# Zokrates/ZoKrates

Measured on AMD Instinct MI355X. Metric: groth16_proofs_per_sec, higher is better.
Workload: dtype u32

## Files before the change

### include/zkhip.h

```cpp
#ifndef ZKHIP_H
#define ZKHIP_H

#include <stddef.h>
#include <stdint.h>

#ifdef __cplusplus
extern "C" {
#endif

#define ZKHIP_OK 0
#define ZKHIP_ERR_BAD_ARG (-1)
#define ZKHIP_ERR_PARSE (-2)
#define ZKHIP_ERR_NOMEM (-3)
#define ZKHIP_ERR_DEVICE (-4)
#define ZKHIP_ERR_UNSATISFIED (-5)
#define ZKHIP_ERR_BUSY (-6)

#define ZKHIP_CURVE_BN128 0
#define ZKHIP_CURVE_BLS12_381 1
#define ZKHIP_CURVE_BLS12_377 2

typedef struct zkhip_ctx zkhip_ctx;
typedef struct zkhip_pk zkhip_pk;
typedef struct zkhip_r1cs zkhip_r1cs;
// ... 55 lines not shown
                        const uint64_t* rowptr_b, const uint32_t* col_b, const uint8_t* val_b,
                        const uint64_t* rowptr_c, const uint32_t* col_c, const uint8_t* val_c,
                        zkhip_r1cs** out);
void zkhip_r1cs_free(zkhip_r1cs* r1cs);

int32_t zkhip_prove_g16(zkhip_ctx* ctx, const zkhip_pk* pk, const zkhip_r1cs* r1cs, const uint8_t* z,
                        const uint8_t* r, const uint8_t* s, uint8_t* proof_out, zkhip_timings* timings);

int32_t zkhip_assignment_upload(zkhip_ctx* ctx, const zkhip_r1cs* r1cs, const uint8_t* z, zkhip_assignment** out);
void zkhip_assignment_free(zkhip_assignment* z);
int32_t zkhip_prove_g16_resident(zkhip_ctx* ctx, const zkhip_pk* pk, const zkhip_r1cs* r1cs, zkhip_assignment* z,
                                 const uint8_t* r, const uint8_t* s, uint8_t* proof_out, zkhip_timings* timings);

int32_t zkhip_assignment_pack_bound(uint64_t m, uint64_t* bytes);
int32_t zkhip_assignment_pack(const uint8_t* z, uint64_t m, uint8_t* out, uint64_t cap, uint64_t* len);
int32_t zkhip_assignment_unpack(const uint8_t* packed, size_t len, uint8_t* z_out, uint64_t m_cap, uint64_t* m);
int32_t zkhip_prog_assignment_packed(const zkhip_prog* prog, const uint8_t* witness, size_t len, uint8_t* packed_out,
                                     uint64_t cap, uint64_t* packed_len, uint8_t* inputs_out, uint64_t inputs_cap,
                                     uint64_t* n_inputs);
int32_t zkhip_assignment_upload_packed(zkhip_ctx* ctx, const zkhip_r1cs* r1cs, const uint8_t* packed, size_t len,
                                       zkhip_assignment** out);

int32_t zkhip_prove_g16_batch(zkhip_ctx* ctx, const zkhip_pk* pk, const zkhip_r1cs* r1cs, uint32_t count,
                              const uint8_t* z, const uint8_t* rs, uint8_t* proofs_out, zkhip_timings* timings);
int32_t zkhip_prove_g16_resident_batch(zkhip_ctx* ctx, const zkhip_pk* pk, const zkhip_r1cs* r1cs, uint32_t count,
                                       zkhip_assignment* const* zs, const uint8_t* rs, uint8_t* proofs_out,
                                       zkhip_timings* timings);

int32_t zkhip_r1cs_check(zkhip_ctx* ctx, const zkhip_r1cs* r1cs, const uint8_t* z, zkhip_assignment* z_resident,
                         uint64_t* first_row, uint64_t* n_bad);
int32_t zkhip_ctx_set_checked(zkhip_ctx* ctx, int32_t on);
int32_t zkhip_ctx_unsatisfied(const zkhip_ctx* ctx, uint32_t cap, uint32_t* proof_idx, uint64_t* first_row,
                              uint64_t* n_bad, uint32_t* count);

typedef struct zkhip_queue zkhip_queue;
int32_t zkhip_queue_open(zkhip_ctx* ctx, const zkhip_pk* pk, const zkhip_r1cs* r1cs, zkhip_queue** out);
int32_t zkhip_queue_state(const zkhip_queue* q, uint32_t* capacity, uint32_t* in_flight);
int32_t zkhip_queue_submit(zkhip_queue* q, const uint8_t* z, zkhip_assignment* z_resident, const uint8_t* rnd, uint64_t* ticket);
int32_t zkhip_queue_submit_packed(zkhip_queue* q, const uint8_t* packed, size_t len, const uint8_t* rnd, uint64_t* ticket);
int32_t zkhip_queue_ready(zkhip_queue* q, int32_t* ready);
int32_t zkhip_queue_collect(zkhip_queue* q, uint64_t* ticket, uint8_t* proof_out, zkhip_timings* timings);
int32_t zkhip_queue_close(zkhip_queue* q);

int32_t zkhip_pk_load_g16_shard(zkhip_ctx* ctx, int32_t curve, const uint8_t* bytes, size_t len, uint32_t rank,
                                uint32_t world, zkhip_pk** out);
int32_t zkhip_partial_size(int32_t curve, uint64_t* bytes);
int32_t zkhip_prove_g16_partial(zkhip_ctx* ctx, const zkhip_pk* pk_shard, const zkhip_r1cs* r1cs, const uint8_t* z,
                                zkhip_assignment* z_resident, const uint8_t* r, const uint8_t* s, uint8_t* partial_out,
                                zkhip_timings* timings);
int32_t zkhip_combine_g16(zkhip_ctx* ctx, const zkhip_pk* pk, uint32_t count, const uint8_t* partials, const uint8_t* r,
                          const uint8_t* s, uint8_t* proof_out);

int32_t zkhip_ntt(zkhip_ctx* ctx, int32_t curve, uint32_t log_n, int32_t dir, uint8_t* data);
int32_t zkhip_witness_map(zkhip_ctx* ctx, const zkhip_r1cs* r1cs, const uint8_t* z, uint8_t* h_out);
int32_t zkhip_msm_g1(zkhip_ctx* ctx, int32_t curve, uint64_t n, const uint8_t* bases, const uint8_t* scalars, uint8_t* out);
int32_t zkhip_msm_g2(zkhip_ctx* ctx, int32_t curve, uint64_t n, const uint8_t* bases, const uint8_t* scalars, uint8_t* out);
int32_t zkhip_field_op(zkhip_ctx* ctx, int32_t curve, int32_t field, int32_t op, uint64_t count,
                       const uint8_t* a, const uint8_t* b, uint8_t* out);

int32_t zkhip_setup_g16_size(const zkhip_r1cs* r1cs, uint64_t* pk_bytes);
int32_t zkhip_setup_g16(zkhip_ctx* ctx, const zkhip_r1cs* r1cs, const uint8_t* toxic, const uint8_t* g1,
                        const uint8_t* g2, uint8_t* pk_out, uint64_t pk_cap);

int32_t zkhip_pk_load_gm17(zkhip_ctx* ctx, int32_t curve, const uint8_t* bytes, size_t len, zkhip_pk** out);
int32_t zkhip_prove_gm17(zkhip_ctx* ctx, const zkhip_pk* pk, const zkhip_r1cs* r1cs, const uint8_t* z, const uint8_t* d1_d2_r,
                         uint8_t* proof_out, zkhip_timings* timings);
// ... 79 lines not shown
```

### integration/zokrates_hip/src/ffi.rs

```rust
#![allow(non_camel_case_types)]
use std::os::raw::c_char;

#[repr(C)] pub struct zkhip_ctx { _p: [u8; 0] }
#[repr(C)] pub struct zkhip_pk { _p: [u8; 0] }
#[repr(C)] pub struct zkhip_r1cs { _p: [u8; 0] }
#[repr(C)] pub struct zkhip_multi { _p: [u8; 0] }
#[repr(C)] pub struct zkhip_prog { _p: [u8; 0] }
#[repr(C)] pub struct zkhip_assignment { _p: [u8; 0] }
#[repr(C)] pub struct zkhip_queue { _p: [u8; 0] }
pub const ZKHIP_ERR_BUSY: i32 = -6;
#[repr(C)] #[derive(Default, Clone, Copy)] pub struct zkhip_timings { pub ms: [f32; 16] }

pub const ZKHIP_CURVE_BN128: i32 = 0;
pub const ZKHIP_CURVE_BLS12_381: i32 = 1;
pub const ZKHIP_CURVE_BLS12_377: i32 = 2;

pub const ZKHIP_TUNE_PIPE_PLAN: i32 = 28;

extern "C" {
    pub fn zkhip_init(hw_queues: i32) -> i32;
    pub fn zkhip_ctx_create(device: i32, out: *mut *mut zkhip_ctx) -> i32;
    pub fn zkhip_ctx_free(ctx: *mut zkhip_ctx);
    pub fn zkhip_ctx_tune(ctx: *mut zkhip_ctx, which: i32, value: i32) -> i32;
    pub fn zkhip_last_error(ctx: *const zkhip_ctx) -> *const c_char;
// ... 6 lines not shown
        rp_c: *const u64, col_c: *const u32, val_c: *const u8, out: *mut *mut zkhip_r1cs) -> i32;
    pub fn zkhip_r1cs_free(cs: *mut zkhip_r1cs);
    pub fn zkhip_prove_g16(ctx: *mut zkhip_ctx, pk: *const zkhip_pk, cs: *const zkhip_r1cs, z: *const u8,
        r: *const u8, s: *const u8, proof_out: *mut u8, timings: *mut zkhip_timings) -> i32;
    pub fn zkhip_prove_gm17(ctx: *mut zkhip_ctx, pk: *const zkhip_pk, cs: *const zkhip_r1cs, z: *const u8,
        d1_d2_r: *const u8, proof_out: *mut u8, timings: *mut zkhip_timings) -> i32;
    pub fn zkhip_prog_parse(bytes: *const u8, len: usize, out: *mut *mut zkhip_prog) -> i32;
    pub fn zkhip_prog_free(prog: *mut zkhip_prog);
    pub fn zkhip_prog_dims(prog: *const zkhip_prog, out: *mut u64 ) -> i32;
    pub fn zkhip_prog_r1cs_load(ctx: *mut zkhip_ctx, prog: *const zkhip_prog, out: *mut *mut zkhip_r1cs) -> i32;
    pub fn zkhip_prog_assignment(prog: *const zkhip_prog, witness: *const u8, len: usize, z_out: *mut u8,
        inputs_out: *mut u8, inputs_cap: u64, n_inputs: *mut u64) -> i32;
    pub fn zkhip_assignment_pack_bound(m: u64, bytes: *mut u64) -> i32;
    pub fn zkhip_assignment_pack(z: *const u8, m: u64, out: *mut u8, cap: u64, len: *mut u64) -> i32;
    pub fn zkhip_assignment_unpack(packed: *const u8, len: usize, z_out: *mut u8, m_cap: u64, m: *mut u64) -> i32;
    pub fn zkhip_prog_assignment_packed(prog: *const zkhip_prog, witness: *const u8, len: usize, packed_out: *mut u8,
        cap: u64, packed_len: *mut u64, inputs_out: *mut u8, inputs_cap: u64, n_inputs: *mut u64) -> i32;
    pub fn zkhip_assignment_upload_packed(ctx: *mut zkhip_ctx, r1cs: *const zkhip_r1cs, packed: *const u8, len: usize,
        out: *mut *mut zkhip_assignment) -> i32;
    pub fn zkhip_assignment_free(z: *mut zkhip_assignment);
    pub fn zkhip_prove_g16_resident(ctx: *mut zkhip_ctx, pk: *const zkhip_pk, cs: *const zkhip_r1cs, z: *mut zkhip_assignment,
        r: *const u8, s: *const u8, proof_out: *mut u8, timings: *mut zkhip_timings) -> i32;
    pub fn zkhip_pk_export_size(pk: *const zkhip_pk, bytes: *mut u64) -> i32;
    pub fn zkhip_pk_export(pk: *const zkhip_pk, out: *mut u8, cap: u64) -> i32;
    pub fn zkhip_pk_import(ctx: *mut zkhip_ctx, bytes: *const u8, len: usize, out: *mut *mut zkhip_pk) -> i32;
    pub fn zkhip_pk_bind_r1cs(ctx: *mut zkhip_ctx, pk: *mut zkhip_pk, r1cs: *const zkhip_r1cs) -> i32;
    pub fn zkhip_pk_unbind(pk: *mut zkhip_pk) -> i32;
    pub fn zkhip_pk_is_bound(pk: *const zkhip_pk, r1cs: *const zkhip_r1cs) -> i32;
    pub fn zkhip_r1cs_check(ctx: *mut zkhip_ctx, r1cs: *const zkhip_r1cs, z: *const u8, z_resident: *mut zkhip_assignment,
        first_row: *mut u64, n_bad: *mut u64) -> i32;
    pub fn zkhip_ctx_set_checked(ctx: *mut zkhip_ctx, on: i32) -> i32;
    pub fn zkhip_ctx_unsatisfied(ctx: *const zkhip_ctx, cap: u32, proof_idx: *mut u32, first_row: *mut u64, n_bad: *mut u64,
        count: *mut u32) -> i32;
    pub fn zkhip_queue_open(ctx: *mut zkhip_ctx, pk: *const zkhip_pk, r1cs: *const zkhip_r1cs, out: *mut *mut zkhip_queue) -> i32;
    pub fn zkhip_queue_state(q: *const zkhip_queue, capacity: *mut u32, in_flight: *mut u32) -> i32;
    pub fn zkhip_queue_submit(q: *mut zkhip_queue, z: *const u8, z_resident: *mut zkhip_assignment, rnd: *const u8, ticket: *mut u64) -> i32;
    pub fn zkhip_queue_submit_packed(q: *mut zkhip_queue, packed: *const u8, len: usize, rnd: *const u8, ticket: *mut u64) -> i32;
    pub fn zkhip_queue_ready(q: *mut zkhip_queue, ready: *mut i32) -> i32;
    pub fn zkhip_queue_collect(q: *mut zkhip_queue, ticket: *mut u64, proof_out: *mut u8, timings: *mut zkhip_timings) -> i32;
    pub fn zkhip_queue_close(q: *mut zkhip_queue) -> i32;
    pub fn zkhip_pk_bind_r1cs_shard(ctx: *mut zkhip_ctx, pk: *mut zkhip_pk, r1cs: *const zkhip_r1cs, key_bytes: *const u8, len: usize) -> i32;
    pub fn zkhip_prove_g16_split_begin(ctx: *mut zkhip_ctx, pk: *const zkhip_pk, r1cs: *const zkhip_r1cs, z: *const u8,
        z_resident: *mut zkhip_assignment, r: *const u8, s: *const u8, half: i32, half_out: *mut u8) -> i32;
    pub fn zkhip_prove_g16_split_end(ctx: *mut zkhip_ctx, pk: *const zkhip_pk, r1cs: *const zkhip_r1cs, other_half: *const u8,
        partial_out: *mut u8, timings: *mut zkhip_timings) -> i32;
    pub fn zkhip_prove_g16_split_abort(ctx: *mut zkhip_ctx) -> i32;
    pub fn zkhip_ctx_create_multi(devices: *const i32, n: i32, out: *mut *mut zkhip_multi) -> i32;
    pub fn zkhip_multi_free(m: *mut zkhip_multi);
    pub fn zkhip_multi_last_error(m: *const zkhip_multi) -> *const c_char;
    pub fn zkhip_multi_use_rccl(m: *mut zkhip_multi, on: i32) -> i32;
    pub fn zkhip_multi_exchange(m: *const zkhip_multi) -> *const c_char;
    pub fn zkhip_multi_r1cs_load(m: *mut zkhip_multi, curve: i32, n: u64, l: u64, w: u64,
        rp_a: *const u64, col_a: *const u32, val_a: *const u8,
        rp_b: *const u64, col_b: *const u32, val_b: *const u8,
        rp_c: *const u64, col_c: *const u32, val_c: *const u8) -> i32;
    pub fn zkhip_multi_pk_load_g16(m: *mut zkhip_multi, curve: i32, bytes: *const u8, len: usize) -> i32;
    pub fn zkhip_multi_pk_load_gm17(m: *mut zkhip_multi, curve: i32, bytes: *const u8, len: usize) -> i32;
    pub fn zkhip_multi_bind(m: *mut zkhip_multi, key_bytes: *const u8, len: usize) -> i32;
    pub fn zkhip_multi_unbind(m: *mut zkhip_multi) -> i32;
    pub fn zkhip_multi_transform_split(m: *mut zkhip_multi, on: i32) -> i32;
    pub fn zkhip_prove_g16_multi(m: *mut zkhip_multi, z: *const u8, r: *const u8, s: *const u8, proof_out: *mut u8,
        timings: *mut zkhip_timings) -> i32;
    pub fn zkhip_prove_gm17_multi(m: *mut zkhip_multi, z: *const u8, d1_d2_r: *const u8, proof_out: *mut u8,
        timings: *mut zkhip_timings) -> i32;
    pub fn zkhip_multi_pk_load_g16_replicas(m: *mut zkhip_multi, curve: i32, bytes: *const u8, len: usize) -> i32;
    pub fn zkhip_prove_g16_multi_batch(m: *mut zkhip_multi, count: u32, z: *const u8, rs: *const u8, proofs_out: *mut u8,
// ... 3 lines not shown
```

### zokrates_amd/csrc/core.cuh

```cuda
#pragma once
#include <algorithm>
#include <atomic>
#include <chrono>
#include <cstdio>
#include <memory>
#include <new>
#include <string>
#include <system_error>
#include <thread>
#include <type_traits>
#include <unordered_set>
#include <vector>

#include "../../include/zkhip.h"
#include "devrt.h"
#include "ec.cuh"
#include "kernels_msm.cuh"
#include "kernels_ntt.cuh"
#include "zpack.cuh"

namespace zk {

struct CurveBn254 {
    static constexpr int ID = ZKHIP_CURVE_BN128;
// ... 49 lines not shown
        dev_free(p);
        p = nullptr;
        cap = 0;
        p = dev_alloc(bytes);
        cap = bytes;
    }
};
template <class T> static inline T* ptr(const DBuf& b) { return (T*)b.p; }

static inline unsigned blocks_for(u64 n, unsigned threads) { return (unsigned)((n + threads - 1) / threads); }
static inline int ilog2_floor(u64 x) { int l = 0; while (x >>= 1) ++l; return l; }
static inline int ilog2_ceil(u64 x) { int l = 0; while (((u64)1 << l) < x) ++l; return l; }

}

using namespace zk;

struct NttPlanBase {
    int curve, logN;
    virtual ~NttPlanBase() {}
};
struct MsmSort {
    DBuf dig, sorted, cnt, off, cursor, chunk_sum, grand;
    DBuf pairs, ccur, tile_off;
    Event ready = nullptr;
};
struct MsmLane {
    Stream stream = 0;
    bool made = false;
    bool high_priority = false;
    DBuf lane_key, heavy, partial, bucket, rows, cols;
    Event done = nullptr;
};
static constexpr int ZK_NLANES = 5;
static constexpr int ZK_NSLOTS = 4;
struct ProofSlot {
    DBuf scalars, zmont, va, vb, vc, ws1, ws2, zflag;
    DBuf verdict;
    int check_idx = -1;
    MsmSort sorts[3];
    MsmLane lanes[ZK_NLANES];
    void* h_ws = nullptr;
    size_t h_ws_cap = 0;
    Event ev[4] = {nullptr, nullptr, nullptr, nullptr};
    Event acc_b[ZK_NLANES] = {}, acc_e[ZK_NLANES] = {};
    Event ntt_b = nullptr, ntt_e = nullptr;
    Event g1_go = nullptr;
    Event half_ready = nullptr;
    int half = -1;
    bool lone = false;
    bool split_pending = false;
    const zkhip_pk* split_pk = nullptr;
    const zkhip_r1cs* split_cs = nullptr;
    bool split_bound = false;
    bool ready = false;
    bool busy = false;
    uint8_t r[32], s[32];
    std::chrono::steady_clock::time_point t_start;
};
struct PackedZ {
    const uint8_t* bytes;
    size_t len;
    u64 tags_off, index_off, payload_off;
};
struct zkhip_queue {
    zkhip_ctx* ctx = nullptr;
    const zkhip_pk* pk = nullptr;
    const zkhip_r1cs* cs = nullptr;
    u32 cap = 0;
    u64 head = 0, next = 0;
    bool checked = false;
    bool broken = false;
    std::string dev_err;
};
struct zkhip_ctx {
    int device = 0;
    Stream stream = 0;
    Stream out_stream = 0;
    Stream ntt_stream = 0;
    bool out_made = false, ntt_made = false;
    Stream ws = 0;
    bool serial = false;
    bool g2_first = true;
    int cus = 256;
    int msm_c_env = 0;
    int b_sort_mode = 0;
    int skip_inf_mode = 0;
    int msm_sets = 0;
    int msm_waves = 0;
    u32 msm_lanes = 0;
    u32 msm_min_slice = 8;
    bool heavy_runs = true;
    int fold_hg = 32;
    bool fold_scan = true;
    bool fuse_z = true;
    int msm_fused_waves = 0;
    int msm_g1_waves = 0, msm_g2_waves = 0;
    int z_gate = 1;
    int g2_head_start = 1;
    int split_min_log = 18;
    int ntt_single_max = 10;
    int ntt_max_sublog = 11;
    int ntt_cols = 2;
    std::vector<Stream> idle_streams;
    std::string pipe_plan;
    bool pipes_made = false;
    Stream ntt_lone_stream = 0;
    bool ntt_lone_made = false;
    int ntt_fuse_first = 1;
    u32 sort_wgs = 256;
    int tenants = 1;
    int nslots = 3;
    bool checked = false;
    struct Unsatisfied { u32 proof; u64 first_row, n_bad; };
    std::vector<Unsatisfied> unsat;
    std::string err;
    std::string desc;
    ProofSlot slots[ZK_NSLOTS];
    ProofSlot* cur = &slots[0];
    zkhip_queue* queue = nullptr;
    DBuf tmp;
    DBuf zpack;
    std::vector<std::unique_ptr<NttPlanBase>> plans;
    std::unordered_set<const void*> lds_opted;
};
#define ZK_PIPE_PLAN_RESIDENT "M=2,N=3,O=1,n=3,G0=0,Z0=1,H0=0,G1=3,Z1=1,H1=0,G2=3,Z2=2,H2=1"
struct PipeWant { Stream* target; bool* made; bool high; int cls; bool done; };
static inline void make_pipe_streams(zkhip_ctx* ctx) {
    if (ctx->pipes_made || ctx->pipe_plan.empty() || ctx->serial) return;
    ctx->pipes_made = true;
    auto find = [&](const std::string& key) -> int {
        size_t pos = 0;
        const std::string& pl = ctx->pipe_plan;
        while (pos < pl.size()) {
            size_t end = pl.find(',', pos);
            if (end == std::string::npos) end = pl.size();
            const std::string tok = pl.substr(pos, end - pos);
            const size_t eq = tok.find('=');
            if (eq != std::string::npos && tok.substr(0, eq) == key && eq + 1 < tok.size() && tok[eq + 1] >= '0' && tok[eq + 1] <= '3') return tok[eq + 1] - '0';
            pos = end + 1;
        }
        return -1;
    };
    std::vector<PipeWant> want;
    static bool dummy_made;
    int c;
    if ((c = find("M")) >= 0) { stream_sync(ctx->stream); stream_destroy(ctx->stream); ctx->stream = 0; want.push_back({&ctx->stream, &dummy_made, true, c, false}); }
    if ((c = find("N")) >= 0 && !ctx->ntt_made) want.push_back({&ctx->ntt_stream, &ctx->ntt_made, true, c, false});
// ... 317 lines not shown
        }
    }
    if (ctx && ctx->msm_c_env) s.c = ctx->msm_c_env;
    if (force_c) s.c = force_c;
    s.c = std::min(s.c, MSM_MAX_C);
    s.W = (scalar_bits + 1 + s.c - 1) / s.c;
    s.K = 1u << (s.c - 1);
    s.sets = table ? (u32)std::max(1, std::min(force_sets ? force_sets : 1, s.W)) : (u32)s.W;
    s.levels = ((u32)s.W + s.sets - 1) / s.sets;
    s.nkeys = s.sets * s.K;
    s.Lw = std::min<u32>(s.K, 256);
    s.H = s.K / s.Lw;
    return s;
}

static inline MsmShape with_inf(MsmShape sh, bool many) { sh.skip_inf = many; return sh; }
static inline u64 msm_table_budget(const zkhip_ctx* ctx, u64 z_n, u64 h_n, u64 N, int W, u32 K) {
    size_t free_b = 0, total_b = 0;
    dev_mem_info(&free_b, &total_b);
    const u64 per_slot = (2 * z_n + h_n) * (u64)W * 16 + 4 * N * 32 + (z_n + 2) * 64 + 6 * ((u64)K + (1u << 19)) * 288 + ((u64)1 << 29);
    const u64 later = (u64)std::max(1, ctx->nslots) * per_slot + ((u64)1 << 30);
    const u64 budget = (u64)((ctx->tenants > 1 ? 0.5 : 0.6) * (double)free_b) / (u64)std::max(1, ctx->tenants);
    return budget > later ? budget - later : 0;
}
static inline void scan_u32(Stream s, const DBuf& cnt, DBuf& off, u64 nk, DBuf& chunk_sum, DBuf& grand) {
    const u32 nchunks = (u32)((nk + SCAN_CHUNK - 1) / SCAN_CHUNK);
    off.ensure((nk + 1) * 4);
    chunk_sum.ensure((size_t)nchunks * 4);
    grand.ensure(4);
    ZK_LAUNCH(k_scan_local, dim3(nchunks), dim3(SCAN_THREADS), 0, s, ptr<u32>(cnt), ptr<u32>(off), ptr<u32>(chunk_sum), nk);
    ZK_LAUNCH(k_scan_chunks, dim3(1), dim3(SCAN_THREADS), 0, s, ptr<u32>(chunk_sum), nchunks, ptr<u32>(grand));
    ZK_LAUNCH(k_scan_add, dim3(blocks_for(nk + 1, 256)), dim3(256), 0, s, ptr<u32>(off), ptr<u32>(chunk_sum), nk, ptr<u32>(grand));
}
static inline void msm_prepare(zkhip_ctx* ctx, Stream s, MsmSort& so, const u32* d_scalars, const MsmShape& sh, u64 level_stride,
                               const u32* keep = nullptr, const MsmSort* wm_of = nullptr) {
    const u64 nk = sh.nkeys;
    require(sh.n * (u64)sh.W < ((u64)1 << 32) - sh.nkeys, ZKHIP_ERR_BAD_ARG, "MSM too large for 32-bit sort offsets");
    require(level_stride * (u64)sh.levels < ((u64)1 << 31) && sh.n < ((u64)1 << 31), ZKHIP_ERR_BAD_ARG, "MSM too large for 31-bit table indices");
    if (!wm_of) so.dig.ensure(sh.n * (u64)sh.W * 4);
    so.sorted.ensure(sh.n * sh.W * 4);
    const unsigned T = 256;
    const u32 kh = std::min(sh.K, MSM_SORT_MAX_KH), halves = sh.K / kh;
    const u64 want_chunks = halves > 1 ? std::max<u64>(1, ctx->sort_wgs / (sh.W * halves)) : std::max<u64>(1, (ctx->sort_wgs + sh.W - 1) / sh.W);
    const u64 max_chunks = std::max<u64>(1, sh.n / (2 * (u64)kh));
    const u64 sort_chunks = std::min(want_chunks, max_chunks);
    const u64 chunk = (sh.n + sort_chunks - 1) / sort_chunks;
    const size_t hist_bytes = (size_t)kh * 4;
    const bool two_level = sh.K >= (1u << MSM_COARSE_BITS) && sh.K <= (1u << 16);
    const u32 nbins = (u32)(nk >> MSM_COARSE_BITS);
    so.cnt.ensure(nk * 4);
    so.cursor.ensure(nk * 4);
    if (two_level) {
        so.ccur.ensure((size_t)nbins * 4);
        so.tile_off.ensure(((size_t)nbins + 1) * 4);
    }
    const MsmZero zero{{ptr<u32>(so.cnt), ptr<u32>(so.cursor), two_level ? ptr<u32>(so.ccur) : nullptr}, {(u32)nk, (u32)nk, two_level ? nbins : 0u}};
    if (!wm_of) ZK_LAUNCH(k_msm_digits, dim3(blocks_for(sh.n, T)), dim3(T), 0, s, d_scalars, sh.n, sh.c, sh.W, ptr<u32>(so.dig), zero);
    else ZK_LAUNCH(k_msm_zero, dim3(blocks_for(nk, T)), dim3(T), 0, s, zero);
    const u32* wm = wm_of ? ptr<u32>(wm_of->dig) : ptr<u32>(so.dig);
    lds_opt_in(ctx, (const void*)k_msm_count);
    lds_opt_in(ctx, (const void*)k_msm_place);
    ZK_LAUNCH(k_msm_count, dim3((unsigned)sort_chunks, sh.W, halves), dim3(ZK_SORT_THREADS), hist_bytes, s, wm, sh.n, sh.c, sh.W, chunk, sh.sets, kh,
              ptr<u32>(so.cnt), keep);
    if (nk <= SCAN_ONE_MAX) {
        so.off.ensure((nk + 1) * 4);
        ZK_LAUNCH(k_scan_one, dim3(1), dim3(SCAN_ONE_THREADS), 0, s, ptr<u32>(so.cnt), ptr<u32>(so.off), (u32)nk, two_level ? ptr<u32>(so.tile_off) : (u32*)nullptr, nbins);
    } else {
        scan_u32(s, so.cnt, so.off, nk, so.chunk_sum, so.grand);
        if (two_level) ZK_LAUNCH(k_msm_tile_offsets, dim3(1), dim3(MSM_TILE_SCAN_THREADS), 0, s, ptr<u32>(so.off), nbins, ptr<u32>(so.tile_off));
    }
    if (two_level) {
        const u64 total_max = sh.n * (u64)sh.W;
        so.pairs.ensure(std::max<u64>(total_max, 1) * 8);
        const u64 c_chunks = std::max<u64>(1, std::min<u64>((1024 + sh.W - 1) / sh.W, (sh.n + 4095) / 4096));
        const u64 c_chunk = (sh.n + c_chunks - 1) / c_chunks;
        ZK_LAUNCH(k_msm_part_coarse, dim3((unsigned)c_chunks, sh.W), dim3(256), 0, s, wm, sh.n, sh.c, sh.W, c_chunk, sh.sets, level_stride, ptr<u32>(so.off),
                  ptr<u32>(so.ccur), (unsigned long long*)so.pairs.p, keep);
        const u64 max_tiles = total_max / MSM_FINE_TILE + nbins;
        ZK_LAUNCH(k_msm_part_fine, dim3((unsigned)max_tiles), dim3(256), 0, s, (const unsigned long long*)so.pairs.p, ptr<u32>(so.off), ptr<u32>(so.tile_off), nbins,
                  ptr<u32>(so.cursor), ptr<u32>(so.sorted));
    } else {
        ZK_LAUNCH(k_msm_place, dim3((unsigned)sort_chunks, sh.W, halves), dim3(ZK_SORT_THREADS), hist_bytes, s, wm, sh.n, sh.c, sh.W, chunk, sh.sets, kh,
                  level_stride, ptr<u32>(so.off), ptr<u32>(so.cursor), ptr<u32>(so.sorted), keep);
    }
    event_record(so.ready, s);
}

template <class F>
void msm_run(zkhip_ctx* ctx, MsmLane& lane, const MsmSort& so, const void* d_table, const MsmShape& sh, Xyzz<F>* d_window_sums,
             Event ev_begin, Event ev_end, Event accum_after = nullptr, Xyzz<F>* h_window_sums = nullptr);
template <class F>
void msm_run_tables(zkhip_ctx* ctx, MsmLane& lane, const MsmSort& so, const void* const* d_tables, int nt, const MsmShape& sh, Xyzz<F>* d_window_sums,
                    u32 sum_stride, Event ev_begin, Event ev_end, Event accum_after, Xyzz<F>* h_window_sums = nullptr);
template <class F>
void points_to_packed(zkhip_ctx* ctx, const Aff<F>* d_in, void* d_out, u64 n);
template <class F>
void msm_table_levels(zkhip_ctx* ctx, void* d_table, u64 count, int bits, int L);
template <class F>
u64 count_infinite(zkhip_ctx* ctx, const void* d_table, u64 count);
template <class F>
void mark_finite(zkhip_ctx* ctx, const void* d_table, u64 count, u32* d_bitmap);
template <class F> static constexpr size_t packed_point_bytes() { return sizeof(AffPacked<typename Unsat<F>::type>); }
template <class F>
size_t bind_xyzz_bytes();
template <class F>
void bind_scale(zkhip_ctx* ctx, const void* d_h_table, u64 N, u64 n_src, u32 n1, u32 n2, u32 n3, const u32* d_scal, const u32* d_konst, int nw, void* d_x);
template <class F>
void bind_fft(zkhip_ctx* ctx, void* d_x, u64 N, const u32* d_tw, int nw);
template <class F>
void bind_h_finish(zkhip_ctx* ctx, const void* d_x, u64 N, int logN, void* d_out);
template <class F>
void bind_cmul(zkhip_ctx* ctx, const void* d_x, int logN, const u32* d_row, const u32* d_val, int nw, const u32* d_minus_one, u64 nnz, void* d_prod);
template <class F>
void bind_l_finish(zkhip_ctx* ctx, const void* d_prod, const u64* d_cptr, const void* d_l_table, u64 m, const u32* d_long_cols, u64 n_long, void* d_sum, void* d_out);
template <class F>
void fixed_base_table(zkhip_ctx* ctx, const Aff<F>* h_pj, int nwin, DBuf& tbl);
template <class F>
void fixed_base_mul(zkhip_ctx* ctx, const DBuf& tbl, int nwin, const u32* d_scalars, u64 count, Aff<F>* d_out);

template <class F>
static Xyzz<F> msm_combine(const Xyzz<F>* ws, const MsmShape& sh) {
    auto set_sum = [&](int j) {
        Xyzz<F> t = ws[sh.ndig * j];
        for (u32 d = 1; d < sh.ndig; ++d) t = xyzz_add(t, ws[sh.ndig * j + d]);
        return t;
    };
// ... 23 lines not shown
static void decode_point(const uint8_t* src, uint8_t* dst) {
    constexpr int SZ = FQ_BYTES * NCOORD;
    const bool inf = src[SZ - 1] & 0x40;
    if (inf) { memset(dst, 0, SZ); return; }
    memcpy(dst, src, SZ);
    dst[SZ - 1] &= 0x3f;
}
template <class F> static void write_fe(const F& mont, uint8_t* out) { F c = fe_from_mont(mont); memcpy(out, c.v, F::BYTES); }

}

struct zkhip_pk {
    int curve;
    int scheme = 0;
    zkhip_ctx* ctx;
    u64 m, w, l, hlen, N;
    int logN;
    DBuf a_ext, b1_ext, l_ext, b2_ext, h_sigma;
    std::vector<uint8_t> delta_g1_canon;
    std::vector<uint8_t> g_gamma2_z2_canon;
    u32 rank = 0, world = 1;
    u64 z_lo = 0, z_n = 0, h_lo = 0, h_n = 0;
    int c_z = 0, c_h = 0;
    DBuf thin_keep;
    u32 thin_mask = 0;
    bool inf_many_thin[4] = {true, true, true, true};
    bool inf_many[5] = {true, true, true, true, true};
    int s_z = 1, s_h = 1;
    int ntt_log1 = -1;
    DBuf h_bound, l_bound;
    u64 bound_uid = 0;
    u64 bound_fp[2] = {0, 0};
    bool inf_many_bound[2] = {true, true};
};

static const char PK_IMAGE_MAGIC[8] = {'Z', 'K', 'H', 'I', 'P', 'P', 'K', '5'};
struct PkImageHeader {
    char magic[8];
    int32_t curve, scheme;
    uint64_t m, w, l, hlen, N;
    int32_t logN, c_z, c_h, sets;
    uint32_t rank, world;
    int32_t ntt_split, reserved;
    uint64_t z_lo, z_n, h_lo, h_n;
    uint64_t len_delta, len_g2z2, len_buf[5];
    uint64_t len_bound[2];
    uint64_t bound_fp[2];
};

static inline u64 zk_next_uid() {
    static std::atomic<u64> next{1};
    return next.fetch_add(1);
}
struct zkhip_r1cs {
    u64 uid = zk_next_uid();
    int curve;
    zkhip_ctx* ctx;
    u64 n, l, w, N;
    int logN;
    DBuf rp[3], col[3], val[3];
    u64 nnz[3];
    u64 nnz_short[3];
    DBuf long_rows;
    u64 n_long = 0, n_huge = 0;
    u64 fp[2] = {0, 0};
    bool fp_made = false;
// ... 20 lines not shown
struct zkhip_assignment {
    int curve;
    zkhip_ctx* ctx;
    u64 m;
    DBuf scalars;
};

namespace zk {

template <class C>
struct SlotSums {
    typedef Xyzz<typename C::Fq> G1;
    typedef Xyzz<typename C::Fq2> G2;
    MsmShape shz, shh;
    int Wmax;
    SlotSums(const zkhip_ctx* ctx, const zkhip_pk* pk)
        : shz(msm_shape(ctx, pk->z_n, C::Fr::Params::BITS, true, pk->c_z, pk->s_z)), shh(msm_shape(ctx, pk->h_n, C::Fr::Params::BITS, true, pk->c_h, pk->s_h)) {
        require(shz.c == pk->c_z && shh.c == pk->c_h && (int)shz.sets == pk->s_z && (int)shh.sets == pk->s_h, ZKHIP_ERR_BAD_ARG,
                "the key's tables were built for a window width this build cannot sort: reload the key");
        Wmax = (int)std::max(shz.nsums(), shh.nsums());
    }
    size_t b1() const { return (size_t)4 * Wmax * sizeof(G1); }
    size_t b2() const { return (size_t)Wmax * sizeof(G2); }
    size_t lane_bytes() const { return (size_t)Wmax * sizeof(G1); }
    size_t record_bytes() const { return b1() + b2() + 24; }
    template <class T> T* lane(T* g1_sums, int k) const { return g1_sums + (size_t)k * Wmax; }
    G1* ws1(const ProofSlot& sl, int k) const { return lane(ptr<G1>(sl.ws1), k); }
    G2* ws2(const ProofSlot& sl) const { return ptr<G2>(sl.ws2); }
    G1* hs1(const ProofSlot& sl, int k) const { return lane((G1*)sl.h_ws, k); }
    G2* hs2(const ProofSlot& sl) const { return (G2*)((uint8_t*)sl.h_ws + b1()); }
    uint8_t* zflag(const ProofSlot& sl) const { return (uint8_t*)sl.h_ws + b1() + b2(); }
    uint8_t* verdict(const ProofSlot& sl) const { return zflag(sl) + 8; }
    u32 zflag_word(const ProofSlot& sl) const { u32 f; memcpy(&f, zflag(sl), 4); return f; }
    void reserve(ProofSlot& sl) const {
        sl.ws1.ensure(b1());
        sl.ws2.ensure(b2());
        if (sl.h_ws_cap < record_bytes()) {
            host_free_pinned(sl.h_ws);
            sl.h_ws = nullptr; sl.h_ws_cap = 0;
            sl.h_ws = host_alloc_pinned(record_bytes());
            sl.h_ws_cap = record_bytes();
        }
    }
};

struct KeySources {
    int scheme;
    u64 m, w, l, hlen, N;
    struct Lane {
        const uint8_t* src; u64 nsrc, shift;
        const uint8_t* extra; u64 extra_at;
        const uint8_t* add0;
    } lane[4];
    const uint8_t* h_src; u64 h_nsrc;
    const uint8_t *delta_g1, *g_gamma2_z2;
};
struct SapShape {
    u64 M, D0, D;
    int logD;
};
static inline SapShape sap_shape(u64 n, u64 l, u64 w) {
    SapShape s;
    s.M = 1 + 2 * (l - 1) + w + n;
    s.D0 = 2 * n + 2 * (l - 1) + 1;
    s.logD = ilog2_ceil(s.D0);
    s.D = (u64)1 << s.logD;
// ... 719 lines not shown
                 (unsigned long long)cs->n, (unsigned long long)u.n_bad);
        throw ApiError{ZKHIP_ERR_UNSATISFIED, msg};
    }
    static Fr k_to_rp() {
        Fr rp = Fr::one();
        for (int i = 32 * Fr::N; i < Fu<typename Fr::Params>::B * Fu<typename Fr::Params>::N; ++i) rp = fe_add(rp, rp);
        return fe_to_mont(rp);
    }
    static void r1cs_check(zkhip_ctx* ctx, const zkhip_r1cs* cs, const uint8_t* z_host, const void* z_dev, u64 out[2]) {
        ProofSlot& sl = *ctx->cur;
        Stream s = ctx->stream;
        ctx->ws = s;
        const u64 m = cs->l + cs->w, n = cs->n;
        const Fr* z = stage_z(ctx, sl, m, m + 2, z_host, z_dev, true, true);
        sl.zmont.ensure(m * 32);
        ZK_LAUNCH((k_mul_const<Fr>), dim3(blocks_for(m, 256)), dim3(256), 0, s, z, ptr<Fr>(sl.zmont), m, k_to_rp());
        sl.vc.ensure(3 * std::max<u64>(n, 1) * sizeof(Fr));
        Fr *ra = ptr<Fr>(sl.vc), *rb = ra + n, *rc = rb + n;
        if (n) matvec(ctx, cs, ptr<Fr>(sl.zmont), ra, rb, rc, n, 0, n);
        enqueue_check(sl, ra, rb, rc, n, s);
        u32 flag = 0;
        dev_d2h(&flag, sl.zflag.p, 4, s);
        dev_d2h(out, sl.verdict.p, 16, s);
        stream_sync(s);
        require_canonical(flag);
    }

    static void upload_z(zkhip_ctx* ctx, DBuf& dst, u64 m, u64 cap, const uint8_t* z, DBuf& flag) {
        Fr z0 = fe_from_bytes_canon<Fr>(z);
        Fr one = Fr::zero(); one.v[0] = 1;
        require(z0.equals(one), ZKHIP_ERR_BAD_ARG, Z0_NOT_ONE_MSG);
        dst.ensure(cap * 32);
        dev_h2d(dst.p, z, m * 32, ctx->stream);
        flag.ensure(4);
        dev_memset(flag.p, 0, 4, ctx->stream);
        ZK_LAUNCH((k_check_canonical<Fr>), dim3(blocks_for(m, 256)), dim3(256), 0, ctx->stream, ptr<Fr>(dst), m, ptr<u32>(flag));
    }
    static void unpack_z(zkhip_ctx* ctx, DBuf& dst, u64 m, u64 cap, const PackedZ& zp, DBuf& flag) {
        Stream s = ctx->stream;
        dst.ensure(cap * 32);
        ctx->zpack.ensure(zp.len);
        dev_h2d(ctx->zpack.p, zp.bytes, zp.len, s);
        flag.ensure(4);
        dev_memset(flag.p, 0, 4, s);
        const uint8_t* d = ptr<uint8_t>(ctx->zpack);
        ZK_LAUNCH((k_unpack_assignment<Fr>), dim3(blocks_for(m, ZPACK_BLOCK_ELEMS)), dim3(256), 0, s, d + zp.tags_off, (const u64*)(d + zp.index_off),
                  d + zp.payload_off, ptr<Fr>(dst), m, ptr<u32>(flag));
    }
    static const Fr* stage_z(zkhip_ctx* ctx, ProofSlot& sl, u64 m, u64 cap, const uint8_t* z_host, const void* z_dev, bool checked, bool in_place = false,
                             const PackedZ* zp = nullptr) {
        Stream st = ctx->stream;
        if (zp) {
            unpack_z(ctx, sl.scalars, m, cap, *zp, sl.zflag);
            if (checked) verdict_reset(sl, st);
            return ptr<Fr>(sl.scalars);
        }
        if (z_host) {
            upload_z(ctx, sl.scalars, m, cap, z_host, sl.zflag);
        } else {
            if (!in_place) {
                sl.scalars.ensure(cap * 32);
                dev_d2d(sl.scalars.p, z_dev, m * 32, st);
            }
            sl.zflag.ensure(4);
            dev_memset(sl.zflag.p, 0, 4, st);
        }
        if (checked) verdict_reset(sl, st);
        return (z_host || !in_place) ? ptr<Fr>(sl.scalars) : (const Fr*)z_dev;
    }
    static void require_canonical(u32 flag) {
        require(flag == 0, ZKHIP_ERR_BAD_ARG, "an assignment entry is not a canonical field element (>= r)");
    }
    static void stage_scalars(zkhip_ctx* ctx, NttPlan<C>* pl, void* d_scalars, u64 m, const uint8_t* r, const uint8_t* s_) {
        Stream s = ctx->stream;
        ctx->cur->zmont.ensure(m * 32);
        dev_h2d((uint8_t*)d_scalars + m * 32, r, 32, s);
        dev_h2d((uint8_t*)d_scalars + (m + 1) * 32, s_, 32, s);
        ZK_LAUNCH((k_mul_const<Fr>), dim3(blocks_for(m, 256)), dim3(256), 0, s, (const Fr*)d_scalars, ptr<Fr>(ctx->cur->zmont), m, pl->k_to_rp);
    }

    static void enqueue(zkhip_ctx* ctx, ProofSlot& sl, const zkhip_pk* pk, const zkhip_r1cs* cs, const uint8_t* z_host, const void* z_dev,
                        const uint8_t* r, const uint8_t* s_, bool lone = false, int check_idx = -1, const PackedZ* zp = nullptr) {
        enqueue_head(ctx, sl, pk, cs, z_host, z_dev, r, s_, lone, -1, check_idx, zp);
        enqueue_tail(ctx, sl, pk, cs);
    }
    static bool can_split(const zkhip_ctx* ctx, const zkhip_pk* pk, const zkhip_r1cs* cs) {
        return pk->scheme == 0 && is_bound(pk, cs) && pk->logN >= ctx->split_min_log;
    }
    static bool is_bound(const zkhip_pk* pk, const zkhip_r1cs* cs) { return pk->bound_uid != 0 && pk->bound_uid == cs->uid; }
    static NttPlan<C>* open_slot(zkhip_ctx* ctx, ProofSlot& sl, const zkhip_pk* pk) {
        require(!sl.busy, ZKHIP_ERR_DEVICE, "internal: proof slot still in flight");
        make_pipe_streams(ctx);
        slot_init(ctx, sl);
        NttPlan<C>* pl = get_plan<C>(ctx, pk->logN);
        require(pl->split() == pk->ntt_log1, ZKHIP_ERR_BAD_ARG, "the key's h bases were ordered for another NTT split (NTT_SINGLE_MAX_LOG changed): reload the key");
        sl.t_start = std::chrono::steady_clock::now();
        ctx->cur = &sl;
        ctx->ws = ctx->stream;
        return pl;
    }
    static void enqueue_head(zkhip_ctx* ctx, ProofSlot& sl, const zkhip_pk* pk, const zkhip_r1cs* cs, const uint8_t* z_host, const void* z_dev,
                             const uint8_t* r, const uint8_t* s_, bool lone, int half, int check_idx = -1, const PackedZ* zp = nullptr) {
        PkLoader<C>::check_match(pk, cs, 0);
        const bool bound = is_bound(pk, cs);
        require(half < 0 || (bound && half <= 1), ZKHIP_ERR_BAD_ARG, "internal: only a proof over a bound key splits its witness map");
        Fr rr = fe_from_bytes_canon<Fr>(r), ss = fe_from_bytes_canon<Fr>(s_);
        require(canon_lt_mod(rr) && canon_lt_mod(ss), ZKHIP_ERR_BAD_ARG, "r or s not a canonical field element");
        NttPlan<C>* pl = open_slot(ctx, sl, pk);
        sl.half = half;
        sl.lone = lone;
        sl.check_idx = half < 0 ? check_idx : -1;
        memcpy(sl.r, r, 32);
        memcpy(sl.s, s_, 32);
        Stream st = ctx->stream;
        stage_z(ctx, sl, pk->m, pk->m + 2, z_host, z_dev, sl.check_idx >= 0, false, zp);
        stage_scalars(ctx, pl, sl.scalars.p, pk->m, r, s_);
        event_record(sl.ev[0], st);

        const Lay ly(ctx, pk);
        ly.reserve(sl);
        start_z_lanes(ctx, sl, pk, ly);

        Stream wn = ctx->serial ? st : slot_ntt_stream(ctx, sl);
        stream_wait_event(wn, sl.ev[0]);
        event_record(sl.ev[1], wn);
        ctx->ws = wn;
        witness_map(ctx, cs, pl, bound, half, sl.check_idx >= 0);
        ctx->ws = ctx->stream;
        if (half >= 0) {
            event_record(sl.half_ready, wn);
            sl.split_pk = pk;
            sl.split_cs = cs;
            sl.split_bound = bound;
            sl.split_pending = true;
        }
    }
    static void enqueue_tail(zkhip_ctx* ctx, ProofSlot& sl, const zkhip_pk* pk, const zkhip_r1cs* cs) {
        const u64 N = pk->N;
        ctx->cur = &sl;
        Stream wn = ctx->serial ? ctx->stream : slot_ntt_stream(ctx, sl);
        const u32* h_scalars = ptr<u32>(sl.va) + (sl.half >= 0 ? 2 * N * 8 : 0);
        if (sl.half >= 0) {
            Fr* a = ptr<Fr>(sl.va);
            ZK_LAUNCH((k_quotient<typename Fr::Params>), dim3(blocks_for(N, 256)), dim3(256), 0, wn, a, a + N, fe_from_mont(get_plan<C>(ctx, pk->logN)->zinv), a + 2 * N, N);
        }
        lanes_after_h(ctx, sl, pk, Lay(ctx, pk), sl.half >= 0 ? sl.split_bound : is_bound(pk, cs), sl.lone, h_scalars, wn);
    }

    static void start_z_lanes(zkhip_ctx* ctx, ProofSlot& sl, const zkhip_pk* pk, const Lay& ly) {
        if (!pk->z_n) return;
        const u32* digits = ptr<u32>(sl.scalars) + pk->z_lo * 8;
        msm_prepare(ctx, ctx->stream, sl.sorts[0], digits, ly.shz, pk->z_n);
        if (pk->thin_mask) msm_prepare(ctx, ctx->stream, sl.sorts[2], digits, ly.shz, pk->z_n, ptr<u32>(pk->thin_keep), &sl.sorts[0]);
        if (z_gate(ctx) < 2) run_g2(ctx, sl, pk, ly, nullptr);
    }
    static void run_g2(zkhip_ctx* ctx, ProofSlot& sl, const zkhip_pk* pk, const Lay& ly, Event after) {
        const bool thin = pk->thin_mask & 8;
        msm_run<Fq2>(ctx, sl.lanes[3], sl.sorts[thin ? 2 : 0], pk->b2_ext.p, with_inf(ly.shz, thin ? pk->inf_many_thin[3] : pk->inf_many[3]), ly.ws2(sl),
                     sl.acc_b[4], sl.acc_e[4], after, ly.hs2(sl));
    }
    static void lanes_after_h(zkhip_ctx* ctx, ProofSlot& sl, const zkhip_pk* pk, const Lay& ly, bool bound, bool lone, const u32* h_scalars, Stream wn) {
        Stream st = ctx->stream;
        event_record(sl.ev[2], wn);
        if (pk->z_n) {
            const int gate = z_gate(ctx);
            const Event h_ready = gate ? sl.ev[2] : nullptr;
            if (gate >= 2) run_g2(ctx, sl, pk, ly, h_ready);
            Event g1_after = h_ready;
            constexpr bool g2_owns_simds = MsmTuning<typename Unsat<Fq2>::type>::ACCUM_WPE == 1;
            if (g2_owns_simds && lone && !ctx->serial && (ctx->g2_head_start == 2 || (ctx->g2_head_start == 1 && bound))) {
                if (h_ready) stream_wait_event(st, h_ready);
                stream_wait_event(st, sl.acc_e[4]);
                event_record(sl.g1_go, st);
                g1_after = sl.g1_go;
            }
            run_z_g1(ctx, sl, pk, ly, g1_after, bound);
        } else {
            empty_msm(ctx, sl, ly, true);
        }
        if (pk->h_n) {
            msm_prepare(ctx, wn, sl.sorts[1], h_scalars + pk->h_lo * 8, ly.shh, pk->h_n);
            msm_run<Fq>(ctx, sl.lanes[4], sl.sorts[1], bound ? pk->h_bound.p : pk->h_sigma.p, with_inf(ly.shh, bound ? pk->inf_many_bound[1] : pk->inf_many[4]),
                        ly.ws1(sl, 3), sl.acc_b[3], sl.acc_e[3], nullptr, ly.hs1(sl, 3));
        } else {
            empty_msm(ctx, sl, ly, false);
        }
        copy_out(ctx, sl, ly);
    }

    static void run_z_g1(zkhip_ctx* ctx, ProofSlot& sl, const zkhip_pk* pk, const Lay& ly, Event h_ready, bool bound) {
        const void* tab[3] = {pk->a_ext.p, pk->b1_ext.p, bound ? pk->l_bound.p : pk->l_ext.p};
        auto thin = [&](int k) { return (bound && k == 2) ? 0u : (pk->thin_mask >> k) & 1u; };
        auto inf_many = [&](int k) { return (bound && k == 2) ? pk->inf_many_bound[0] : thin(k) ? pk->inf_many_thin[k] : pk->inf_many[k]; };
        if (!ctx->fuse_z) {
            for (int k = 0; k < 3; ++k)
                msm_run<Fq>(ctx, sl.lanes[k], thin(k) ? sl.sorts[2] : sl.sorts[0], tab[k], with_inf(ly.shz, inf_many(k)), ly.ws1(sl, k), sl.acc_b[k], sl.acc_e[k], h_ready,
                            ly.hs1(sl, k));
            return;
        }
        for (u32 which = 0; which < 2; ++which) {
            int member[3], nm = 0;
            for (int k = 0; k < 3; ++k)
                if (thin(k) == which) member[nm++] = k;
            if (!nm) continue;
            const int lead = member[0];
            const void* tabs[3];
            bool many = false;
            for (int q = 0; q < nm; ++q) { tabs[q] = tab[member[q]]; many = many || inf_many(member[q]); }
            const int step = nm > 1 ? member[1] - member[0] : 1;
            msm_run_tables<Fq>(ctx, sl.lanes[lead], which ? sl.sorts[2] : sl.sorts[0], tabs, nm, with_inf(ly.shz, many), ly.ws1(sl, lead), (u32)(step * ly.Wmax),
                               sl.acc_b[lead], sl.acc_e[lead], h_ready, ly.hs1(sl, lead));
            Stream s0 = ctx->serial ? ctx->stream : lane_stream(sl.lanes[lead]);
            for (int q = 1; q < nm; ++q) {
                event_record(sl.acc_b[member[q]], s0);
                event_record(sl.acc_e[member[q]], s0);
                event_record(sl.lanes[member[q]].done, s0);
            }
        }
    }

    static void copy_out(zkhip_ctx* ctx, ProofSlot& sl, const Lay& ly) {
        Stream st = ctx->stream;
        Stream so = ctx->serial ? st : ctx_out_stream(ctx);
        for (int k = 0; k < ZK_NLANES; ++k) stream_wait_event(so, sl.lanes[k].done);
        sl.zflag.ensure(4);
        dev_d2h_pinned(ly.zflag(sl), sl.zflag.p, 4, so);
        if (sl.check_idx >= 0) {
            stream_wait_event(so, sl.ev[2]);
            dev_d2h_pinned(ly.verdict(sl), sl.verdict.p, 16, so);
        }
        event_record(sl.ev[3], so);
        sl.busy = true;
    }

    static void empty_msm(zkhip_ctx* ctx, ProofSlot& sl, const Lay& ly, bool over_z) {
        Stream st = ctx->stream;
        const int k0 = over_z ? 0 : 3, nk = over_z ? 3 : 1;
        dev_memset(ly.ws1(sl, k0), 0, nk * ly.lane_bytes(), st);
        memset(ly.hs1(sl, k0), 0, nk * ly.lane_bytes());
        if (over_z) {
            dev_memset(ly.ws2(sl), 0, ly.b2(), st);
            memset(ly.hs2(sl), 0, ly.b2());
        }
        for (int k = over_z ? 0 : 4; k < (over_z ? 4 : 5); ++k) {
            const int e = k == 3 ? 4 : k == 4 ? 3 : k;
            event_record(sl.acc_b[e], st);
            event_record(sl.acc_e[e], st);
            event_record(sl.lanes[k].done, st);
        }
    }

    struct Sums {
        Xyzz<Fq> a, b1, l, h;
        Xyzz<Fq2> b2;
    };
    static Sums collect(zkhip_ctx* ctx, ProofSlot& sl, const zkhip_pk* pk) {
        require(sl.busy, ZKHIP_ERR_DEVICE, "internal: no proof in flight in this slot");
        event_sync(sl.ev[3]);
        sl.busy = false;
        split_clear(sl);
        const Lay ly(ctx, pk);
        require_canonical(ly.zflag_word(sl));
        Sums g;
        HostThreads th;
        th.run([&] { g.a = msm_combine(ly.hs1(sl, 0), ly.shz); });
        th.run([&] { g.b1 = msm_combine(ly.hs1(sl, 1), ly.shz); });
        th.run([&] { g.l = msm_combine(ly.hs1(sl, 2), ly.shz); });
        th.run([&] { g.h = msm_combine(ly.hs1(sl, 3), ly.shh); });
        g.b2 = msm_combine(ly.hs2(sl), ly.shz);
        th.join();
        return g;
    }
    static void assemble(const zkhip_pk* pk, const Sums& g, const uint8_t* r, const uint8_t* s_, uint8_t* out) {
        const Fr rr = fe_from_bytes_canon<Fr>(r), ss = fe_from_bytes_canon<Fr>(s_);
        Xyzz<Fq> sA, rB1, rsD;
        {
            HostThreads th;
            th.run([&] { sA = xyzz_mul_limbs(g.a, ss.v, Fr::N); });
            th.run([&] { rB1 = xyzz_mul_limbs(g.b1, rr.v, Fr::N); });
            rsD = rs_delta(pk, rr, ss);
        }
        assemble_tail(g, sA, rB1, rsD, out);
    }
    static void assemble_tail(const Sums& g, const Xyzz<Fq>& sA, const Xyzz<Fq>& rB1, const Xyzz<Fq>& rsD, uint8_t* out) {
        Xyzz<Fq> gC = xyzz_add(sA, rB1);
        gC = xyzz_add(gC, xyzz_neg(rsD));
        gC = xyzz_add(gC, g.l);
        gC = xyzz_add(gC, g.h);
        Aff<Fq> pa, pc;
        Aff<Fq2> pb;
        {
            HostThreads th;
            th.run([&] { pa = xyzz_to_affine(g.a); });
            th.run([&] { pc = xyzz_to_affine(gC); });
// ... 25 lines not shown
            for (int k = 0; k < 4; ++k) tm->kernel_msm_accum_g1_ms += event_elapsed_ms(sl.acc_b[k], sl.acc_e[k]);
            tm->kernel_msm_accum_g2_ms = event_elapsed_ms(sl.acc_b[4], sl.acc_e[4]);
        }
    }
    static void finish(zkhip_ctx* ctx, ProofSlot& sl, const zkhip_pk* pk, uint8_t* out, zkhip_timings* tm) {
        require(pk->world == 1, ZKHIP_ERR_BAD_ARG, "this proving key is one shard of a multi-GPU key: use zkhip_prove_g16_partial + zkhip_combine_g16");
        require(sl.busy, ZKHIP_ERR_DEVICE, "internal: no proof in flight in this slot");
        const Lay ly(ctx, pk);
        const Fr rr = fe_from_bytes_canon<Fr>(sl.r), ss = fe_from_bytes_canon<Fr>(sl.s);
        Sums g;
        Xyzz<Fq> sA, rB1, rsD;
        std::chrono::steady_clock::time_point t_fin;
        try {
            HostThreads th;
            th.run([&] { rsD = rs_delta(pk, rr, ss); });
            event_sync(sl.lanes[3].done);
            g.b2 = msm_combine(ly.hs2(sl), ly.shz);
            for (int k = 0; k < 3; ++k) event_sync(sl.lanes[k].done);
            g.a = msm_combine(ly.hs1(sl, 0), ly.shz);
            g.b1 = msm_combine(ly.hs1(sl, 1), ly.shz);
            th.run([&] { sA = xyzz_mul_limbs(g.a, ss.v, Fr::N); });
            th.run([&] { rB1 = xyzz_mul_limbs(g.b1, rr.v, Fr::N); });
            g.l = msm_combine(ly.hs1(sl, 2), ly.shz);
            event_sync(sl.lanes[4].done);
            t_fin = std::chrono::steady_clock::now();
            g.h = msm_combine(ly.hs1(sl, 3), ly.shh);
            event_sync(sl.ev[3]);
            th.join();
        } catch (...) {
            sl.busy = false;
            throw;
        }
        sl.busy = false;
        require_canonical(ly.zflag_word(sl));
        if (unsatisfied(ctx, sl, ly)) memset(out, 0, PROOF_BYTES);
        else assemble_tail(g, sA, rB1, rsD, out);
        fill_timings(sl, tm, t_fin);
    }
    static Xyzz<Fq> rs_delta(const zkhip_pk* pk, const Fr& rr, const Fr& ss) {
        const Fr rs = fe_from_mont(fe_mul(fe_to_mont(rr), fe_to_mont(ss)));
        uint8_t dec[2 * FQB];
        decode_point<FQB, 2>(pk->delta_g1_canon.data(), dec);
        Aff<Fq> d1;
        memcpy(&d1, dec, sizeof(d1));
        d1 = PkLoader<C>::to_mont_point(d1);
        return xyzz_mul_limbs(Xyzz<Fq>::from_affine(d1), rs.v, Fr::N);
    }
    template <class F>
    static Xyzz<F> canonical(const Xyzz<F>& p) {
        if (p.is_inf()) return Xyzz<F>::inf();
        const Aff<F> a = xyzz_to_affine(p);
        return {a.x, a.y, F::one(), F::one()};
    }
    static void emit_partial(zkhip_ctx* ctx, ProofSlot& sl, const zkhip_pk* pk, uint8_t* partial_out, zkhip_timings* tm) {
        Sums g = collect(ctx, sl, pk);
        const auto t_fin = std::chrono::steady_clock::now();
        HostThreads th;
        th.run([&] { g.a = canonical(g.a); });
        th.run([&] { g.b1 = canonical(g.b1); });
        th.run([&] { g.l = canonical(g.l); });
        th.run([&] { g.h = canonical(g.h); });
        g.b2 = canonical(g.b2);
        th.join();
        memcpy(partial_out, &g, sizeof(g));
        fill_timings(sl, tm, t_fin);
    }
// ... 36 lines not shown
    static void split_half_out(zkhip_ctx* ctx, const zkhip_pk* pk, uint8_t* out) {
        Stream wn;
        ProofSlot& sl = split_slot(ctx, pk, &wn);
        dev_d2h(out, ptr<Fr>(sl.va) + (u64)sl.half * pk->N, pk->N * sizeof(Fr), wn);
        stream_sync(wn);
    }
    static void split_end_partial(zkhip_ctx* ctx, const zkhip_pk* pk, const zkhip_r1cs* cs, uint8_t* partial_out, zkhip_timings* tm) {
        ProofSlot& sl = split_slot(ctx, pk);
        require(sl.split_cs == cs, ZKHIP_ERR_BAD_ARG, "the split proof pending in this context was begun with another constraint system");
        enqueue_tail(ctx, sl, pk, cs);
        emit_partial(ctx, ctx->slots[0], pk, partial_out, tm);
    }
    static void split_end_device_sums(zkhip_ctx* ctx, const zkhip_pk* pk, const zkhip_r1cs* cs, const void** d_ws1, size_t* b1, const void** d_ws2, size_t* b2,
                                      zkhip_timings* tm) {
        ProofSlot& sl = split_slot(ctx, pk);
        require(sl.split_cs == cs, ZKHIP_ERR_BAD_ARG, "the split proof pending in this context was begun with another constraint system");
        enqueue_tail(ctx, sl, pk, cs);
        hand_out_sums(ctx, ctx->slots[0], pk, d_ws1, b1, d_ws2, b2, tm);
    }
    static void prove_device_sums(zkhip_ctx* ctx, const zkhip_pk* pk, const zkhip_r1cs* cs, const uint8_t* z_host, const uint8_t* r,
                                  const uint8_t* s_, const void** d_ws1, size_t* b1, const void** d_ws2, size_t* b2, zkhip_timings* tm) {
        enqueue(ctx, ctx->slots[0], pk, cs, z_host, nullptr, r, s_);
        hand_out_sums(ctx, ctx->slots[0], pk, d_ws1, b1, d_ws2, b2, tm);
    }
    static void hand_out_sums(zkhip_ctx* ctx, ProofSlot& sl, const zkhip_pk* pk, const void** d_ws1, size_t* b1, const void** d_ws2, size_t* b2,
                              zkhip_timings* tm) {
        require(sl.busy, ZKHIP_ERR_DEVICE, "internal: no proof in flight in this slot");
        event_sync(sl.ev[3]);
        sl.busy = false;
        split_clear(sl);
        const Lay ly(ctx, pk);
        *b1 = ly.b1();
        *b2 = ly.b2();
        require_canonical(ly.zflag_word(sl));
        *d_ws1 = sl.ws1.p;
        *d_ws2 = sl.ws2.p;
        fill_timings(sl, tm, std::chrono::steady_clock::now());
    }
    static void record_from_sums(zkhip_ctx* ctx, const zkhip_pk* pk, const uint8_t* ws1, const uint8_t* ws2, uint8_t* record_out) {
        const Lay ly(ctx, pk);
        std::vector<Xyzz<Fq>> a1(ly.b1() / sizeof(Xyzz<Fq>));
        std::vector<Xyzz<Fq2>> a2(ly.b2() / sizeof(Xyzz<Fq2>));
        memcpy(a1.data(), ws1, ly.b1());
        memcpy(a2.data(), ws2, ly.b2());
        Sums g;
        g.a = msm_combine(ly.lane(a1.data(), 0), ly.shz);
        g.b1 = msm_combine(ly.lane(a1.data(), 1), ly.shz);
        g.l = msm_combine(ly.lane(a1.data(), 2), ly.shz);
        g.h = msm_combine(ly.lane(a1.data(), 3), ly.shh);
        g.b2 = msm_combine(a2.data(), ly.shz);
        memcpy(record_out, &g, sizeof(g));
    }
    static Sums sum_partials(u32 count, const uint8_t* partials) {
        Sums t;
        t.a = t.b1 = t.l = t.h = Xyzz<Fq>::inf();
        t.b2 = Xyzz<Fq2>::inf();
        for (u32 i = 0; i < count; ++i) {
            Sums g;
            memcpy(&g, partials + (size_t)i * sizeof(Sums), sizeof(g));
            t.a = xyzz_add(t.a, g.a); t.b1 = xyzz_add(t.b1, g.b1); t.l = xyzz_add(t.l, g.l); t.h = xyzz_add(t.h, g.h);
            t.b2 = xyzz_add(t.b2, g.b2);
        }
        return t;
    }
    static void combine(const zkhip_pk* pk, u32 count, const uint8_t* partials, const uint8_t* r, const uint8_t* s_, uint8_t* out) {
        const Sums t = sum_partials(count, partials);
// ... 55 lines not shown
        stream_sync(ctx->stream);
        require_canonical(verdict);
    }
    static void assignment_upload_packed(zkhip_ctx* ctx, zkhip_assignment* a, const uint8_t* packed, size_t len, u64 tags_off, u64 index_off,
                                         u64 payload_off) {
        Stream s = ctx->stream;
        DBuf flag;
        unpack_z(ctx, a->scalars, a->m, a->m + 2, PackedZ{packed, len, tags_off, index_off, payload_off}, flag);
        u32 verdict = 0;
        dev_d2h(&verdict, flag.p, 4, s);
        stream_sync(s);
        require_canonical(verdict);
    }

    template <class F, int NC>
    static void msm_api(zkhip_ctx* ctx, u64 n, const uint8_t* bases, const uint8_t* scalars, uint8_t* out) {
        constexpr int PB = FQB * NC;
        memset(out, 0, PB + 1);
        if (n == 0) { out[PB] = 1; return; }
        require(n < ((u64)1 << 31), ZKHIP_ERR_BAD_ARG, "too many points");
        Stream s = ctx->stream;
        std::vector<uint8_t> host(n * PB);
        for (u64 i = 0; i < n; ++i) decode_point<FQB, NC>(bases + i * PB, &host[i * PB]);
        DBuf d_bases, d_ws;
        d_bases.ensure(host.size());
        dev_h2d(d_bases.p, host.data(), host.size(), s);
        ZK_LAUNCH((k_to_mont<Fq>), dim3(blocks_for(n * NC, 256)), dim3(256), 0, s, ptr<Fq>(d_bases), ptr<Fq>(d_bases), n * NC);
        ctx->cur->scalars.ensure(n * 32);
        dev_h2d(ctx->cur->scalars.p, scalars, n * 32, s);
        const MsmShape sh = msm_shape(ctx, n, Fr::Params::BITS, false);
        d_ws.ensure((size_t)sh.nsums() * sizeof(Xyzz<F>));
        DBuf d_packed;
        d_packed.ensure(n * packed_point_bytes<F>());
#ifdef ZK_TEST_MSM_RACE
        msm_prepare(ctx, s, ctx->cur->sorts[0], ptr<u32>(ctx->cur->scalars), sh, 0);
        points_to_packed<F>(ctx, ptr<Aff<F>>(d_bases), d_packed.p, n);
#else
        points_to_packed<F>(ctx, ptr<Aff<F>>(d_bases), d_packed.p, n);
        msm_prepare(ctx, s, ctx->cur->sorts[0], ptr<u32>(ctx->cur->scalars), sh, 0);
#endif
        msm_run<F>(ctx, ctx->cur->lanes[0], ctx->cur->sorts[0], d_packed.p, sh, ptr<Xyzz<F>>(d_ws), nullptr, nullptr);
        stream_wait_event(s, ctx->cur->lanes[0].done);
        std::vector<Xyzz<F>> ws(sh.nsums());
        dev_d2h(ws.data(), d_ws.p, ws.size() * sizeof(Xyzz<F>), s);
        stream_sync(s);
        Xyzz<F> res = msm_combine(ws.data(), sh);
        if (res.is_inf()) { out[PB] = 1; return; }
        Aff<F> a = xyzz_to_affine(res);
        uint8_t tmp[sizeof(Aff<F>)];
        Aff<F> canon = from_mont_point(a);
        memcpy(tmp, &canon, sizeof(canon));
        memcpy(out, tmp, PB);
    }
    static Aff<Fq> from_mont_point(const Aff<Fq>& p) { return {fe_from_mont(p.x), fe_from_mont(p.y)}; }
    static Aff<Fq2> from_mont_point(const Aff<Fq2>& p) { return {fe_from_mont(p.x), fe_from_mont(p.y)}; }

    static void ntt_api(zkhip_ctx* ctx, u32 log_n, int dir, uint8_t* data) {
        NttPlan<C>* pl = get_plan<C>(ctx, (int)log_n);
        Stream s = ctx->stream;
        ctx->ws = s;
        const u64 N = pl->N;
        const unsigned T = 256, B = blocks_for(N, T);
        ctx->cur->va.ensure(N * sizeof(Fr));
        ctx->cur->vb.ensure(N * sizeof(Fr));
        ctx->cur->vc.ensure(N * sizeof(Fr));
        Fr *a = ptr<Fr>(ctx->cur->va), *b = ptr<Fr>(ctx->cur->vb), *t = ptr<Fr>(ctx->cur->vc);
        dev_h2d(a, data, N * 32, s);
        ZK_LAUNCH((k_mul_const<Fr>), dim3(B), dim3(T), 0, s, a, a, N, pl->k_to_rp);
        const bool inverse = dir == 1 || dir == 3;
        if (dir == 2) {
            ZK_LAUNCH((k_pow_table<Fr>), dim3(B), dim3(T), 0, s, t, pl->g, Fr::one(), N, 0u, 0u, 0);
            ZK_LAUNCH((k_mul_table<Fr>), dim3(B), dim3(T), 0, s, a, t, a, N);
        }
        ntt_kind_a<C>(ctx, pl, a, inverse, nullptr, 1, 0, 1);
        ZK_LAUNCH((k_sigma_permute<Fr>), dim3(B), dim3(T), 0, s, a, b, N, pl->N1, pl->N2, 1, pl->N3);
        if (inverse) {
            ZK_LAUNCH((k_pow_table<Fr>), dim3(B), dim3(T), 0, s, t, dir == 3 ? pl->g_inv : Fr::one(), pl->n_inv, N, 0u, 0u, 0);
            ZK_LAUNCH((k_mul_table<Fr>), dim3(B), dim3(T), 0, s, b, t, b, N);
        }
        ZK_LAUNCH((k_from_rp<Fr>), dim3(B), dim3(T), 0, s, b, b, N);
        dev_d2h(data, b, N * 32, s);
        stream_sync(s);
        if (log_n > 24) {
            ctx->cur->va.release(); ctx->cur->vb.release(); ctx->cur->vc.release();
            for (size_t k = 0; k < ctx->plans.size(); ++k)
                if (ctx->plans[k].get() == pl) { ctx->plans.erase(ctx->plans.begin() + (long)k); break; }
        }
    }

    static void witness_map_api(zkhip_ctx* ctx, const zkhip_r1cs* cs, const uint8_t* z, uint8_t* h_out) {
        ctx->ws = ctx->stream;
        NttPlan<C>* pl = get_plan<C>(ctx, cs->logN);
        const u64 m = cs->l + cs->w;
        uint8_t zero[32] = {0};
        upload_z(ctx, ctx->cur->scalars, m, m + 2, z, ctx->cur->zflag);
        stage_scalars(ctx, pl, ctx->cur->scalars.p, m, zero, zero);
        witness_map(ctx, cs, pl);
        ctx->cur->vb.ensure(pl->N * sizeof(Fr));
        ZK_LAUNCH((k_sigma_permute<Fr>), dim3(blocks_for(pl->N, 256)), dim3(256), 0, ctx->stream, ptr<Fr>(ctx->cur->va), ptr<Fr>(ctx->cur->vb), pl->N,
                  pl->N1, pl->N2, 1, pl->N3);
        dev_d2h(h_out, ctx->cur->vb.p, pl->N * 32, ctx->stream);
        stream_sync(ctx->stream);
    }

    template <class F, class Launch>
    static void field_op_api(zkhip_ctx* ctx, u64 count, unsigned T, const uint8_t* a, const uint8_t* b, uint8_t* out, Launch launch) {
        Stream s = ctx->stream;
        const size_t bytes = count * sizeof(F);
        ctx->cur->va.ensure(bytes); ctx->cur->vb.ensure(bytes);
        dev_h2d(ctx->cur->va.p, a, bytes, s);
        dev_h2d(ctx->cur->vb.p, b, bytes, s);
        const unsigned B = blocks_for(count, T);
        ZK_LAUNCH((k_to_mont<F>), dim3(B), dim3(T), 0, s, ptr<F>(ctx->cur->va), ptr<F>(ctx->cur->va), count);
        ZK_LAUNCH((k_to_mont<F>), dim3(B), dim3(T), 0, s, ptr<F>(ctx->cur->vb), ptr<F>(ctx->cur->vb), count);
        launch(dim3(B), dim3(T), s, ptr<F>(ctx->cur->va), ptr<F>(ctx->cur->vb));
        ZK_LAUNCH((k_from_mont<F>), dim3(B), dim3(T), 0, s, ptr<F>(ctx->cur->va), ptr<F>(ctx->cur->va), count);
        dev_d2h(out, ctx->cur->va.p, bytes, s);
        stream_sync(s);
    }

    static void r1cs_load(zkhip_ctx* ctx, zkhip_r1cs* cs, const u64* const rp[3], const u32* const col[3], const uint8_t* const val[3]) {
        Stream s = ctx->stream;
        std::vector<u64> long_rows, huge_rows;
        const u64 huge_min = env_int("ZKHIP_MATVEC_HUGE", 0, 1, 1) ? (u64)MATVEC_HUGE : ~(u64)0;
        for (int k = 0; k < 3; ++k) {
            const u64 nnz = rp[k][cs->n];
            require(rp[k][0] == 0, ZKHIP_ERR_BAD_ARG, "rowptr[0] must be 0");
            for (u64 i = 0; i < cs->n; ++i) require(rp[k][i] <= rp[k][i + 1], ZKHIP_ERR_BAD_ARG, "rowptr not monotone");
            cs->nnz_short[k] = nnz;
// ... 155 lines not shown
```

### zokrates_amd/csrc/devrt.h

```cpp
#pragma once
#include <algorithm>
#include <atomic>
#include <cstddef>
#include <mutex>
#include <unordered_map>
#include <cstdint>
#include <cstdio>
#include <cstdlib>
#include <cstring>
#include <string>
#include <system_error>
#include <thread>
#include <vector>

#ifdef ZK_EMU
#include "emu.h"
#else
#include <hip/hip_runtime.h>
#endif

namespace zk {

struct DevError {
    std::string msg;
// ... 2 lines not shown
struct HostThreads {
    std::vector<std::thread> th;
    HostThreads() { th.reserve(64); }
    HostThreads(const HostThreads&) = delete;
    HostThreads& operator=(const HostThreads&) = delete;
    template <class Fn>
    void run(Fn&& fn) {
        try {
            th.emplace_back(fn);
        } catch (const std::system_error&) {
            fn();
        }
    }
    void join() {
        for (auto& t : th)
            if (t.joinable()) t.join();
        th.clear();
    }
    ~HostThreads() { join(); }
};


template <class Fn>
inline void host_parallel_for(uint64_t n, Fn&& fn, unsigned max_threads = 8) {
    unsigned hw = std::thread::hardware_concurrency();
    const unsigned T = (unsigned)std::max<uint64_t>(1, std::min<uint64_t>(std::min<unsigned>(hw ? hw : 1, max_threads), n / 65536));
    if (T <= 1) { fn((uint64_t)0, n); return; }
    HostThreads th;
    for (unsigned t = 1; t < T; ++t) th.run([&fn, n, t, T] { fn(n * t / T, n * (t + 1) / T); });
    fn((uint64_t)0, n / T);
    th.join();
}

#ifndef ZK_EMU
#define ZK_HIP_CHECK(expr)                                                                        \
    do {                                                                                          \
        hipError_t e_ = (expr);                                                                   \
        if (e_ != hipSuccess)                                                                     \
            throw zk::DevError{std::string(#expr) + ": " + hipGetErrorString(e_)};                \
    } while (0)

typedef hipStream_t Stream;
typedef hipEvent_t Event;

inline int dev_count() {
    int n = 0;
    if (hipGetDeviceCount(&n) != hipSuccess) return 0;
    return n;
}
inline void dev_set(int d) { ZK_HIP_CHECK(hipSetDevice(d)); }
inline void dev_pci_bus_id(int d, char* out, size_t cap) { ZK_HIP_CHECK(hipDeviceGetPCIBusId(out, (int)cap, d)); }
struct DevAllocTable {
    std::mutex mu;
    std::unordered_map<void*, void*> base_of;
    unsigned counter = 0;
};
inline DevAllocTable& dev_alloc_table() {
    static DevAllocTable t;
    return t;
}
inline void* dev_alloc(size_t bytes) {
    const size_t page = (size_t)2 << 20, slots = 61;
    static const size_t step = getenv("ZKHIP_ALLOC_STEP") ? (size_t)atol(getenv("ZKHIP_ALLOC_STEP")) / 256 * 256 : 4352;
    DevAllocTable& t = dev_alloc_table();
    std::lock_guard<std::mutex> lock(t.mu);
    const size_t offset = (size_t)(t.counter++ % slots) * step;
    void* base = nullptr;
    ZK_HIP_CHECK(hipMalloc(&base, (std::max<size_t>(bytes, 1) + offset + page - 1) / page * page));
// ... 71 lines not shown
    std::mutex mu;
    void init() {
        if (buf[0]) return;
        for (int i = 0; i < SLOTS; ++i) {
            ZK_HIP_CHECK(hipHostMalloc(&buf[i], CHUNK, hipHostMallocDefault));
            ZK_HIP_CHECK(hipEventCreateWithFlags(&ev[i], hipEventDisableTiming));
        }
    }
    int acquire() {
        const int i = next;
        next = (next + 1) % SLOTS;
        if (used[i]) ZK_HIP_CHECK(hipEventSynchronize(ev[i]));
        used[i] = false;
        return i;
    }
};
inline StagingRing& staging_ring() {
    static StagingRing rings[64];
    int d = 0;
    (void)hipGetDevice(&d);
    StagingRing& r = rings[d & 63];
    return r;
}
inline void staging_drain() {
    StagingRing& r = staging_ring();
    std::lock_guard<std::mutex> lock(r.mu);
    if (!r.buf[0]) return;
    for (int i = 0; i < StagingRing::SLOTS; ++i)
        if (r.used[i]) {
            (void)hipEventSynchronize(r.ev[i]);
            r.used[i] = false;
        }
}
inline void dev_h2d_pinned(void* d, const void* h, size_t n, Stream s) { jitter_before(s); ZK_HIP_CHECK(hipMemcpyAsync(d, h, n, hipMemcpyHostToDevice, s)); }
inline void dev_d2h_pinned(void* h, const void* d, size_t n, Stream s) { jitter_before(s); ZK_HIP_CHECK(hipMemcpyAsync(h, d, n, hipMemcpyDeviceToHost, s)); }
inline void dev_h2d(void* d, const void* h, size_t n, Stream s) {
    if (!n) return;
    const int mode = copy_mode();
    if (mode == 0) { dev_h2d_pinned(d, h, n, s); return; }
    if (mode == 1) {
        ZK_HIP_CHECK(hipStreamSynchronize(s));
        ZK_HIP_CHECK(hipMemcpy(d, h, n, hipMemcpyHostToDevice));
        return;
    }
    StagingRing& r = staging_ring();
    std::lock_guard<std::mutex> lock(r.mu);
    r.init();
    const size_t nchunks = (n + StagingRing::CHUNK - 1) / StagingRing::CHUNK;
    const unsigned T = nchunks >= 2 ? staging_copy_threads() : 1;
    if (T > 1) {
        struct Shared {
            std::atomic<long> go{-1}, done{0};
            std::atomic<bool> abort{false};
            unsigned T = 1;
            std::vector<char*> slot;
        } sh;
        sh.slot.assign(nchunks, nullptr);
        auto share = [n](size_t c, unsigned t, unsigned T_, size_t& lo, size_t& hi) {
            const size_t len = std::min(StagingRing::CHUNK, n - c * StagingRing::CHUNK);
            lo = len * t / T_ / 64 * 64;
            hi = t + 1 == T_ ? len : len * (t + 1) / T_ / 64 * 64;
        };
        struct Release {
            Shared& sh;
            ~Release() { sh.abort.store(true, std::memory_order_release); }
        };
        HostThreads th;
        Release release{sh};
        for (unsigned t = 1; t < T; ++t) {
            try {
                const unsigned me = (unsigned)th.th.size() + 1;
                th.th.emplace_back([&sh, &share, h, nchunks, me] {
// ... 45 lines not shown
    if (!n) return;
    StagingRing& r = staging_ring();
    std::lock_guard<std::mutex> lock(r.mu);
    r.init();
    const size_t chunk = std::max<size_t>(unit, StagingRing::CHUNK / unit * unit);
    if (chunk > StagingRing::CHUNK) throw DevError{"dev_h2d_fill: unit larger than a staging slot"};
    for (size_t off = 0; off < n; off += chunk) {
        const size_t len = std::min(chunk, n - off);
        const int i = r.acquire();
        char* dst = (char*)r.buf[i];
        const size_t units = len / unit;
        const unsigned T = (unsigned)std::max<size_t>(1, std::min<size_t>(threads, units / 4096));
        if (T <= 1) {
            fill(dst, off, len);
        } else {
            HostThreads th;
            for (unsigned t = 1; t < T; ++t) {
                const size_t lo = units * t / T * unit, hi = (t + 1 == T ? len : units * (t + 1) / T * unit);
                th.run([&fill, dst, off, lo, hi] { fill(dst + lo, off + lo, hi - lo); });
            }
            fill(dst, off, units / T * unit);
            th.join();
        }
        jitter_before(s);
        ZK_HIP_CHECK(hipMemcpyAsync((char*)d + off, r.buf[i], len, hipMemcpyHostToDevice, s));
        ZK_HIP_CHECK(hipEventRecord(r.ev[i], s));
        r.used[i] = true;
    }
}
inline void dev_d2h(void* h, const void* d, size_t n, Stream s) {
    if (!n) return;
    const int mode = copy_mode();
    if (mode == 0) { dev_d2h_pinned(h, d, n, s); return; }
    if (mode == 1) {
        ZK_HIP_CHECK(hipStreamSynchronize(s));
        ZK_HIP_CHECK(hipMemcpy(h, d, n, hipMemcpyDeviceToHost));
        return;
    }
    StagingRing& r = staging_ring();
    std::lock_guard<std::mutex> lock(r.mu);
    r.init();
    int pending[2] = {-1, -1};
    size_t pend_off[2] = {0, 0}, pend_len[2] = {0, 0};
    int q = 0;
    auto drain = [&](int k) {
        if (pending[k] < 0) return;
        ZK_HIP_CHECK(hipEventSynchronize(r.ev[pending[k]]));
        memcpy((char*)h + pend_off[k], r.buf[pending[k]], pend_len[k]);
        r.used[pending[k]] = false;
        pending[k] = -1;
    };
    for (size_t off = 0; off < n; off += StagingRing::CHUNK) {
        const size_t len = std::min(StagingRing::CHUNK, n - off);
        drain(q);
        const int i = r.acquire();
        jitter_before(s);
        ZK_HIP_CHECK(hipMemcpyAsync(r.buf[i], (const char*)d + off, len, hipMemcpyDeviceToHost, s));
        ZK_HIP_CHECK(hipEventRecord(r.ev[i], s));
        r.used[i] = true;
        pending[q] = i; pend_off[q] = off; pend_len[q] = len;
        q ^= 1;
    }
    drain(q);
    drain(q ^ 1);
}
inline void dev_d2d(void* d, const void* s_, size_t n, Stream s) { jitter_before(s); ZK_HIP_CHECK(hipMemcpyAsync(d, s_, n, hipMemcpyDeviceToDevice, s)); }
inline void dev_copy_between(void* d, int dst_dev, const void* s_, int src_dev, size_t n, Stream s) {
    jitter_before(s);
    if (dst_dev == src_dev) ZK_HIP_CHECK(hipMemcpyAsync(d, s_, n, hipMemcpyDeviceToDevice, s));
    else ZK_HIP_CHECK(hipMemcpyPeerAsync(d, dst_dev, s_, src_dev, n, s));
}
inline void dev_memset(void* d, int v, size_t n, Stream s) { jitter_before(s); ZK_HIP_CHECK(hipMemsetAsync(d, v, n, s)); }
inline Stream stream_create() {
    Stream s;
    ZK_HIP_CHECK(hipStreamCreateWithFlags(&s, hipStreamNonBlocking));
    return s;
}
inline Stream stream_create_high_priority() {
    int lo = 0, hi = 0;
    ZK_HIP_CHECK(hipDeviceGetStreamPriorityRange(&lo, &hi));
    Stream s;
    ZK_HIP_CHECK(hipStreamCreateWithPriority(&s, hipStreamNonBlocking, hi));
    return s;
}
inline Stream stream_create_low_priority() {
    int lo = 0, hi = 0;
    ZK_HIP_CHECK(hipDeviceGetStreamPriorityRange(&lo, &hi));
    Stream s;
    ZK_HIP_CHECK(hipStreamCreateWithPriority(&s, hipStreamNonBlocking, lo));
    return s;
}
inline void stream_destroy(Stream s) { (void)hipStreamDestroy(s); }
inline void stream_sync(Stream s) { ZK_HIP_CHECK(hipStreamSynchronize(s)); }
inline void dev_sync_all() { (void)hipDeviceSynchronize(); }
inline void dev_mem_info(size_t* free_b, size_t* total_b) { ZK_HIP_CHECK(hipMemGetInfo(free_b, total_b)); }
inline Event event_create() {
    Event e;
    ZK_HIP_CHECK(hipEventCreate(&e));
    return e;
// ... 2 lines not shown
inline void event_record(Event e, Stream s) { ZK_HIP_CHECK(hipEventRecord(e, s)); }
inline void event_sync(Event e) { ZK_HIP_CHECK(hipEventSynchronize(e)); }
inline bool event_done(Event e) {
    const hipError_t rc = hipEventQuery(e);
    if (rc == hipErrorNotReady) return false;
    ZK_HIP_CHECK(rc);
    return true;
}
inline void stream_wait_event(Stream s, Event e) { ZK_HIP_CHECK(hipStreamWaitEvent(s, e, 0)); }
inline float event_elapsed_ms(Event a, Event b) {
    float ms = 0;
    hipError_t e = hipEventElapsedTime(&ms, a, b);
    if (e == hipErrorNotReady) {
        (void)hipGetLastError();
        ZK_HIP_CHECK(hipEventSynchronize(a));
        ZK_HIP_CHECK(hipEventSynchronize(b));
        e = hipEventElapsedTime(&ms, a, b);
    }
    ZK_HIP_CHECK(e);
    return ms;
}
inline void dev_check_last() { ZK_HIP_CHECK(hipGetLastError()); }

inline bool trace_enabled() {
    static const bool on = getenv("ZKHIP_TRACE") != nullptr;
    return on;
}
inline bool grid_nonempty(const dim3& g) { return g.x != 0 && g.y != 0 && g.z != 0; }
#define ZK_LAUNCH(kernel, grid, block, smem, stream, ...)                                 \
    do {                                                                                  \
        if (!zk::grid_nonempty(dim3(grid))) break;                                        \
        if (zk::trace_enabled()) fprintf(stderr, "[zkhip] launch %s ...", #kernel);       \
        zk::jitter_before(stream);                                                        \
        hipLaunchKernelGGL(kernel, grid, block, smem, stream, __VA_ARGS__);               \
        zk::dev_check_last();                                                             \
        if (zk::trace_enabled()) {                                                        \
            ZK_HIP_CHECK(hipStreamSynchronize(stream));                                   \
            fprintf(stderr, " done\n");                                                   \
        }                                                                                 \
    } while (0)
#define ZK_DYN_SMEM(name) extern __shared__ __attribute__((aligned(16))) unsigned char name[]
#ifndef ZK_WAVE_PRIO
#define ZK_WAVE_PRIO 3
#endif
#define ZK_PRIO_HIGH() __builtin_amdgcn_s_setprio(ZK_WAVE_PRIO)
#define ZK_WAVE_ANY(pred) (__builtin_amdgcn_ballot_w64(pred) != 0)
#define ZK_WAVE_BALLOT(pred) ((unsigned long long)__builtin_amdgcn_ballot_w64(pred))
#ifdef ZK_CHECKED
#define ZK_ASSERT_IDX(cond) do { if (!(cond)) __builtin_trap(); } while (0)
#else
#define ZK_ASSERT_IDX(cond) ((void)0)
#endif

#else

typedef int Stream;
typedef double* Event;
inline int dev_count() { return 1; }
inline void dev_set(int) {}
inline void dev_pci_bus_id(int, char* out, size_t cap) { snprintf(out, cap, "0000:00:00.0"); }
inline void* dev_alloc(size_t bytes) { return aligned_alloc(256, ((bytes ? bytes : 16) + 255) / 256 * 256); }
inline void dev_free(void* p) { free(p); }
inline void* host_alloc_pinned(size_t bytes) { return dev_alloc(bytes); }
inline void host_free_pinned(void* p) { free(p); }
inline void dev_h2d(void* d, const void* h, size_t n, Stream) { memcpy(d, h, n); }
template <class Fill>
inline void dev_h2d_fill(void* d, size_t n, size_t unit, Stream, Fill&& fill, unsigned = 8) {
    const size_t units = n / unit, cut = units / 3 * unit;
    if (cut) fill((char*)d, (size_t)0, cut);
    if (n > cut) fill((char*)d + cut, cut, n - cut);
}
inline void dev_d2h(void* h, const void* d, size_t n, Stream) { memcpy(h, d, n); }
inline void staging_drain() {}
inline void dev_h2d_pinned(void* d, const void* h, size_t n, Stream) { memcpy(d, h, n); }
inline void dev_d2h_pinned(void* h, const void* d, size_t n, Stream) { memcpy(h, d, n); }
inline void dev_d2d(void* d, const void* s_, size_t n, Stream) { memcpy(d, s_, n); }
inline void dev_copy_between(void* d, int, const void* s_, int, size_t n, Stream) { memcpy(d, s_, n); }
inline void dev_memset(void* d, int v, size_t n, Stream) { memset(d, v, n); }
inline Stream stream_create() { return 0; }
inline Stream stream_create_high_priority() { return 0; }
inline Stream stream_create_low_priority() { return 0; }
inline void stream_destroy(Stream) {}
inline void stream_sync(Stream) {}
inline void dev_sync_all() {}
inline void dev_mem_info(size_t* free_b, size_t* total_b) { *free_b = *total_b = (size_t)1 << 40; }
inline Event event_create() { return new double(0); }
inline void event_destroy(Event e) { delete e; }
inline void event_record(Event e, Stream) { *e = emu::now_ms(); }
inline void event_sync(Event) {}
inline bool event_done(Event) { return true; }
inline void stream_wait_event(Stream, Event) {}
inline float event_elapsed_ms(Event a, Event b) { return (float)(*b - *a); }
inline void dev_check_last() {}
struct JitterState { std::atomic<int> max_us{0}; };
inline JitterState& jitter_state() { static JitterState st; return st; }

#define ZK_LAUNCH(kernel, grid, block, smem, stream, ...) \
    emu::launch(dim3(grid), dim3(block), (size_t)(smem), [&]() { kernel(__VA_ARGS__); })
#define ZK_DYN_SMEM(name) unsigned char* name = emu::dyn_smem()
#define ZK_PRIO_HIGH() ((void)0)
#define ZK_WAVE_ANY(pred) (emu::wave_ballot(pred) != 0)
#define ZK_WAVE_BALLOT(pred) emu::wave_ballot(pred)
#ifdef ZK_CHECKED
#define ZK_ASSERT_IDX(cond) do { if (!(cond)) { fprintf(stderr, "ZK_ASSERT_IDX failed: %s (%s:%d)\n", #cond, __FILE__, __LINE__); abort(); } } while (0)
#else
#define ZK_ASSERT_IDX(cond) ((void)0)
#endif

#endif

}
```

### zokrates_amd/csrc/gm17.cuh

```cuda
#pragma once

namespace zk {

template <class P>
__global__ void k_sap_rows(const Fe<P>* __restrict__ ra, const Fe<P>* __restrict__ rb, const Fe<P>* __restrict__ rc, const Fe<P>* __restrict__ z,
                           Fe<P>* __restrict__ sa, Fe<P>* __restrict__ sc, Fe<P>* __restrict__ ext, u64 n, u64 l, u64 m) {
    ZK_PRIO_HIGH();
    typedef Fe<P> F;
    u64 i = (u64)blockIdx.x * blockDim.x + threadIdx.x;
    if (i >= n + l) return;
    if (i < n) {
        const F a = ra[i], b = rb[i];
        const F d = fe_sub(a, b);
        const F e = rp_sqr(d);
        sa[2 * i] = fe_add(a, b);
        sa[2 * i + 1] = d;
        if (sc) {
            sc[2 * i] = fe_add(fe_dbl(fe_dbl(rc[i])), e);
            sc[2 * i + 1] = e;
        }
        ext[m + i] = rp_to_plain(e);
    } else if (i == n) {
        sa[2 * n] = rp_one<P>();
        if (sc) sc[2 * n] = rp_one<P>();
// ... 23 lines not shown
__global__ void k_gm17_coeffs(const F* __restrict__ a, const F* __restrict__ c, F gamma, F ab, F two_g2z, F* __restrict__ aq, F* __restrict__ c1,
                              F* __restrict__ c2, F* __restrict__ vq, u64 n) {
    u64 i = (u64)blockIdx.x * blockDim.x + threadIdx.x;
    if (i >= n) return;
    const F v = fe_add(fe_mul(gamma, c[i]), fe_mul(ab, a[i]));
    aq[i] = fe_from_mont(fe_mul(gamma, a[i]));
    c1[i] = fe_from_mont(fe_mul(gamma, v));
    c2[i] = fe_from_mont(fe_mul(two_g2z, a[i]));
    vq[i] = fe_from_mont(v);
}

template <class C>
struct Gm17 {
    typedef typename C::Fr Fr;
    typedef typename C::Fq Fq;
    typedef typename C::Fq2 Fq2;
    typedef PkLoader<C> L;
    typedef Prover<C> P;
    static constexpr int FQB = Fq::BYTES;
    static constexpr int G1B = 2 * FQB, G2B = 4 * FQB;

    static Fr add_mod(const Fr& a, const Fr& b) {
        return fe_from_mont(fe_add(fe_to_mont(a), fe_to_mont(b)));
    }
    static void enqueue(zkhip_ctx* ctx, ProofSlot& sl, const zkhip_pk* pk, const zkhip_r1cs* cs, const uint8_t* z_host, const void* z_dev,
                        const uint8_t* d1, const uint8_t* r, int check_idx = -1, const PackedZ* zp = nullptr) {
        L::check_match(pk, cs, 1);
        const u64 m = cs->l + cs->w, n = cs->n, l = cs->l, M = pk->m, D = pk->N;
        Fr dd = fe_from_bytes_canon<Fr>(d1), rr = fe_from_bytes_canon<Fr>(r);
        require(canon_lt_mod(dd) && canon_lt_mod(rr), ZKHIP_ERR_BAD_ARG, "d1 or r not a canonical field element");
        const Fr rho = add_mod(dd, rr);
        const bool bound = P::is_bound(pk, cs);
        NttPlan<C>* pl = P::open_slot(ctx, sl, pk);
        sl.check_idx = check_idx;
        memcpy(sl.r, rho.v, 32);
        memset(sl.s, 0, 32);
        Stream st = ctx->stream;
        P::stage_z(ctx, sl, m, M + 2, z_host, z_dev, check_idx >= 0, false, zp);
        uint8_t* d_scalars = (uint8_t*)sl.scalars.p;
        sl.zmont.ensure(m * 32);
        dev_h2d(d_scalars + M * 32, sl.r, 32, st);
        dev_memset(d_scalars + (M + 1) * 32, 0, 32, st);
        ZK_LAUNCH((k_mul_const<Fr>), dim3(blocks_for(m, 256)), dim3(256), 0, st, (const Fr*)d_scalars, ptr<Fr>(sl.zmont), m, pl->k_to_rp);
        event_record(sl.ev[0], st);

        sl.va.ensure(2 * D * sizeof(Fr));
        Fr *sa = ptr<Fr>(sl.va), *sc = sa + D;
        const u64 D0 = 2 * n + 2 * (l - 1) + 1;
        if (D0 < D) {
            dev_memset(sa + D0, 0, (D - D0) * sizeof(Fr), st);
            if (!bound) dev_memset(sc + D0, 0, (D - D0) * sizeof(Fr), st);
        }
        sl.vc.ensure(3 * std::max<u64>(n, 1) * sizeof(Fr));
        Fr *ra = ptr<Fr>(sl.vc), *rb = ra + n, *rc = rb + n;
        if (n) P::matvec(ctx, cs, ptr<Fr>(sl.zmont), ra, rb, rc, n, 0, n, (bound && check_idx < 0) ? 2 : 3);
        if (check_idx >= 0) P::enqueue_check(sl, ra, rb, rc, n, st);
        ZK_LAUNCH((k_sap_rows<typename Fr::Params>), dim3(blocks_for(n + l, 256)), dim3(256), 0, st, ra, rb, rc, ptr<Fr>(sl.zmont), sa, bound ? (Fr*)nullptr : sc,
                  (Fr*)d_scalars, n, l, m);
        event_record(sl.ev[1], st);

        const typename P::Lay ly(ctx, pk);
        ly.reserve(sl);
        P::start_z_lanes(ctx, sl, pk, ly);

        Stream wn = ctx->serial ? st : ctx_ntt_stream(ctx);
        stream_wait_event(wn, sl.ev[1]);
        ctx->ws = wn;
        event_record(sl.ntt_b, wn);
        if (bound) {
            ntt_kind_a<C>(ctx, pl, sa, true, ptr<Fr>(pl->s_coset), 1, 0);
            ntt_kind_b<C>(ctx, pl, sa, false, nullptr, 1, 0);
            ZK_LAUNCH((k_sap_quotient<typename Fr::Params>), dim3(blocks_for(D, 256)), dim3(256), 0, wn, sa, fe_from_mont(pl->zinv), sa, D);
        } else {
            ntt_kind_a<C>(ctx, pl, sa, true, ptr<Fr>(pl->s_coset), 1, 0);
            ntt_kind_a<C>(ctx, pl, sc, true, ptr<Fr>(pl->s_cexit), 1, 0, 1);
            ntt_kind_b<C>(ctx, pl, sa, false, nullptr, 1, 0);
            ZK_LAUNCH((k_sap_quotient<typename Fr::Params>), dim3(blocks_for(D, 256)), dim3(256), 0, wn, sa, pl->zinv_rp, sa, D);
            ntt_kind_a<C>(ctx, pl, sa, true, ptr<Fr>(pl->s_cosetinv_canon), 1, 0, 1, sc);
        }
        ctx->ws = ctx->stream;
        event_record(sl.ntt_e, wn);

        P::lanes_after_h(ctx, sl, pk, ly, bound, false, ptr<u32>(sl.va), wn);
    }

    static void finish(zkhip_ctx* ctx, ProofSlot& sl, const zkhip_pk* pk, uint8_t* out, zkhip_timings* tm) {
        require(pk->world == 1, ZKHIP_ERR_BAD_ARG, "this proving key is one shard of a multi-GPU key: use zkhip_prove_gm17_partial + zkhip_combine_gm17");
        const typename P::Sums g = P::collect(ctx, sl, pk);
        const auto t_fin = std::chrono::steady_clock::now();
        Fr rho;
        memcpy(rho.v, sl.r, 32);
        if (P::unsatisfied(ctx, sl, typename P::Lay(ctx, pk))) memset(out, 0, P::PROOF_BYTES);
        else assemble(pk, g, rho, out);
        P::fill_timings(sl, tm, t_fin);
    }
    static void assemble(const zkhip_pk* pk, const typename P::Sums& g, const Fr& rho, uint8_t* out) {
        const Fr rho2 = fe_from_mont(fe_sqr(fe_to_mont(rho)));
        uint8_t dec[2 * FQB];
        decode_point<FQB, 2>(pk->g_gamma2_z2_canon.data(), dec);
        Aff<Fq> z2;
        memcpy(&z2, dec, sizeof(z2));
        z2 = L::to_mont_point(z2);
        Xyzz<Fq> t1, t2;
        {
            HostThreads th;
            th.run([&] { t1 = xyzz_mul_limbs(g.b1, rho.v, Fr::N); });
            t2 = xyzz_mul_limbs(Xyzz<Fq>::from_affine(z2), rho2.v, Fr::N);
        }
        Xyzz<Fq> gC = xyzz_add(g.l, t1);
        gC = xyzz_add(gC, t2);
        gC = xyzz_add(gC, g.h);
        P::write_proof(g.a.is_inf(), xyzz_to_affine(g.a), g.b2.is_inf(), xyzz_to_affine(g.b2), gC.is_inf(), xyzz_to_affine(gC), out);
    }
    static void prove_partial(zkhip_ctx* ctx, const zkhip_pk* pk, const zkhip_r1cs* cs, const uint8_t* z_host, const void* z_dev, const uint8_t* rnd,
                              uint8_t* partial_out, zkhip_timings* tm) {
        check_d2(rnd);
// ... 171 lines not shown
```

### zokrates_amd/csrc/group.cuh

```cuda
#pragma once
#include "core.cuh"
#include "bind.cuh"

namespace zk {

template <class FS>
void points_to_packed(zkhip_ctx* ctx, const Aff<FS>* d_in, void* d_out, u64 n) {
    typedef typename Unsat<FS>::type U;
    ZK_LAUNCH((k_points_to_packed<FS, U>), dim3(blocks_for(n, 256)), dim3(256), 0, ctx->stream, d_in, (AffPacked<U>*)d_out, n);
}

template <class FS>
void msm_table_levels(zkhip_ctx* ctx, void* d_table, u64 count, int c, int W) {
    typedef typename Unsat<FS>::type F;
    if (W <= 1 || count == 0) return;
    const u64 chunk = std::min<u64>(count, std::max<u64>(1024, ((u64)768 << 20) / ((u64)(W - 1) * (sizeof(Xyzz<F>) + sizeof(F)))));
    DBuf tmp, pre;
    tmp.ensure((u64)(W - 1) * chunk * sizeof(Xyzz<F>));
    pre.ensure((u64)(W - 1) * chunk * sizeof(F));
    for (u64 i0 = 0; i0 < count; i0 += chunk) {
        const u64 cnt = std::min(chunk, count - i0);
        ZK_LAUNCH((k_msm_table_levels<F, FS>), dim3(blocks_for(cnt, 256)), dim3(256), 0, ctx->stream, (AffPacked<F>*)d_table, count, i0, cnt, c, W,
                  ptr<Xyzz<F>>(tmp), ptr<F>(pre));
    }
    stream_sync(ctx->stream);
}

template <class FS>
void msm_run_tables(zkhip_ctx* ctx, MsmLane& lane, const MsmSort& so, const void* const* d_tables, int nt, const MsmShape& sh, Xyzz<FS>* d_window_sums,
                    u32 sum_stride, Event ev_begin, Event ev_end, Event accum_after, Xyzz<FS>* h_window_sums) {
    typedef typename Unsat<FS>::type F;
    require(nt >= 1 && nt <= MSM_MAX_TABLES, ZKHIP_ERR_BAD_ARG, "internal: number of tables of one MSM launch");
    MsmTables tables{};
    for (int t = 0; t < nt; ++t) tables.p[t] = d_tables[t];
    Stream s = ctx->serial ? ctx->stream : lane_stream(lane);
    stream_wait_event(s, so.ready);
    const int single = MsmTuning<F>::IS_EXT ? (ctx->msm_g2_waves ? ctx->msm_g2_waves : MsmTuning<F>::SLICE_WPE)
                                            : (ctx->msm_g1_waves ? ctx->msm_g1_waves : MsmTuning<F>::SLICE_WPE);
    const int wpe = ctx->msm_waves ? ctx->msm_waves : (nt > 1 ? std::max(1, (ctx->msm_fused_waves ? ctx->msm_fused_waves : MsmTuning<F>::FUSED_WPE)) : single);
    const u64 machine = ctx->msm_lanes ? (u64)ctx->msm_lanes : (u64)ctx->cus * 4 * 64 * wpe / (nt > 1 && !ctx->msm_waves ? nt : 1);
    const u32 nlanes = (u32)std::max<u64>(1, std::min<u64>(machine, (sh.n * (u64)sh.W + ctx->msm_min_slice - 1) / ctx->msm_min_slice));
    const MsmCut cut{nlanes, ctx->msm_min_slice, (u32)std::min<u64>(sh.n * (u64)sh.levels, 0x7fffffffu)};
    const u64 partial_stride = (u64)sh.nkeys + nlanes;
    lane.heavy.ensure(((size_t)sh.nkeys + 1) * 4);
    lane.lane_key.ensure((size_t)nlanes * 4);
    lane.partial.ensure((size_t)nt * partial_stride * sizeof(Xyzz<F>));
    lane.bucket.ensure((size_t)nt * sh.nkeys * sizeof(Xyzz<F>));
    lane.rows.ensure((size_t)nt * sh.sets * sh.H * sizeof(Xyzz<F>));
    lane.cols.ensure((size_t)nt * sh.sets * sh.Lw * sizeof(Xyzz<F>));
    lds_opt_in(ctx, (const void*)k_msm_fold_rows<F>);
    lds_opt_in(ctx, (const void*)k_msm_fold_cols<F>);
    lds_opt_in(ctx, (const void*)k_msm_fold_final<F, FS>);
    lds_opt_in(ctx, (const void*)k_msm_fold_final_scan<F, FS>);
    const unsigned T = 256;
    ZK_LAUNCH(k_msm_lane_keys, dim3(blocks_for(nlanes, T)), dim3(T), 0, s, ptr<u32>(so.off), sh.nkeys, cut, ptr<u32>(lane.lane_key), ptr<u32>(lane.heavy));
    ZK_LAUNCH(k_msm_find_heavy, dim3(blocks_for(sh.nkeys, T)), dim3(T), 0, s, ptr<u32>(so.off), sh.nkeys, cut, ptr<u32>(lane.heavy) + 1,
              ptr<u32>(lane.heavy));
    if (accum_after && !ctx->serial) stream_wait_event(s, accum_after);
    if (ev_begin) event_record(ev_begin, s);
    const size_t acc_lds = msm_accum_lds_bytes<F>();
    if (ctx->skip_inf_mode == 1 || (ctx->skip_inf_mode == 0 && sh.skip_inf)) {
        if (acc_lds > 64 * 1024) lds_opt_in(ctx, (const void*)k_msm_accum<F, MsmTuning<F>::ACCUM_WPE, true>);
        ZK_LAUNCH((k_msm_accum<F, MsmTuning<F>::ACCUM_WPE, true>), dim3(blocks_for(nlanes, T), nt), dim3(T), acc_lds, s, tables, ptr<u32>(so.off), ptr<u32>(so.sorted),
                  ptr<u32>(lane.lane_key), ptr<Xyzz<F>>(lane.partial), partial_stride, sh.nkeys, cut);
    } else {
        if (acc_lds > 64 * 1024) lds_opt_in(ctx, (const void*)k_msm_accum<F, MsmTuning<F>::ACCUM_WPE, false>);
        ZK_LAUNCH((k_msm_accum<F, MsmTuning<F>::ACCUM_WPE, false>), dim3(blocks_for(nlanes, T), nt), dim3(T), acc_lds, s, tables, ptr<u32>(so.off), ptr<u32>(so.sorted),
                  ptr<u32>(lane.lane_key), ptr<Xyzz<F>>(lane.partial), partial_stride, sh.nkeys, cut);
    }
    if (ev_end) event_record(ev_end, s);
    if (ctx->heavy_runs) {
        lds_opt_in(ctx, (const void*)k_msm_heavy_reduce<F>);
        const unsigned TH = MSM_HEAVY_THREADS;
        ZK_LAUNCH((k_msm_heavy_reduce<F>), dim3(MSM_HEAVY_CHUNKS, nt), dim3(TH), (size_t)TH * sizeof(Xyzz<F>), s, ptr<Xyzz<F>>(lane.partial), partial_stride,
                  ptr<u32>(so.off), sh.nkeys, cut, ptr<u32>(lane.heavy) + 1, ptr<u32>(lane.heavy));
    }
    FoldDigits digs{};
    ZK_LAUNCH((k_msm_fold_rows<F>), dim3(sh.H, sh.sets, nt), dim3(sh.Lw), (size_t)sh.Lw * sizeof(Xyzz<F>), s, ptr<Xyzz<F>>(lane.partial), partial_stride,
              ptr<u32>(so.off), sh.nkeys, cut, sh.K, sh.Lw, ptr<u32>(lane.heavy) + 1, ptr<u32>(lane.heavy), ctx->heavy_runs ? 1u : 0u, ptr<Xyzz<F>>(lane.bucket),
              ptr<Xyzz<F>>(lane.rows));
    const u32 RG = sh.H;
    const u32 HG = std::max<u32>(1, std::min<u32>((u32)ctx->fold_hg, RG)), CW = std::min<u32>(sh.Lw, 256 / HG), NG = sh.H / RG;
    ZK_LAUNCH((k_msm_fold_cols<F>), dim3(sh.Lw / CW, sh.sets * NG, nt), dim3(CW, HG), (size_t)CW * HG * sizeof(Xyzz<F>), s, ptr<Xyzz<F>>(lane.bucket), (u64)sh.K,
              (u64)sh.nkeys, sh.Lw, sh.H, RG, ptr<Xyzz<F>>(lane.cols));
    digs.d[0] = FoldDigit{lane.cols.p, sh.Lw, 1, 0};
    digs.d[1] = FoldDigit{lane.rows.p, sh.H, 0, (u32)ilog2_floor(sh.Lw)};
    u32 longest = 0;
    for (u32 d = 0; d < sh.ndig; ++d) longest = std::max(longest, digs.d[d].len);
    const unsigned TS = std::max<u32>(64, longest);
    if (ctx->fold_scan && TS <= 256) {
        ZK_LAUNCH((k_msm_fold_final_scan<F, FS>), dim3(sh.sets, nt, sh.ndig), dim3(TS), TS * sizeof(Xyzz<F>), s, digs, d_window_sums, sum_stride);
    } else {
        const unsigned TF = std::max<u32>(64, sh.Lw);
        ZK_LAUNCH((k_msm_fold_final<F, FS>), dim3(sh.sets, nt), dim3(TF), TF * sizeof(Xyzz<F>), s, ptr<Xyzz<F>>(lane.rows), ptr<Xyzz<F>>(lane.cols), sh.Lw,
                  sh.H, d_window_sums, sum_stride);
    }
    if (h_window_sums)
        for (int t = 0; t < nt; ++t)
            dev_d2h_pinned(h_window_sums + (size_t)t * sum_stride, d_window_sums + (size_t)t * sum_stride, (size_t)sh.nsums() * sizeof(Xyzz<FS>), s);
    event_record(lane.done, s);
}
template <class FS>
u64 count_infinite(zkhip_ctx* ctx, const void* d_table, u64 count) {
    typedef typename Unsat<FS>::type F;
    if (!count) return 0;
    DBuf d;
    d.ensure(4);
    dev_memset(d.p, 0, 4, ctx->stream);
    ZK_LAUNCH((k_count_infinite<F>), dim3(blocks_for(count, 256)), dim3(256), 0, ctx->stream, (const AffPacked<F>*)d_table, count, ptr<u32>(d));
    u32 n = 0;
    dev_d2h(&n, d.p, 4, ctx->stream);
    stream_sync(ctx->stream);
    return n;
}
template <class FS>
void mark_finite(zkhip_ctx* ctx, const void* d_table, u64 count, u32* d_bitmap) {
    typedef typename Unsat<FS>::type F;
    ZK_LAUNCH((k_mark_finite<F>), dim3(blocks_for(count, 256)), dim3(256), 0, ctx->stream, (const AffPacked<F>*)d_table, count, d_bitmap);
}
template <class FS>
void msm_run(zkhip_ctx* ctx, MsmLane& lane, const MsmSort& so, const void* d_table, const MsmShape& sh, Xyzz<FS>* d_window_sums,
             Event ev_begin, Event ev_end, Event accum_after, Xyzz<FS>* h_window_sums) {
    msm_run_tables<FS>(ctx, lane, so, &d_table, 1, sh, d_window_sums, 0, ev_begin, ev_end, accum_after, h_window_sums);
}

template <class F>
void fixed_base_table(zkhip_ctx* ctx, const Aff<F>* h_pj, int nwin, DBuf& tbl) {
    DBuf d_pj;
    d_pj.ensure((size_t)nwin * sizeof(Aff<F>));
    dev_h2d(d_pj.p, h_pj, (size_t)nwin * sizeof(Aff<F>), ctx->stream);
    tbl.ensure((size_t)nwin * 256 * sizeof(Aff<F>));
    ZK_LAUNCH((k_fixed_base_table<F>), dim3(blocks_for(nwin * 256, 64)), dim3(64), 0, ctx->stream, ptr<Aff<F>>(d_pj), ptr<Aff<F>>(tbl), nwin);
    stream_sync(ctx->stream);
}
template <class F>
void fixed_base_mul(zkhip_ctx* ctx, const DBuf& tbl, int nwin, const u32* d_scalars, u64 count, Aff<F>* d_out) {
    ZK_LAUNCH((k_fixed_base_mul<F>), dim3(blocks_for(count, 64)), dim3(64), 0, ctx->stream, d_scalars, count, ptr<Aff<F>>(tbl), nwin, d_out);
}

template <class FS>
size_t bind_xyzz_bytes() { return sizeof(Xyzz<typename Unsat<FS>::type>); }
template <class FS>
void bind_scale(zkhip_ctx* ctx, const void* d_h_table, u64 N, u64 n_src, u32 n1, u32 n2, u32 n3, const u32* d_scal, const u32* d_konst, int nw, void* d_x) {
    typedef typename Unsat<FS>::type F;
    ZK_LAUNCH((k_bind_scale<F>), dim3(blocks_for(N, 256), 2), dim3(256), 0, ctx->stream, (const AffPacked<F>*)d_h_table, N, n_src, n1, n2, n3, d_scal, d_konst, nw,
              (Xyzz<F>*)d_x);
}
template <class FS>
void bind_fft(zkhip_ctx* ctx, void* d_x, u64 N, const u32* d_tw, int nw) {
    typedef typename Unsat<FS>::type F;
    for (u64 q = N / 2; q >= 1; q >>= 1)
        ZK_LAUNCH((k_bind_fft_stage<F>), dim3(blocks_for(N / 2, 256), 2), dim3(256), 0, ctx->stream, (Xyzz<F>*)d_x, N, q, d_tw, nw);
}
template <class FS>
void bind_h_finish(zkhip_ctx* ctx, const void* d_x, u64 N, int logN, void* d_out) {
    typedef typename Unsat<FS>::type F;
    ZK_LAUNCH((k_bind_h_finish<F>), dim3(blocks_for(N, 256)), dim3(256), 0, ctx->stream, (const Xyzz<F>*)d_x, N, logN, (AffPacked<F>*)d_out);
}
template <class FS>
void bind_cmul(zkhip_ctx* ctx, const void* d_x, int logN, const u32* d_row, const u32* d_val, int nw, const u32* d_minus_one, u64 nnz, void* d_prod) {
    typedef typename Unsat<FS>::type F;
    ZK_LAUNCH((k_bind_cmul<F>), dim3(blocks_for(nnz, 256)), dim3(256), 0, ctx->stream, (const Xyzz<F>*)d_x, logN, d_row, d_val, nw, d_minus_one, nnz, (Xyzz<F>*)d_prod);
}
template <class FS>
void bind_l_finish(zkhip_ctx* ctx, const void* d_prod, const u64* d_cptr, const void* d_l_table, u64 m, const u32* d_long_cols, u64 n_long, void* d_sum, void* d_out) {
    typedef typename Unsat<FS>::type F;
    ZK_LAUNCH((k_bind_l_sum_short<F>), dim3(blocks_for(m, 256)), dim3(256), 0, ctx->stream, (const Xyzz<F>*)d_prod, d_cptr, (const AffPacked<F>*)d_l_table, m, (Xyzz<F>*)d_sum);
    if (n_long)
        ZK_LAUNCH((k_bind_l_sum_long<F>), dim3((unsigned)n_long), dim3(64), 0, ctx->stream, (const Xyzz<F>*)d_prod, d_cptr, (const AffPacked<F>*)d_l_table, d_long_cols, (Xyzz<F>*)d_sum);
    ZK_LAUNCH((k_bind_l_affine<F>), dim3(blocks_for(m, 256)), dim3(256), 0, ctx->stream, (const Xyzz<F>*)d_sum, m, (AffPacked<F>*)d_out);
}
#define ZK_INSTANTIATE_BIND(F)                                                                                          \
    template size_t bind_xyzz_bytes<F>();                                                                               \
    template void bind_scale<F>(zkhip_ctx*, const void*, u64, u64, u32, u32, u32, const u32*, const u32*, int, void*);  \
    template void bind_fft<F>(zkhip_ctx*, void*, u64, const u32*, int);                                                 \
    template void bind_h_finish<F>(zkhip_ctx*, const void*, u64, int, void*);                                           \
    template void bind_cmul<F>(zkhip_ctx*, const void*, int, const u32*, const u32*, int, const u32*, u64, void*);      \
    template void bind_l_finish<F>(zkhip_ctx*, const void*, const u64*, const void*, u64, const u32*, u64, void*, void*);

#define ZK_INSTANTIATE_GROUP(F)                                                                                         \
    template void msm_run<F>(zkhip_ctx*, MsmLane&, const MsmSort&, const void*, const MsmShape&, Xyzz<F>*, Event, Event, Event, Xyzz<F>*);   \
    template void msm_run_tables<F>(zkhip_ctx*, MsmLane&, const MsmSort&, const void* const*, int, const MsmShape&, Xyzz<F>*, u32, Event, Event, Event, Xyzz<F>*); \
    template void points_to_packed<F>(zkhip_ctx*, const Aff<F>*, void*, u64);                    \
    template void msm_table_levels<F>(zkhip_ctx*, void*, u64, int, int);                         \
    template u64 count_infinite<F>(zkhip_ctx*, const void*, u64);                                \
    template void mark_finite<F>(zkhip_ctx*, const void*, u64, u32*);                            \
    template void fixed_base_table<F>(zkhip_ctx*, const Aff<F>*, int, DBuf&);                                           \
    template void fixed_base_mul<F>(zkhip_ctx*, const DBuf&, int, const u32*, u64, Aff<F>*);

}
```

### zokrates_amd/csrc/kernels_msm.cuh

```cuda
#pragma once
#include "devrt.h"
#include "ec.cuh"

namespace zk {

#ifndef ZK_G2_ACCUM_WPE
#define ZK_G2_ACCUM_WPE 2
#endif
#ifndef ZK_G1_FUSED_WPE
#define ZK_G1_FUSED_WPE 6
#endif
#ifndef ZK_G1_SLICE_WPE
#define ZK_G1_SLICE_WPE 4
#endif
#ifndef ZK_G2_SLICE_WPE
#define ZK_G2_SLICE_WPE 4
#endif
#ifndef ZK_G2_COLD_WPE
#define ZK_G2_COLD_WPE 2
#endif
#ifndef ZK_G2_PREFETCH_REGS
#define ZK_G2_PREFETCH_REGS 1
#endif
#ifndef ZK_G2_ZZ_LDS
// ... 61 lines not shown
template <class F>
ZK_HD Aff<F> aff_unpack(const u32* w) {
    return {FuUnpack<F>::get(w), FuUnpack<F>::get(w + PackedWords<F>::N)};
}
template <class F>
ZK_HD void aff_pack(const Aff<F>& p, AffPacked<F>* out) {
    fu_pack(p.x, out->w);
    fu_pack(p.y, out->w + PackedWords<F>::N);
}
template <class F>
__device__ __forceinline__ void aff_load_words(const AffPacked<F>* __restrict__ tbl, u64 idx, u32* w) {
    const uint4* src = (const uint4*)(tbl + idx);
    ZK_UNROLL for (int q = 0; q < AffPacked<F>::NW / 2; ++q) {
        const uint4 t = src[q];
        w[4 * q] = t.x; w[4 * q + 1] = t.y; w[4 * q + 2] = t.z; w[4 * q + 3] = t.w;
    }
}
template <class FS, class U>
__global__ void k_points_to_packed(const Aff<FS>* __restrict__ in, AffPacked<U>* __restrict__ out, u64 n) {
    u64 i = (u64)blockIdx.x * blockDim.x + threadIdx.x;
    if (i >= n) return;
    Aff<FS> p = in[i];
    Aff<U> q = Aff<U>::inf();
    if (!p.is_inf()) { q.x = fu_from_fe(p.x); q.y = fu_from_fe(p.y); }
    aff_pack(q, out + i);
}

static constexpr u32 MSM_NO_DIGIT = 0xffffffffu;
#ifndef ZK_SORT_THREADS
#define ZK_SORT_THREADS 512
#endif
static constexpr u32 MSM_HEAVY = 16;

struct MsmZero { u32* p[3]; u32 n[3]; };
static __device__ __forceinline__ void msm_zero(const MsmZero& z) {
    const u64 g = (u64)blockIdx.x * blockDim.x + threadIdx.x, stride = (u64)gridDim.x * blockDim.x;
    ZK_UNROLL for (int k = 0; k < 3; ++k)
        if (z.p[k]) for (u64 i = g; i < z.n[k]; i += stride) z.p[k][i] = 0;
}
static __global__ void k_msm_zero(MsmZero z) { ZK_PRIO_HIGH(); msm_zero(z); }
static __global__ void k_msm_digits(const u32* __restrict__ scalars, u64 n, int c, int W, u32* __restrict__ dig, MsmZero zero) {
    ZK_PRIO_HIGH();
    msm_zero(zero);
    const u64 i = (u64)blockIdx.x * blockDim.x + threadIdx.x;
    if (i >= n) return;
    const u32* __restrict__ sw = scalars + i * 8;
    const u32 K = 1u << (c - 1), full = 1u << c;
    u32 carry = 0;
    for (int j = 0; j < W; ++j) {
        const int bit = j * c;
        u32 raw = 0;
        if (bit < 256) {
            const int limb = bit >> 5, offb = bit & 31;
            u64 two = sw[limb];
            if (offb + c > 32 && limb + 1 < 8) two |= (u64)sw[limb + 1] << 32;
            raw = (u32)(two >> offb) & (full - 1);
        }
        raw += carry;
        u32 d;
        if (raw > K) {
            const u32 mag = full - raw;
            d = mag ? ((mag - 1) | 0x80000000u) : MSM_NO_DIGIT;
            carry = 1;
        } else {
            d = raw ? raw - 1 : MSM_NO_DIGIT;
            carry = 0;
        }
        dig[(u64)j * n + i] = d;
    }
}
static __device__ __forceinline__ bool msm_skipped(const u32* __restrict__ keep, u64 i) { return keep && !((keep[i >> 5] >> (i & 31)) & 1u); }
static constexpr int MSM_SORT_ILP = 4;
static __global__ void __launch_bounds__(ZK_SORT_THREADS) k_msm_count(const u32* __restrict__ dig, u64 n, int c, int W, u64 chunk, u32 sets, u32 kh,
                                                        u32* __restrict__ cnt, const u32* __restrict__ keep) {
    ZK_PRIO_HIGH();
    ZK_DYN_SMEM(smem);
    u32* hist = (u32*)smem;
    const u32 K = 1u << (c - 1);
    const int j = blockIdx.y;
// ... 317 lines not shown
    if (threadIdx.x == 0) carry = 0;
    __syncthreads();
    for (u32 b = 0; b < nchunks; b += SCAN_THREADS) {
        u32 i = b + threadIdx.x;
        u32 x = i < nchunks ? chunk_sum[i] : 0;
        sh[threadIdx.x] = x;
        __syncthreads();
        for (int d = 1; d < SCAN_THREADS; d <<= 1) {
            u32 t = threadIdx.x >= (unsigned)d ? sh[threadIdx.x - d] : 0;
            __syncthreads();
            sh[threadIdx.x] += t;
            __syncthreads();
        }
        if (i < nchunks) chunk_sum[i] = carry + sh[threadIdx.x] - x;
        __syncthreads();
        if (threadIdx.x == SCAN_THREADS - 1) carry += sh[threadIdx.x];
        __syncthreads();
    }
    if (threadIdx.x == 0) *grand_total = carry;
}
static __global__ void k_scan_add(u32* __restrict__ off, const u32* __restrict__ chunk_sum, u64 total, const u32* __restrict__ grand_total) {
    ZK_PRIO_HIGH();
    u64 i = (u64)blockIdx.x * blockDim.x + threadIdx.x;
    if (i < total) off[i] += chunk_sum[i / SCAN_CHUNK];
    if (i == total) off[total] = *grand_total;
}

struct MsmCut { u32 nlanes, min_slice; u32 table_len; };
static __device__ __forceinline__ u32 msm_slice_len(const u32* __restrict__ off, u32 nkeys, MsmCut cut) {
    const u32 total = off[nkeys];
    const u32 P = (total + cut.nlanes - 1) / cut.nlanes;
    return P > cut.min_slice ? P : cut.min_slice;
}
static __global__ void k_msm_lane_keys(const u32* __restrict__ off, u32 nkeys, MsmCut cut, u32* __restrict__ lane_key, u32* __restrict__ heavy_count) {
    ZK_PRIO_HIGH();
    const u32 g = blockIdx.x * blockDim.x + threadIdx.x;
    if (g == 0) *heavy_count = 0;
    if (g >= cut.nlanes) return;
    const u32 P = msm_slice_len(off, nkeys, cut);
    const u64 pos = (u64)g * P;
    if (pos >= off[nkeys]) { lane_key[g] = nkeys; return; }
    u32 lo = 0, hi = nkeys;
    while (hi - lo > 1) {
        const u32 mid = lo + ((hi - lo) >> 1);
        if (off[mid] <= pos) lo = mid; else hi = mid;
    }
    lane_key[g] = lo;
}
static __global__ void k_msm_find_heavy(const u32* __restrict__ off, u32 nkeys, MsmCut cut, u32* __restrict__ heavy_list,
                                        u32* __restrict__ heavy_count) {
    ZK_PRIO_HIGH();
    const u32 k = blockIdx.x * blockDim.x + threadIdx.x;
    if (k >= nkeys) return;
    const u32 P = msm_slice_len(off, nkeys, cut);
    const u32 b = off[k], e = off[k + 1];
    if (e > b && (e - 1) / P - b / P + 1 > MSM_HEAVY) heavy_list[atomicAdd(heavy_count, 1u)] = k;
}

#if defined(__HIP_DEVICE_COMPILE__)
template <class T>
__device__ __forceinline__ void zk_pin_words(T& obj) {
    u32* w = (u32*)&obj;
    ZK_UNROLL for (unsigned i = 0; i < sizeof(T) / 4; ++i) asm volatile("" : "+v"(w[i]));
}
#define ZK_PIN_WORDS(x) zk_pin_words(x)
#define ZK_LDS_REREAD() asm volatile("" ::: "memory")
#define ZK_OPAQUE(x) asm volatile("" : "+v"(x))
#else
#define ZK_PIN_WORDS(x) ((void)0)
#define ZK_LDS_REREAD() ((void)0)
#define ZK_OPAQUE(x) ((void)0)
#endif
#ifndef ZK_ACCUM_FENCE
#define ZK_ACCUM_FENCE 0
#endif
#ifndef ZK_ACCUM_X_UNREDUCED
#define ZK_ACCUM_X_UNREDUCED 0
#endif
#if defined(__HIP_DEVICE_COMPILE__)
#define ZK_SCHED_FENCE(on) do { if (on) __builtin_amdgcn_sched_barrier(0); } while (0)
#else
#define ZK_SCHED_FENCE(on) ((void)0)
#endif
template <class F, int WPE, bool SKIP_INF>
__global__ void __launch_bounds__(256, WPE) k_msm_accum(MsmTables tables, const u32* __restrict__ off, const u32* __restrict__ sorted,
                                                    const u32* __restrict__ lane_key, Xyzz<F>* __restrict__ partial, u64 partial_stride, u32 nkeys, MsmCut cut) {
    constexpr int NW2 = 2 * AffPacked<F>::NW;
    const AffPacked<F>* __restrict__ bases = (const AffPacked<F>*)tables.p[blockIdx.y];
    partial += (u64)blockIdx.y * partial_stride;
// ... 410 lines not shown
```

### zokrates_amd/csrc/zkhip_api.hip

```cpp
#include "core.cuh"
#include "ingest.h"
#ifndef ZK_EMU
#include <dlfcn.h>
#include <rccl/rccl.h>
#endif

static const CurveOps* ops_for(int curve) {
    if (curve == ZKHIP_CURVE_BN128) return curve_ops_bn254();
    if (curve == ZKHIP_CURVE_BLS12_381) return curve_ops_bls381();
    if (curve == ZKHIP_CURVE_BLS12_377) return curve_ops_bls377();
    throw ApiError{ZKHIP_ERR_BAD_ARG, "unknown curve id"};
}
static thread_local std::string g_create_err;

static void release_slots(zkhip_ctx* ctx) {
    if (ctx->queue) return;
    bool any = false;
    for (auto& sl : ctx->slots) any = any || sl.busy;
    if (!any) return;
    dev_sync_all();
    for (auto& sl : ctx->slots) sl.busy = false;
}
static const char* const SPLIT_PENDING_MSG =
    "a split proof is pending in this context (zkhip_prove_g16_split_begin): finish it with zkhip_prove_g16_split_end or drop it with "
// ... 622 lines not shown
        ops_for(r1cs->curve)->r1cs_check(ctx, r1cs, z, z ? nullptr : z_resident->scalars.p, v);
        if (first_row) *first_row = v[0];
        if (n_bad) *n_bad = v[1];
        if (v[1]) {
            char msg[160];
            snprintf(msg, sizeof(msg), "constraint %llu of %llu is not satisfied (%llu in all)", (unsigned long long)v[0], (unsigned long long)r1cs->n,
                     (unsigned long long)v[1]);
            throw ApiError{ZKHIP_ERR_UNSATISFIED, msg};
        }
    });
}
int32_t zkhip_ctx_set_checked(zkhip_ctx* ctx, int32_t on) {
    if (!ctx) return ZKHIP_ERR_BAD_ARG;
    const int32_t was = ctx->checked ? 1 : 0;
    if (on >= 0 && split_pending(ctx)) {
        ctx->err = SPLIT_PENDING_MSG;
        return ZKHIP_ERR_BAD_ARG;
    }
    if (on >= 0 && ctx->queue) {
        ctx->err = QUEUE_OPEN_MSG;
        return ZKHIP_ERR_BAD_ARG;
    }
    if (on >= 0) ctx->checked = on != 0;
    return was;
}
int32_t zkhip_ctx_unsatisfied(const zkhip_ctx* ctx, uint32_t cap, uint32_t* proof_idx, uint64_t* first_row, uint64_t* n_bad, uint32_t* count) {
    if (!ctx) return ZKHIP_ERR_BAD_ARG;
    for (size_t k = 0; k < ctx->unsat.size() && k < cap; ++k) {
        if (proof_idx) proof_idx[k] = ctx->unsat[k].proof;
        if (first_row) first_row[k] = ctx->unsat[k].first_row;
        if (n_bad) n_bad[k] = ctx->unsat[k].n_bad;
    }
    if (count) *count = (uint32_t)ctx->unsat.size();
    return ZKHIP_OK;
}

int32_t zkhip_queue_open(zkhip_ctx* ctx, const zkhip_pk* pk, const zkhip_r1cs* r1cs, zkhip_queue** out) {
    if (!ctx) return ZKHIP_ERR_BAD_ARG;
    return guarded(ctx, [&] {
        require(pk && r1cs && out, ZKHIP_ERR_BAD_ARG, "null argument");
        *out = nullptr;
        require(pk->ctx == ctx && r1cs->ctx == ctx, ZKHIP_ERR_BAD_ARG, "key / constraint system belong to another context");
        require(pk->world == 1, ZKHIP_ERR_BAD_ARG, "this proving key is one shard of a multi-GPU key: a proof queue takes a whole key");
        for (auto& sl : ctx->slots) require(!sl.busy, ZKHIP_ERR_BAD_ARG, "a proof is in flight in this context");
        ops_for(pk->curve)->queue_check(pk, r1cs);
        std::unique_ptr<zkhip_queue> q(new zkhip_queue());
        q->ctx = ctx;
        q->pk = pk;
        q->cs = r1cs;
        q->cap = (u32)std::max(1, std::min(ctx->nslots, ZK_NSLOTS));
        q->checked = ctx->checked;
        ctx->queue = q.get();
        *out = q.release();
    });
}
int32_t zkhip_queue_state(const zkhip_queue* q, uint32_t* capacity, uint32_t* in_flight) {
    if (!q) return ZKHIP_ERR_BAD_ARG;
    if (capacity) *capacity = q->cap;
    if (in_flight) *in_flight = (uint32_t)(q->next - q->head);
    return ZKHIP_OK;
}
int32_t zkhip_queue_submit(zkhip_queue* q, const uint8_t* z, zkhip_assignment* z_resident, const uint8_t* rnd, uint64_t* ticket) {
    return queue_submit(q, z, z_resident, nullptr, 0, false, rnd, ticket);
}
int32_t zkhip_queue_submit_packed(zkhip_queue* q, const uint8_t* packed, size_t len, const uint8_t* rnd, uint64_t* ticket) {
    return queue_submit(q, nullptr, nullptr, packed, len, true, rnd, ticket);
// ... 658 lines not shown
```

### zokrates_amd/native.py

```python
import ctypes as C
import os

import numpy as np

HERE = os.path.dirname(os.path.abspath(__file__))
DEFAULT_LIB = os.environ.get("ZKHIP_LIBRARY") or os.path.join(HERE, "libzkhip.so")

CURVE_IDS = {"bn128": 0, "bls12_381": 1, "bls12_377": 2}
FQ_BYTES = {0: 32, 1: 48, 2: 48}

ERR_NAMES = {0: "OK", -1: "BAD_ARG", -2: "PARSE", -3: "NOMEM", -4: "DEVICE", -5: "UNSATISFIED", -6: "BUSY"}


class ZkhipError(RuntimeError):

    def __init__(self, code, msg):
        super().__init__(f"zkhip error {code} ({ERR_NAMES.get(code, '?')}): {msg}")
        self.code = code
        self.unsatisfied = []
        self.proofs = None


class Timings(C.Structure):
    _fields_ = [(n, C.c_float) for n in (
# ... 4 lines not shown
        return {n: float(getattr(self, n)) for n, _ in self._fields_ if n != "reserved"}


def _ptr(a):
    return a.ctypes.data_as(C.c_void_p)


def _u8(buf, n=None):
    a = np.frombuffer(buf, dtype=np.uint8) if not isinstance(buf, np.ndarray) else np.ascontiguousarray(buf, dtype=np.uint8)
    if n is not None and a.size != n:
        raise ValueError(f"buffer has {a.size} bytes, expected {n}")
    return a


class Library:

    SYMBOLS = [
        "zkhip_device_count", "zkhip_device_pci_bus_id", "zkhip_ctx_create", "zkhip_ctx_free", "zkhip_last_error", "zkhip_pk_load_g16",
        "zkhip_pk_free", "zkhip_pk_dims", "zkhip_r1cs_load", "zkhip_r1cs_free", "zkhip_prove_g16",
        "zkhip_prove_g16_batch", "zkhip_assignment_upload", "zkhip_assignment_free", "zkhip_prove_g16_resident", "zkhip_prove_g16_resident_batch",
        "zkhip_pk_load_g16_shard", "zkhip_partial_size", "zkhip_prove_g16_partial", "zkhip_combine_g16", "zkhip_ntt", "zkhip_witness_map", "zkhip_msm_g1", "zkhip_msm_g2",
        "zkhip_field_op", "zkhip_setup_g16_size", "zkhip_setup_g16", "zkhip_describe",
        "zkhip_pk_load_gm17", "zkhip_prove_gm17", "zkhip_prove_gm17_resident", "zkhip_prove_gm17_resident_batch",
        "zkhip_setup_gm17_size", "zkhip_setup_gm17", "zkhip_pk_load_gm17_shard", "zkhip_prove_gm17_partial", "zkhip_combine_gm17",
        "zkhip_prog_parse", "zkhip_prog_free", "zkhip_prog_dims", "zkhip_prog_matrix", "zkhip_prog_variable_order",
        "zkhip_prog_r1cs_load", "zkhip_prog_assignment", "zkhip_prog_write_bound", "zkhip_prog_write",
        "zkhip_pk_export_size", "zkhip_pk_export", "zkhip_pk_import",
        "zkhip_pk_bind_r1cs", "zkhip_pk_unbind", "zkhip_pk_is_bound", "zkhip_pk_bind_r1cs_shard", "zkhip_r1cs_fingerprint",
        "zkhip_ctx_tune", "zkhip_init", "zkhip_ctx_clock_probe", "zkhip_multi_bind", "zkhip_multi_unbind",
        "zkhip_multi_transform_split", "zkhip_multi_last_split", "zkhip_prove_g16_split_begin", "zkhip_prove_g16_split_end", "zkhip_prove_g16_split_abort",
        "zkhip_ctx_create_multi", "zkhip_multi_free", "zkhip_multi_size", "zkhip_multi_ctx", "zkhip_multi_last_error", "zkhip_multi_r1cs_load",
        "zkhip_multi_pk_load_g16", "zkhip_multi_pk_load_gm17", "zkhip_prove_g16_multi", "zkhip_prove_gm17_multi",
        "zkhip_multi_pk_load_g16_replicas", "zkhip_prove_g16_multi_batch", "zkhip_multi_use_rccl", "zkhip_multi_exchange",
        "zkhip_r1cs_check", "zkhip_ctx_set_checked", "zkhip_ctx_unsatisfied",
        "zkhip_assignment_pack_bound", "zkhip_assignment_pack", "zkhip_assignment_unpack", "zkhip_prog_assignment_packed",
        "zkhip_assignment_upload_packed",
        "zkhip_queue_open", "zkhip_queue_state", "zkhip_queue_submit", "zkhip_queue_submit_packed", "zkhip_queue_ready", "zkhip_queue_collect",
        "zkhip_queue_close",
    ]

    def __init__(self, path=None):
        self.path = path or DEFAULT_LIB
        if not os.path.exists(self.path):
            raise ZkhipError(-4, f"{self.path} not found: build it with `python -m zokrates_amd.build` "
                                 "(libzkhip has no CPU fallback)")
        L = C.CDLL(self.path)
        vp, u64, u32, i32, sz = C.c_void_p, C.c_uint64, C.c_uint32, C.c_int32, C.c_size_t
        pp = C.POINTER(C.c_void_p)
        L.zkhip_device_count.restype = i32
        L.zkhip_device_pci_bus_id.restype = i32; L.zkhip_device_pci_bus_id.argtypes = [i32, C.c_char_p, sz]
        L.zkhip_ctx_create.restype = i32; L.zkhip_ctx_create.argtypes = [i32, pp]
        L.zkhip_ctx_free.restype = None; L.zkhip_ctx_free.argtypes = [vp]
        L.zkhip_ctx_tune.restype = i32; L.zkhip_ctx_tune.argtypes = [vp, i32, i32]
        L.zkhip_ctx_create_multi.restype = i32; L.zkhip_ctx_create_multi.argtypes = [vp, i32, pp]
        L.zkhip_multi_free.restype = None; L.zkhip_multi_free.argtypes = [vp]
        L.zkhip_multi_size.restype = i32; L.zkhip_multi_size.argtypes = [vp]
        L.zkhip_multi_ctx.restype = vp; L.zkhip_multi_ctx.argtypes = [vp, i32]
        L.zkhip_multi_last_error.restype = C.c_char_p; L.zkhip_multi_last_error.argtypes = [vp]
        L.zkhip_multi_use_rccl.restype = i32; L.zkhip_multi_use_rccl.argtypes = [vp, i32]
        L.zkhip_multi_exchange.restype = C.c_char_p; L.zkhip_multi_exchange.argtypes = [vp]
        L.zkhip_multi_r1cs_load.restype = i32; L.zkhip_multi_r1cs_load.argtypes = [vp, i32, u64, u64, u64] + [vp] * 9
        L.zkhip_multi_pk_load_g16.restype = i32; L.zkhip_multi_pk_load_g16.argtypes = [vp, i32, vp, sz]
        L.zkhip_multi_pk_load_gm17.restype = i32; L.zkhip_multi_pk_load_gm17.argtypes = [vp, i32, vp, sz]
        L.zkhip_prove_g16_multi.restype = i32; L.zkhip_prove_g16_multi.argtypes = [vp] * 6
        L.zkhip_prove_gm17_multi.restype = i32; L.zkhip_prove_gm17_multi.argtypes = [vp] * 5
        L.zkhip_multi_pk_load_g16_replicas.restype = i32; L.zkhip_multi_pk_load_g16_replicas.argtypes = [vp, i32, vp, sz]
        L.zkhip_prove_g16_multi_batch.restype = i32; L.zkhip_prove_g16_multi_batch.argtypes = [vp, u32, vp, vp, vp, vp]
# ... 29 lines not shown
        L.zkhip_prove_gm17_partial.restype = i32; L.zkhip_prove_gm17_partial.argtypes = [vp] * 8
        L.zkhip_combine_gm17.restype = i32; L.zkhip_combine_gm17.argtypes = [vp, vp, u32, vp, vp, vp]
        L.zkhip_setup_gm17_size.restype = i32; L.zkhip_setup_gm17_size.argtypes = [vp, vp]
        L.zkhip_setup_gm17.restype = i32; L.zkhip_setup_gm17.argtypes = [vp, vp, vp, vp, vp, vp, u64]
        L.zkhip_pk_export_size.restype = i32; L.zkhip_pk_export_size.argtypes = [vp, vp]
        L.zkhip_pk_export.restype = i32; L.zkhip_pk_export.argtypes = [vp, vp, u64]
        L.zkhip_pk_import.restype = i32; L.zkhip_pk_import.argtypes = [vp, vp, sz, pp]
        L.zkhip_pk_bind_r1cs.restype = i32; L.zkhip_pk_bind_r1cs.argtypes = [vp, vp, vp]
        L.zkhip_pk_unbind.restype = i32; L.zkhip_pk_unbind.argtypes = [vp]
        L.zkhip_pk_is_bound.restype = i32; L.zkhip_pk_is_bound.argtypes = [vp, vp]
        L.zkhip_pk_bind_r1cs_shard.restype = i32; L.zkhip_pk_bind_r1cs_shard.argtypes = [vp, vp, vp, vp, sz]
        L.zkhip_r1cs_fingerprint.restype = i32; L.zkhip_r1cs_fingerprint.argtypes = [vp, vp, vp]
        L.zkhip_init.restype = i32; L.zkhip_init.argtypes = [i32]
        L.zkhip_ctx_clock_probe.restype = i32; L.zkhip_ctx_clock_probe.argtypes = [vp, u32, vp]
        L.zkhip_multi_bind.restype = i32; L.zkhip_multi_bind.argtypes = [vp, vp, sz]
        L.zkhip_multi_unbind.restype = i32; L.zkhip_multi_unbind.argtypes = [vp]
        L.zkhip_multi_transform_split.restype = i32; L.zkhip_multi_transform_split.argtypes = [vp, i32]
        L.zkhip_multi_last_split.restype = i32; L.zkhip_multi_last_split.argtypes = [vp]
        L.zkhip_prove_g16_split_begin.restype = i32; L.zkhip_prove_g16_split_begin.argtypes = [vp, vp, vp, vp, vp, vp, vp, i32, vp]
        L.zkhip_prove_g16_split_end.restype = i32; L.zkhip_prove_g16_split_end.argtypes = [vp, vp, vp, vp, vp, vp]
        L.zkhip_prove_g16_split_abort.restype = i32; L.zkhip_prove_g16_split_abort.argtypes = [vp]
        L.zkhip_prog_parse.restype = i32; L.zkhip_prog_parse.argtypes = [vp, sz, pp]
        L.zkhip_prog_free.restype = None; L.zkhip_prog_free.argtypes = [vp]
        L.zkhip_prog_dims.restype = i32; L.zkhip_prog_dims.argtypes = [vp, vp]
        L.zkhip_prog_matrix.restype = i32; L.zkhip_prog_matrix.argtypes = [vp, i32, pp, pp, pp]
        L.zkhip_prog_variable_order.restype = i32; L.zkhip_prog_variable_order.argtypes = [vp, pp]
        L.zkhip_prog_r1cs_load.restype = i32; L.zkhip_prog_r1cs_load.argtypes = [vp, vp, pp]
        L.zkhip_prog_write_bound.restype = i32; L.zkhip_prog_write_bound.argtypes = [u64, u64, u64, vp]
        L.zkhip_prog_write.restype = i32; L.zkhip_prog_write.argtypes = [i32, u64, u64] + [vp] * 9 + [vp, vp, vp, u64, u32, vp, u64, vp]
        L.zkhip_prog_assignment.restype = i32; L.zkhip_prog_assignment.argtypes = [vp, vp, sz, vp, vp, u64, vp]
        L.zkhip_r1cs_check.restype = i32; L.zkhip_r1cs_check.argtypes = [vp] * 6
        L.zkhip_ctx_set_checked.restype = i32; L.zkhip_ctx_set_checked.argtypes = [vp, i32]
        L.zkhip_ctx_unsatisfied.restype = i32; L.zkhip_ctx_unsatisfied.argtypes = [vp, u32, vp, vp, vp, vp]
        L.zkhip_assignment_pack_bound.restype = i32; L.zkhip_assignment_pack_bound.argtypes = [u64, vp]
        L.zkhip_assignment_pack.restype = i32; L.zkhip_assignment_pack.argtypes = [vp, u64, vp, u64, vp]
        L.zkhip_assignment_unpack.restype = i32; L.zkhip_assignment_unpack.argtypes = [vp, sz, vp, u64, vp]
        L.zkhip_prog_assignment_packed.restype = i32; L.zkhip_prog_assignment_packed.argtypes = [vp, vp, sz, vp, u64, vp, vp, u64, vp]
        L.zkhip_assignment_upload_packed.restype = i32; L.zkhip_assignment_upload_packed.argtypes = [vp, vp, vp, sz, pp]
        L.zkhip_queue_open.restype = i32; L.zkhip_queue_open.argtypes = [vp, vp, vp, pp]
        L.zkhip_queue_state.restype = i32; L.zkhip_queue_state.argtypes = [vp, vp, vp]
        L.zkhip_queue_submit.restype = i32; L.zkhip_queue_submit.argtypes = [vp, vp, vp, vp, vp]
        L.zkhip_queue_submit_packed.restype = i32; L.zkhip_queue_submit_packed.argtypes = [vp, vp, sz, vp, vp]
        L.zkhip_queue_ready.restype = i32; L.zkhip_queue_ready.argtypes = [vp, vp]
        L.zkhip_queue_collect.restype = i32; L.zkhip_queue_collect.argtypes = [vp, vp, vp, vp]
        L.zkhip_queue_close.restype = i32; L.zkhip_queue_close.argtypes = [vp]
        self.L = L

    def init(self, hw_queues):
        rc = self.L.zkhip_init(int(hw_queues))
        if rc != 0:
            raise ZkhipError(rc, self.L.zkhip_last_error(None).decode(errors="replace"))

    def device_count(self):
        return int(self.L.zkhip_device_count())

    def device_pci_bus_id(self, device):
        buf = C.create_string_buffer(32)
        if self.L.zkhip_device_pci_bus_id(int(device), buf, 32) != 0:
            return None
        return buf.value.decode().lower() or None


_default = None


def default_library():
# ... 3 lines not shown
    return _default


class Context:

    def __init__(self, device=0, library=None):
        self.lib = library or default_library()
        self.h = C.c_void_p()
        rc = self.lib.L.zkhip_ctx_create(device, C.byref(self.h))
        if rc != 0:
            raise ZkhipError(rc, self.lib.L.zkhip_last_error(None).decode())

    def _check(self, rc, proofs=None):
        if rc != 0:
            e = ZkhipError(rc, self.lib.L.zkhip_last_error(self.h).decode())
            if rc == -5:
                e.unsatisfied = self.unsatisfied()
                e.proofs = proofs() if proofs else None
            raise e

    def set_checked(self, on=True):
        was = self.lib.L.zkhip_ctx_set_checked(self.h, -1 if on is None else int(bool(on)))
        if was < 0:
            self._check(was)
        return bool(was)

    def unsatisfied(self):
        count = C.c_uint32()
        self.lib.L.zkhip_ctx_unsatisfied(self.h, 0, None, None, None, C.byref(count))
        k = count.value
        idx, row, bad = np.zeros(max(k, 1), dtype=np.uint32), np.zeros(max(k, 1), dtype=np.uint64), np.zeros(max(k, 1), dtype=np.uint64)
        self.lib.L.zkhip_ctx_unsatisfied(self.h, k, _ptr(idx), _ptr(row), _ptr(bad), C.byref(count))
        return [(int(idx[i]), int(row[i]), int(bad[i])) for i in range(k)]

    def describe(self):
        buf = C.create_string_buffer(256)
        self._check(self.lib.L.zkhip_describe(self.h, buf, 256))
        return buf.value.decode()

    TUNABLES = {"msm_c": 1, "msm_waves": 2, "msm_lanes": 3, "msm_min_slice": 4, "fold_scan": 5, "serial": 6, "ntt_single_max_log": 7, "ntt_cols": 8, "slots": 9, "z_gate": 10, "fuse_z": 11, "msm_fused_waves": 12, "stream_jitter": 13, "ntt_max_sublog": 16, "msm_sets": 17, "skip_inf": 18, "b_sort": 19, "heavy_runs": 20, "fold_hg": 25, "ntt_fuse_first": 26, "pipe_plan": 28}

    def clock_probe(self, duration_us=2000):
        out = C.c_double()
        self._check(self.lib.L.zkhip_ctx_clock_probe(self.h, int(duration_us), C.byref(out)))
        return out.value

    def tune(self, name, value):
        self._check(self.lib.L.zkhip_ctx_tune(self.h, self.TUNABLES[name], int(value)))

    def close(self):
        if self.h:
            self.lib.L.zkhip_ctx_free(self.h)
            self.h = C.c_void_p()

    def __del__(self):
        try:
            self.close()
        except Exception:
            pass

    def ntt(self, curve_id, data, direction):
        d = np.array(_u8(data), dtype=np.uint8, copy=True)
        n = d.size // 32
        logn = n.bit_length() - 1
        if n == 0 or (1 << logn) != n:
            raise ValueError("NTT size must be a power of two")
# ... 682 lines not shown
```

Baseline: 110.0.

## Fuse MSM slicing into sort prep, read resident z in place, skip idle heavy passes

Lane-key slicing and heavy-bucket detection are merged into one k_msm_slices kernel launched inside msm_prepare, and the lane heavy counters are zeroed inside the digits kernel. Resident assignments are read in place, with r and s placed in a small tail buffer, so the per-proof device-to-device copy of z goes away. Per-lane heavy counts are reported back so later proofs can skip the heavy pass when none were seen. A dispatch-count API is added to expose kernel and copy counts. The intent is fewer kernel launches and copies per proof, at the cost of extra bookkeeping and a heuristic that relies on earlier proofs having similar heavy-bucket patterns.

```diff
diff --git a/include/zkhip.h b/include/zkhip.h
--- a/include/zkhip.h
+++ b/include/zkhip.h
@@ -111,6 +111,7 @@
 int32_t zkhip_ctx_set_checked(zkhip_ctx* ctx, int32_t on);
 int32_t zkhip_ctx_unsatisfied(const zkhip_ctx* ctx, uint32_t cap, uint32_t* proof_idx, uint64_t* first_row,
                               uint64_t* n_bad, uint32_t* count);
+int32_t zkhip_ctx_dispatch_count(const zkhip_ctx* ctx, uint32_t cap, uint64_t* out);
 
 typedef struct zkhip_queue zkhip_queue;
 int32_t zkhip_queue_open(zkhip_ctx* ctx, const zkhip_pk* pk, const zkhip_r1cs* r1cs, zkhip_queue** out);
diff --git a/integration/zokrates_hip/src/ffi.rs b/integration/zokrates_hip/src/ffi.rs
--- a/integration/zokrates_hip/src/ffi.rs
+++ b/integration/zokrates_hip/src/ffi.rs
@@ -62,6 +62,7 @@
     pub fn zkhip_ctx_set_checked(ctx: *mut zkhip_ctx, on: i32) -> i32;
     pub fn zkhip_ctx_unsatisfied(ctx: *const zkhip_ctx, cap: u32, proof_idx: *mut u32, first_row: *mut u64, n_bad: *mut u64,
         count: *mut u32) -> i32;
+    pub fn zkhip_ctx_dispatch_count(ctx: *const zkhip_ctx, cap: u32, out: *mut u64) -> i32;
     pub fn zkhip_queue_open(ctx: *mut zkhip_ctx, pk: *const zkhip_pk, r1cs: *const zkhip_r1cs, out: *mut *mut zkhip_queue) -> i32;
     pub fn zkhip_queue_state(q: *const zkhip_queue, capacity: *mut u32, in_flight: *mut u32) -> i32;
     pub fn zkhip_queue_submit(q: *mut zkhip_queue, z: *const u8, z_resident: *mut zkhip_assignment, rnd: *const u8, ticket: *mut u64) -> i32;
diff --git a/zokrates_amd/csrc/core.cuh b/zokrates_amd/csrc/core.cuh
--- a/zokrates_amd/csrc/core.cuh
+++ b/zokrates_amd/csrc/core.cuh
@@ -105,10 +105,13 @@
     DBuf lane_key, heavy, partial, bucket, rows, cols;
     Event done = nullptr;
 };
+struct ZkDispatch { u64 kernels = 0, copies = 0, heavy_launches = 0; };
 static constexpr int ZK_NLANES = 5;
 static constexpr int ZK_NSLOTS = 4;
 struct ProofSlot {
     DBuf scalars, zmont, va, vb, vc, ws1, ws2, zflag;
+    DBuf tail;
+    const u32 *z_src = nullptr, *z_tail = nullptr;
     DBuf verdict;
     int check_idx = -1;
     MsmSort sorts[3];
@@ -123,6 +126,8 @@
     int half = -1;
     bool lone = false;
     bool split_pending = false;
+    u32 sliced_lanes = 0;
+    ZkDispatch disp;
     const zkhip_pk* split_pk = nullptr;
     const zkhip_r1cs* split_cs = nullptr;
     bool split_bound = false;
@@ -187,6 +192,9 @@
     bool checked = false;
     struct Unsatisfied { u32 proof; u64 first_row, n_bad; };
     std::vector<Unsatisfied> unsat;
+    ZkDispatch enq, last_dispatch;
+    DispatchCount enq_mark;
+    u32 last_heavy[ZK_NLANES] = {};
     std::string err;
     std::string desc;
     ProofSlot slots[ZK_NSLOTS];
@@ -570,8 +578,25 @@
     ZK_LAUNCH(k_scan_chunks, dim3(1), dim3(SCAN_THREADS), 0, s, ptr<u32>(chunk_sum), nchunks, ptr<u32>(grand));
     ZK_LAUNCH(k_scan_add, dim3(blocks_for(nk + 1, 256)), dim3(256), 0, s, ptr<u32>(off), ptr<u32>(chunk_sum), nk, ptr<u32>(grand));
 }
-static inline void msm_prepare(zkhip_ctx* ctx, Stream s, MsmSort& so, const u32* d_scalars, const MsmShape& sh, u64 level_stride,
-                               const u32* keep = nullptr, const MsmSort* wm_of = nullptr) {
+template <class FS>
+static inline MsmCut msm_cut(const zkhip_ctx* ctx, const MsmShape& sh, int nt) {
+    typedef typename Unsat<FS>::type F;
+    const int single = MsmTuning<F>::IS_EXT ? (ctx->msm_g2_waves ? ctx->msm_g2_waves : MsmTuning<F>::SLICE_WPE)
+                                            : (ctx->msm_g1_waves ? ctx->msm_g1_waves : MsmTuning<F>::SLICE_WPE);
+    const int wpe = ctx->msm_waves ? ctx->msm_waves : (nt > 1 ? std::max(1, (ctx->msm_fused_waves ? ctx->msm_fused_waves : MsmTuning<F>::FUSED_WPE)) : single);
+    const u64 machine = ctx->msm_lanes ? (u64)ctx->msm_lanes : (u64)ctx->cus * 4 * 64 * wpe / (nt > 1 && !ctx->msm_waves ? nt : 1);
+    const u32 nlanes = (u32)std::max<u64>(1, std::min<u64>(machine, (sh.n * (u64)sh.W + ctx->msm_min_slice - 1) / ctx->msm_min_slice));
+    return MsmCut{nlanes, ctx->msm_min_slice, (u32)std::min<u64>(sh.n * (u64)sh.levels, 0x7fffffffu)};
+}
+struct MsmUse {
+    MsmLane* lane;
+    MsmCut cut;
+    u32* report;
+    u32 report_shift;
+};
+static inline void msm_prepare(zkhip_ctx* ctx, Stream s, MsmSort& so, const u32* d_scalars, const MsmShape& sh, u64 level_stride, const MsmUse* uses, int nuses,
+                               const u32* keep = nullptr, const MsmSort* wm_of = nullptr, const u32* d_tail = nullptr, u64 n_head = 0) {
+    require(nuses >= 0 && nuses <= MSM_MAX_USES, ZKHIP_ERR_BAD_ARG, "internal: lanes over one sorted list");
     const u64 nk = sh.nkeys;
     require(sh.n * (u64)sh.W < ((u64)1 << 32) - sh.nkeys, ZKHIP_ERR_BAD_ARG, "MSM too large for 32-bit sort offsets");
     require(level_stride * (u64)sh.levels < ((u64)1 << 31) && sh.n < ((u64)1 << 31), ZKHIP_ERR_BAD_ARG, "MSM too large for 31-bit table indices");
@@ -592,8 +617,15 @@
         so.ccur.ensure((size_t)nbins * 4);
         so.tile_off.ensure(((size_t)nbins + 1) * 4);
     }
-    const MsmZero zero{{ptr<u32>(so.cnt), ptr<u32>(so.cursor), two_level ? ptr<u32>(so.ccur) : nullptr}, {(u32)nk, (u32)nk, two_level ? nbins : 0u}};
-    if (!wm_of) ZK_LAUNCH(k_msm_digits, dim3(blocks_for(sh.n, T)), dim3(T), 0, s, d_scalars, sh.n, sh.c, sh.W, ptr<u32>(so.dig), zero);
+    MsmZero zero{{ptr<u32>(so.cnt), ptr<u32>(so.cursor), two_level ? ptr<u32>(so.ccur) : nullptr}, {(u32)nk, (u32)nk, two_level ? nbins : 0u}};
+    for (int u = 0; u < nuses; ++u) {
+        MsmLane& lane = *uses[u].lane;
+        lane.heavy.ensure(((size_t)nk + 1) * 4);
+        lane.lane_key.ensure((size_t)uses[u].cut.nlanes * 4);
+        zero.p[3 + u] = ptr<u32>(lane.heavy);
+        zero.n[3 + u] = 1;
+    }
+    if (!wm_of) ZK_LAUNCH(k_msm_digits, dim3(blocks_for(sh.n, T)), dim3(T), 0, s, d_scalars, d_tail ? n_head : sh.n, d_tail, sh.n, sh.c, sh.W, ptr<u32>(so.dig), zero);
     else ZK_LAUNCH(k_msm_zero, dim3(blocks_for(nk, T)), dim3(T), 0, s, zero);
     const u32* wm = wm_of ? ptr<u32>(wm_of->dig) : ptr<u32>(so.dig);
     lds_opt_in(ctx, (const void*)k_msm_count);
@@ -607,6 +639,9 @@
         scan_u32(s, so.cnt, so.off, nk, so.chunk_sum, so.grand);
         if (two_level) ZK_LAUNCH(k_msm_tile_offsets, dim3(1), dim3(MSM_TILE_SCAN_THREADS), 0, s, ptr<u32>(so.off), nbins, ptr<u32>(so.tile_off));
     }
+    for (int u = 0; u < nuses; ++u)
+        ZK_LAUNCH(k_msm_slices, dim3(blocks_for(std::max<u64>(uses[u].cut.nlanes, nk), T)), dim3(T), 0, s, ptr<u32>(so.off), (u32)nk, uses[u].cut,
+                  ptr<u32>(uses[u].lane->lane_key), ptr<u32>(uses[u].lane->heavy) + 1, ptr<u32>(uses[u].lane->heavy), uses[u].report, uses[u].report_shift);
     if (two_level) {
         const u64 total_max = sh.n * (u64)sh.W;
         so.pairs.ensure(std::max<u64>(total_max, 1) * 8);
@@ -626,10 +661,10 @@
 
 template <class F>
 void msm_run(zkhip_ctx* ctx, MsmLane& lane, const MsmSort& so, const void* d_table, const MsmShape& sh, Xyzz<F>* d_window_sums,
-             Event ev_begin, Event ev_end, Event accum_after = nullptr, Xyzz<F>* h_window_sums = nullptr);
+             Event ev_begin, Event ev_end, Event accum_after, Xyzz<F>* h_window_sums, bool heavy_pass);
 template <class F>
 void msm_run_tables(zkhip_ctx* ctx, MsmLane& lane, const MsmSort& so, const void* const* d_tables, int nt, const MsmShape& sh, Xyzz<F>* d_window_sums,
-                    u32 sum_stride, Event ev_begin, Event ev_end, Event accum_after, Xyzz<F>* h_window_sums = nullptr);
+                    u32 sum_stride, Event ev_begin, Event ev_end, Event accum_after, Xyzz<F>* h_window_sums, bool heavy_pass, bool one_copy);
 template <class F>
 void points_to_packed(zkhip_ctx* ctx, const Aff<F>* d_in, void* d_out, u64 n);
 template <class F>
@@ -719,6 +754,7 @@
     u64 bound_uid = 0;
     u64 bound_fp[2] = {0, 0};
     bool inf_many_bound[2] = {true, true};
+    mutable int heavy_seen[5] = {-1, -1, -1, -1, -1};
 };
 
 static const char PK_IMAGE_MAGIC[8] = {'Z', 'K', 'H', 'I', 'P', 'P', 'K', '5'};
@@ -805,6 +841,8 @@
     uint8_t* zflag(const ProofSlot& sl) const { return (uint8_t*)sl.h_ws + b1() + b2(); }
     uint8_t* verdict(const ProofSlot& sl) const { return zflag(sl) + 8; }
     u32 zflag_word(const ProofSlot& sl) const { u32 f; memcpy(&f, zflag(sl), 4); return f; }
+    u32 heavy_word(const ProofSlot& sl) const { u32 f; memcpy(&f, zflag(sl) + 4, 4); return f; }
+    static u32* heavy_report(const ProofSlot& sl) { return ptr<u32>(sl.zflag) + 1; }
     void reserve(ProofSlot& sl) const {
         sl.ws1.ensure(b1());
         sl.ws2.ensure(b2());
@@ -1590,8 +1628,8 @@
         require(z0.equals(one), ZKHIP_ERR_BAD_ARG, Z0_NOT_ONE_MSG);
         dst.ensure(cap * 32);
         dev_h2d(dst.p, z, m * 32, ctx->stream);
-        flag.ensure(4);
-        dev_memset(flag.p, 0, 4, ctx->stream);
+        flag.ensure(8);
+        dev_memset(flag.p, 0, 8, ctx->stream);
         ZK_LAUNCH((k_check_canonical<Fr>), dim3(blocks_for(m, 256)), dim3(256), 0, ctx->stream, ptr<Fr>(dst), m, ptr<u32>(flag));
     }
     static void unpack_z(zkhip_ctx* ctx, DBuf& dst, u64 m, u64 cap, const PackedZ& zp, DBuf& flag) {
@@ -1599,8 +1637,8 @@
         dst.ensure(cap * 32);
         ctx->zpack.ensure(zp.len);
         dev_h2d(ctx->zpack.p, zp.bytes, zp.len, s);
-        flag.ensure(4);
-        dev_memset(flag.p, 0, 4, s);
+        flag.ensure(8);
+        dev_memset(flag.p, 0, 8, s);
         const uint8_t* d = ptr<uint8_t>(ctx->zpack);
         ZK_LAUNCH((k_unpack_assignment<Fr>), dim3(blocks_for(m, ZPACK_BLOCK_ELEMS)), dim3(256), 0, s, d + zp.tags_off, (const u64*)(d + zp.index_off),
                   d + zp.payload_off, ptr<Fr>(dst), m, ptr<u32>(flag));
@@ -1620,8 +1658,8 @@
                 sl.scalars.ensure(cap * 32);
                 dev_d2d(sl.scalars.p, z_dev, m * 32, st);
             }
-            sl.zflag.ensure(4);
-            dev_memset(sl.zflag.p, 0, 4, st);
+            sl.zflag.ensure(8);
+            dev_memset(sl.zflag.p, 0, 8, st);
         }
         if (checked) verdict_reset(sl, st);
         return (z_host || !in_place) ? ptr<Fr>(sl.scalars) : (const Fr*)z_dev;
@@ -1629,12 +1667,12 @@
     static void require_canonical(u32 flag) {
         require(flag == 0, ZKHIP_ERR_BAD_ARG, "an assignment entry is not a canonical field element (>= r)");
     }
-    static void stage_scalars(zkhip_ctx* ctx, NttPlan<C>* pl, void* d_scalars, u64 m, const uint8_t* r, const uint8_t* s_) {
+    static void stage_scalars(zkhip_ctx* ctx, NttPlan<C>* pl, const Fr* z, void* d_tail, u64 m, const uint8_t* r, const uint8_t* s_) {
         Stream s = ctx->stream;
         ctx->cur->zmont.ensure(m * 32);
-        dev_h2d((uint8_t*)d_scalars + m * 32, r, 32, s);
-        dev_h2d((uint8_t*)d_scalars + (m + 1) * 32, s_, 32, s);
-        ZK_LAUNCH((k_mul_const<Fr>), dim3(blocks_for(m, 256)), dim3(256), 0, s, (const Fr*)d_scalars, ptr<Fr>(ctx->cur->zmont), m, pl->k_to_rp);
+        dev_h2d(d_tail, r, 32, s);
+        dev_h2d((uint8_t*)d_tail + 32, s_, 32, s);
+        ZK_LAUNCH((k_mul_const<Fr>), dim3(blocks_for(m, 256)), dim3(256), 0, s, z, ptr<Fr>(ctx->cur->zmont), m, pl->k_to_rp);
     }
 
     static void enqueue(zkhip_ctx* ctx, ProofSlot& sl, const zkhip_pk* pk, const zkhip_r1cs* cs, const uint8_t* z_host, const void* z_dev,
@@ -1665,19 +1703,25 @@
         Fr rr = fe_from_bytes_canon<Fr>(r), ss = fe_from_bytes_canon<Fr>(s_);
         require(canon_lt_mod(rr) && canon_lt_mod(ss), ZKHIP_ERR_BAD_ARG, "r or s not a canonical field element");
         NttPlan<C>* pl = open_slot(ctx, sl, pk);
+        sl.disp = ZkDispatch{};
+        count_begin(ctx);
         sl.half = half;
         sl.lone = lone;
         sl.check_idx = half < 0 ? check_idx : -1;
         memcpy(sl.r, r, 32);
         memcpy(sl.s, s_, 32);
         Stream st = ctx->stream;
-        stage_z(ctx, sl, pk->m, pk->m + 2, z_host, z_dev, sl.check_idx >= 0, false, zp);
-        stage_scalars(ctx, pl, sl.scalars.p, pk->m, r, s_);
+        const bool in_place = z_dev && !z_host && !zp && half < 0;
+        const Fr* z = stage_z(ctx, sl, pk->m, pk->m + 2, z_host, z_dev, sl.check_idx >= 0, in_place, zp);
+        if (in_place) sl.tail.ensure(64);
+        sl.z_src = (const u32*)z;
+        sl.z_tail = in_place ? ptr<u32>(sl.tail) : ptr<u32>(sl.scalars) + pk->m * 8;
+        stage_scalars(ctx, pl, z, (void*)sl.z_tail, pk->m, r, s_);
         event_record(sl.ev[0], st);
 
         const Lay ly(ctx, pk);
         ly.reserve(sl);
-        start_z_lanes(ctx, sl, pk, ly);
+        start_z_lanes(ctx, sl, pk, ly, bound);
 
         Stream wn = ctx->serial ? st : slot_ntt_stream(ctx, sl);
         stream_wait_event(wn, sl.ev[0]);
@@ -1692,10 +1736,12 @@
             sl.split_bound = bound;
             sl.split_pending = true;
         }
+        count_end(ctx, sl, false);
     }
     static void enqueue_tail(zkhip_ctx* ctx, ProofSlot& sl, const zkhip_pk* pk, const zkhip_r1cs* cs) {
         const u64 N = pk->N;
         ctx->cur = &sl;
+        count_begin(ctx);
         Stream wn = ctx->serial ? ctx->stream : slot_ntt_stream(ctx, sl);
         const u32* h_scalars = ptr<u32>(sl.va) + (sl.half >= 0 ? 2 * N * 8 : 0);
         if (sl.half >= 0) {
@@ -1703,19 +1749,54 @@
             ZK_LAUNCH((k_quotient<typename Fr::Params>), dim3(blocks_for(N, 256)), dim3(256), 0, wn, a, a + N, fe_from_mont(get_plan<C>(ctx, pk->logN)->zinv), a + 2 * N, N);
         }
         lanes_after_h(ctx, sl, pk, Lay(ctx, pk), sl.half >= 0 ? sl.split_bound : is_bound(pk, cs), sl.lone, h_scalars, wn);
-    }
-
-    static void start_z_lanes(zkhip_ctx* ctx, ProofSlot& sl, const zkhip_pk* pk, const Lay& ly) {
+        count_end(ctx, sl, true);
+    }
+
+    static void start_z_lanes(zkhip_ctx* ctx, ProofSlot& sl, const zkhip_pk* pk, const Lay& ly, bool bound) {
+        sl.sliced_lanes = 0;
         if (!pk->z_n) return;
-        const u32* digits = ptr<u32>(sl.scalars) + pk->z_lo * 8;
-        msm_prepare(ctx, ctx->stream, sl.sorts[0], digits, ly.shz, pk->z_n);
-        if (pk->thin_mask) msm_prepare(ctx, ctx->stream, sl.sorts[2], digits, ly.shz, pk->z_n, ptr<u32>(pk->thin_keep), &sl.sorts[0]);
+        MsmUse uses[2][MSM_MAX_USES];
+        int nu[2] = {0, 0};
+        const int g2_list = (pk->thin_mask & 8) ? 1 : 0;
+        uses[g2_list][nu[g2_list]++] = lane_use<Fq2>(ctx, sl, 3, ly.shz, 1);
+        ZLaunch zl[3];
+        const int nz = z_launches(ctx, pk, bound, zl);
+        for (int q = 0; q < nz; ++q) uses[zl[q].list][nu[zl[q].list]++] = lane_use<Fq>(ctx, sl, zl[q].member[0], ly.shz, zl[q].nm);
+        const u64 n_head = pk->z_lo < pk->m ? std::min<u64>(pk->z_n, pk->m - pk->z_lo) : 0;
+        const u32* head = sl.z_src + pk->z_lo * 8;
+        const u32* tail = n_head < pk->z_n ? sl.z_tail + (pk->z_lo + n_head - pk->m) * 8 : nullptr;
+        msm_prepare(ctx, ctx->stream, sl.sorts[0], head, ly.shz, pk->z_n, uses[0], nu[0], nullptr, nullptr, tail, n_head);
+        if (pk->thin_mask) msm_prepare(ctx, ctx->stream, sl.sorts[2], head, ly.shz, pk->z_n, uses[1], nu[1], ptr<u32>(pk->thin_keep), &sl.sorts[0]);
         if (z_gate(ctx) < 2) run_g2(ctx, sl, pk, ly, nullptr);
+    }
+    template <class FS>
+    static MsmUse lane_use(const zkhip_ctx* ctx, ProofSlot& sl, int k, const MsmShape& sh, int nt) {
+        sl.sliced_lanes |= 1u << k;
+        return MsmUse{&sl.lanes[k], msm_cut<FS>(ctx, sh, nt), Lay::heavy_report(sl), (u32)k * MSM_HEAVY_REPORT_BITS};
+    }
+    static bool heavy_pass(const zkhip_ctx* ctx, const zkhip_pk* pk, int k) { return ctx->heavy_runs && pk->heavy_seen[k] != 0; }
+    static void note_heavy(zkhip_ctx* ctx, const ProofSlot& sl, const zkhip_pk* pk, const Lay& ly) {
+        const u32 w = ly.heavy_word(sl);
+        for (int k = 0; k < ZK_NLANES; ++k) {
+            ctx->last_heavy[k] = (sl.sliced_lanes >> k) & 1u ? (w >> (k * MSM_HEAVY_REPORT_BITS)) & MSM_HEAVY_REPORT_MAX : 0;
+            if ((sl.sliced_lanes >> k) & 1u) pk->heavy_seen[k] = (int)ctx->last_heavy[k];
+        }
+    }
+    static void count_begin(zkhip_ctx* ctx) {
+        ctx->enq_mark = dispatch_count();
+        ctx->enq = ZkDispatch{};
+    }
+    static void count_end(zkhip_ctx* ctx, ProofSlot& sl, bool all_enqueued) {
+        const DispatchCount now = dispatch_count();
+        sl.disp.kernels += now.kernels - ctx->enq_mark.kernels;
+        sl.disp.copies += now.copies - ctx->enq_mark.copies;
+        sl.disp.heavy_launches += ctx->enq.heavy_launches;
+        if (all_enqueued) ctx->last_dispatch = sl.disp;
     }
     static void run_g2(zkhip_ctx* ctx, ProofSlot& sl, const zkhip_pk* pk, const Lay& ly, Event after) {
         const bool thin = pk->thin_mask & 8;
         msm_run<Fq2>(ctx, sl.lanes[3], sl.sorts[thin ? 2 : 0], pk->b2_ext.p, with_inf(ly.shz, thin ? pk->inf_many_thin[3] : pk->inf_many[3]), ly.ws2(sl),
-                     sl.acc_b[4], sl.acc_e[4], after, ly.hs2(sl));
+                     sl.acc_b[4], sl.acc_e[4], after, ly.hs2(sl), heavy_pass(ctx, pk, 3));
     }
     static void lanes_after_h(zkhip_ctx* ctx, ProofSlot& sl, const zkhip_pk* pk, const Lay& ly, bool bound, bool lone, const u32* h_scalars, Stream wn) {
         Stream st = ctx->stream;
@@ -1737,42 +1818,54 @@
             empty_msm(ctx, sl, ly, true);
         }
         if (pk->h_n) {
-            msm_prepare(ctx, wn, sl.sorts[1], h_scalars + pk->h_lo * 8, ly.shh, pk->h_n);
+            const MsmUse use = lane_use<Fq>(ctx, sl, 4, ly.shh, 1);
+            msm_prepare(ctx, wn, sl.sorts[1], h_scalars + pk->h_lo * 8, ly.shh, pk->h_n, &use, 1);
             msm_run<Fq>(ctx, sl.lanes[4], sl.sorts[1], bound ? pk->h_bound.p : pk->h_sigma.p, with_inf(ly.shh, bound ? pk->inf_many_bound[1] : pk->inf_many[4]),
-                        ly.ws1(sl, 3), sl.acc_b[3], sl.acc_e[3], nullptr, ly.hs1(sl, 3));
+                        ly.ws1(sl, 3), sl.acc_b[3], sl.acc_e[3], nullptr, ly.hs1(sl, 3), heavy_pass(ctx, pk, 4));
         } else {
             empty_msm(ctx, sl, ly, false);
         }
         copy_out(ctx, sl, ly);
     }
 
+    struct ZLaunch {
+        int list;
+        int nm, member[3];
+    };
+    static u32 z_thin(const zkhip_pk* pk, bool bound, int k) { return (bound && k == 2) ? 0u : (pk->thin_mask >> k) & 1u; }
+    static int z_launches(const zkhip_ctx* ctx, const zkhip_pk* pk, bool bound, ZLaunch out[3]) {
+        int n = 0;
+        if (!ctx->fuse_z) {
+            for (int k = 0; k < 3; ++k) out[n++] = ZLaunch{(int)z_thin(pk, bound, k), 1, {k, 0, 0}};
+            return n;
+        }
+        for (u32 which = 0; which < 2; ++which) {
+            ZLaunch z{(int)which, 0, {0, 0, 0}};
+            for (int k = 0; k < 3; ++k)
+                if (z_thin(pk, bound, k) == which) z.member[z.nm++] = k;
+            if (z.nm) out[n++] = z;
+        }
+        return n;
+    }
     static void run_z_g1(zkhip_ctx* ctx, ProofSlot& sl, const zkhip_pk* pk, const Lay& ly, Event h_ready, bool bound) {
         const void* tab[3] = {pk->a_ext.p, pk->b1_ext.p, bound ? pk->l_bound.p : pk->l_ext.p};
-        auto thin = [&](int k) { return (bound && k == 2) ? 0u : (pk->thin_mask >> k) & 1u; };
-        auto inf_many = [&](int k) { return (bound && k == 2) ? pk->inf_many_bound[0] : thin(k) ? pk->inf_many_thin[k] : pk->inf_many[k]; };
-        if (!ctx->fuse_z) {
-            for (int k = 0; k < 3; ++k)
-                msm_run<Fq>(ctx, sl.lanes[k], thin(k) ? sl.sorts[2] : sl.sorts[0], tab[k], with_inf(ly.shz, inf_many(k)), ly.ws1(sl, k), sl.acc_b[k], sl.acc_e[k], h_ready,
-                            ly.hs1(sl, k));
-            return;
-        }
-        for (u32 which = 0; which < 2; ++which) {
-            int member[3], nm = 0;
-            for (int k = 0; k < 3; ++k)
-                if (thin(k) == which) member[nm++] = k;
-            if (!nm) continue;
-            const int lead = member[0];
+        auto inf_many = [&](int k) { return (bound && k == 2) ? pk->inf_many_bound[0] : z_thin(pk, bound, k) ? pk->inf_many_thin[k] : pk->inf_many[k]; };
+        ZLaunch zl[3];
+        const int nz = z_launches(ctx, pk, bound, zl);
+        for (int i = 0; i < nz; ++i) {
+            const ZLaunch& z = zl[i];
+            const int lead = z.member[0];
             const void* tabs[3];
             bool many = false;
-            for (int q = 0; q < nm; ++q) { tabs[q] = tab[member[q]]; many = many || inf_many(member[q]); }
-            const int step = nm > 1 ? member[1] - member[0] : 1;
-            msm_run_tables<Fq>(ctx, sl.lanes[lead], which ? sl.sorts[2] : sl.sorts[0], tabs, nm, with_inf(ly.shz, many), ly.ws1(sl, lead), (u32)(step * ly.Wmax),
-                               sl.acc_b[lead], sl.acc_e[lead], h_ready, ly.hs1(sl, lead));
+            for (int q = 0; q < z.nm; ++q) { tabs[q] = tab[z.member[q]]; many = many || inf_many(z.member[q]); }
+            const int step = z.nm > 1 ? z.member[1] - z.member[0] : 1;
+            msm_run_tables<Fq>(ctx, sl.lanes[lead], z.list ? sl.sorts[2] : sl.sorts[0], tabs, z.nm, with_inf(ly.shz, many), ly.ws1(sl, lead), (u32)(step * ly.Wmax),
+                               sl.acc_b[lead], sl.acc_e[lead], h_ready, ly.hs1(sl, lead), heavy_pass(ctx, pk, lead), step == 1);
             Stream s0 = ctx->serial ? ctx->stream : lane_stream(sl.lanes[lead]);
-            for (int q = 1; q < nm; ++q) {
-                event_record(sl.acc_b[member[q]], s0);
-                event_record(sl.acc_e[member[q]], s0);
-                event_record(sl.lanes[member[q]].done, s0);
+            for (int q = 1; q < z.nm; ++q) {
+                event_record(sl.acc_b[z.member[q]], s0);
+                event_record(sl.acc_e[z.member[q]], s0);
+                event_record(sl.lanes[z.member[q]].done, s0);
             }
         }
     }
@@ -1781,8 +1874,8 @@
         Stream st = ctx->stream;
         Stream so = ctx->serial ? st : ctx_out_stream(ctx);
         for (int k = 0; k < ZK_NLANES; ++k) stream_wait_event(so, sl.lanes[k].done);
-        sl.zflag.ensure(4);
-        dev_d2h_pinned(ly.zflag(sl), sl.zflag.p, 4, so);
+        sl.zflag.ensure(8);
+        dev_d2h_pinned(ly.zflag(sl), sl.zflag.p, 8, so);
         if (sl.check_idx >= 0) {
             stream_wait_event(so, sl.ev[2]);
             dev_d2h_pinned(ly.verdict(sl), sl.verdict.p, 16, so);
@@ -1818,6 +1911,7 @@
         sl.busy = false;
         split_clear(sl);
         const Lay ly(ctx, pk);
+        note_heavy(ctx, sl, pk, ly);
         require_canonical(ly.zflag_word(sl));
         Sums g;
         HostThreads th;
@@ -1909,6 +2003,7 @@
             throw;
         }
         sl.busy = false;
+        note_heavy(ctx, sl, pk, ly);
         require_canonical(ly.zflag_word(sl));
         if (unsatisfied(ctx, sl, ly)) memset(out, 0, PROOF_BYTES);
         else assemble_tail(g, sA, rB1, rsD, out);
@@ -2011,6 +2106,7 @@
         const Lay ly(ctx, pk);
         *b1 = ly.b1();
         *b2 = ly.b2();
+        note_heavy(ctx, sl, pk, ly);
         require_canonical(ly.zflag_word(sl));
         *d_ws1 = sl.ws1.p;
         *d_ws2 = sl.ws2.p;
@@ -2132,14 +2228,15 @@
         d_ws.ensure((size_t)sh.nsums() * sizeof(Xyzz<F>));
         DBuf d_packed;
         d_packed.ensure(n * packed_point_bytes<F>());
+        const MsmUse use{&ctx->cur->lanes[0], msm_cut<F>(ctx, sh, 1), nullptr, 0};
 #ifdef ZK_TEST_MSM_RACE
-        msm_prepare(ctx, s, ctx->cur->sorts[0], ptr<u32>(ctx->cur->scalars), sh, 0);
+        msm_prepare(ctx, s, ctx->cur->sorts[0], ptr<u32>(ctx->cur->scalars), sh, 0, &use, 1);
         points_to_packed<F>(ctx, ptr<Aff<F>>(d_bases), d_packed.p, n);
 #else
         points_to_packed<F>(ctx, ptr<Aff<F>>(d_bases), d_packed.p, n);
-        msm_prepare(ctx, s, ctx->cur->sorts[0], ptr<u32>(ctx->cur->scalars), sh, 0);
+        msm_prepare(ctx, s, ctx->cur->sorts[0], ptr<u32>(ctx->cur->scalars), sh, 0, &use, 1);
 #endif
-        msm_run<F>(ctx, ctx->cur->lanes[0], ctx->cur->sorts[0], d_packed.p, sh, ptr<Xyzz<F>>(d_ws), nullptr, nullptr);
+        msm_run<F>(ctx, ctx->cur->lanes[0], ctx->cur->sorts[0], d_packed.p, sh, ptr<Xyzz<F>>(d_ws), nullptr, nullptr, nullptr, nullptr, ctx->heavy_runs);
         stream_wait_event(s, ctx->cur->lanes[0].done);
         std::vector<Xyzz<F>> ws(sh.nsums());
         dev_d2h(ws.data(), d_ws.p, ws.size() * sizeof(Xyzz<F>), s);
@@ -2194,7 +2291,7 @@
         const u64 m = cs->l + cs->w;
         uint8_t zero[32] = {0};
         upload_z(ctx, ctx->cur->scalars, m, m + 2, z, ctx->cur->zflag);
-        stage_scalars(ctx, pl, ctx->cur->scalars.p, m, zero, zero);
+        stage_scalars(ctx, pl, ptr<Fr>(ctx->cur->scalars), ptr<Fr>(ctx->cur->scalars) + m, m, zero, zero);
         witness_map(ctx, cs, pl);
         ctx->cur->vb.ensure(pl->N * sizeof(Fr));
         ZK_LAUNCH((k_sigma_permute<Fr>), dim3(blocks_for(pl->N, 256)), dim3(256), 0, ctx->stream, ptr<Fr>(ctx->cur->va), ptr<Fr>(ctx->cur->vb), pl->N,
diff --git a/zokrates_amd/csrc/devrt.h b/zokrates_amd/csrc/devrt.h
--- a/zokrates_amd/csrc/devrt.h
+++ b/zokrates_amd/csrc/devrt.h
@@ -58,8 +58,14 @@
     th.join();
 }
 
+struct DispatchCount { uint64_t kernels = 0, copies = 0; };
+inline DispatchCount& dispatch_count() {
+    static thread_local DispatchCount c;
+    return c;
+}
+
 #ifndef ZK_EMU
-#define ZK_HIP_CHECK(expr)                                                                        \
+#define ZK_HIP_CHECK(expr)                                                                     \
     do {                                                                                          \
         hipError_t e_ = (expr);                                                                   \
         if (e_ != hipSuccess)                                                                     \
@@ -197,12 +203,13 @@
             r.used[i] = false;
         }
 }
-inline void dev_h2d_pinned(void* d, const void* h, size_t n, Stream s) { jitter_before(s); ZK_HIP_CHECK(hipMemcpyAsync(d, h, n, hipMemcpyHostToDevice, s)); }
-inline void dev_d2h_pinned(void* h, const void* d, size_t n, Stream s) { jitter_before(s); ZK_HIP_CHECK(hipMemcpyAsync(h, d, n, hipMemcpyDeviceToHost, s)); }
+inline void dev_h2d_pinned(void* d, const void* h, size_t n, Stream s) { ++dispatch_count().copies; jitter_before(s); ZK_HIP_CHECK(hipMemcpyAsync(d, h, n, hipMemcpyHostToDevice, s)); }
+inline void dev_d2h_pinned(void* h, const void* d, size_t n, Stream s) { ++dispatch_count().copies; jitter_before(s); ZK_HIP_CHECK(hipMemcpyAsync(h, d, n, hipMemcpyDeviceToHost, s)); }
 inline void dev_h2d(void* d, const void* h, size_t n, Stream s) {
     if (!n) return;
     const int mode = copy_mode();
     if (mode == 0) { dev_h2d_pinned(d, h, n, s); return; }
+    ++dispatch_count().copies;
     if (mode == 1) {
         ZK_HIP_CHECK(hipStreamSynchronize(s));
         ZK_HIP_CHECK(hipMemcpy(d, h, n, hipMemcpyHostToDevice));
@@ -314,6 +321,7 @@
     if (!n) return;
     const int mode = copy_mode();
     if (mode == 0) { dev_d2h_pinned(h, d, n, s); return; }
+    ++dispatch_count().copies;
     if (mode == 1) {
         ZK_HIP_CHECK(hipStreamSynchronize(s));
         ZK_HIP_CHECK(hipMemcpy(h, d, n, hipMemcpyDeviceToHost));
@@ -346,7 +354,7 @@
     drain(q);
     drain(q ^ 1);
 }
-inline void dev_d2d(void* d, const void* s_, size_t n, Stream s) { jitter_before(s); ZK_HIP_CHECK(hipMemcpyAsync(d, s_, n, hipMemcpyDeviceToDevice, s)); }
+inline void dev_d2d(void* d, const void* s_, size_t n, Stream s) { ++dispatch_count().copies; jitter_before(s); ZK_HIP_CHECK(hipMemcpyAsync(d, s_, n, hipMemcpyDeviceToDevice, s)); }
 inline void dev_copy_between(void* d, int dst_dev, const void* s_, int src_dev, size_t n, Stream s) {
     jitter_before(s);
     if (dst_dev == src_dev) ZK_HIP_CHECK(hipMemcpyAsync(d, s_, n, hipMemcpyDeviceToDevice, s));
@@ -415,6 +423,7 @@
         if (!zk::grid_nonempty(dim3(grid))) break;                                        \
         if (zk::trace_enabled()) fprintf(stderr, "[zkhip] launch %s ...", #kernel);       \
         zk::jitter_before(stream);                                                        \
+        ++zk::dispatch_count().kernels;                                                   \
         hipLaunchKernelGGL(kernel, grid, block, smem, stream, __VA_ARGS__);               \
         zk::dev_check_last();                                                             \
         if (zk::trace_enabled()) {                                                        \
@@ -446,18 +455,18 @@
 inline void dev_free(void* p) { free(p); }
 inline void* host_alloc_pinned(size_t bytes) { return dev_alloc(bytes); }
 inline void host_free_pinned(void* p) { free(p); }
-inline void dev_h2d(void* d, const void* h, size_t n, Stream) { memcpy(d, h, n); }
+inline void dev_h2d(void* d, const void* h, size_t n, Stream) { if (n) ++dispatch_count().copies; memcpy(d, h, n); }
 template <class Fill>
 inline void dev_h2d_fill(void* d, size_t n, size_t unit, Stream, Fill&& fill, unsigned = 8) {
     const size_t units = n / unit, cut = units / 3 * unit;
     if (cut) fill((char*)d, (size_t)0, cut);
     if (n > cut) fill((char*)d + cut, cut, n - cut);
 }
-inline void dev_d2h(void* h, const void* d, size_t n, Stream) { memcpy(h, d, n); }
+inline void dev_d2h(void* h, const void* d, size_t n, Stream) { if (n) ++dispatch_count().copies; memcpy(h, d, n); }
 inline void staging_drain() {}
-inline void dev_h2d_pinned(void* d, const void* h, size_t n, Stream) { memcpy(d, h, n); }
-inline void dev_d2h_pinned(void* h, const void* d, size_t n, Stream) { memcpy(h, d, n); }
-inline void dev_d2d(void* d, const void* s_, size_t n, Stream) { memcpy(d, s_, n); }
+inline void dev_h2d_pinned(void* d, const void* h, size_t n, Stream) { ++dispatch_count().copies; memcpy(d, h, n); }
+inline void dev_d2h_pinned(void* h, const void* d, size_t n, Stream) { ++dispatch_count().copies; memcpy(h, d, n); }
+inline void dev_d2d(void* d, const void* s_, size_t n, Stream) { ++dispatch_count().copies; memcpy(d, s_, n); }
 inline void dev_copy_between(void* d, int, const void* s_, int, size_t n, Stream) { memcpy(d, s_, n); }
 inline void dev_memset(void* d, int v, size_t n, Stream) { memset(d, v, n); }
 inline Stream stream_create() { return 0; }
@@ -479,7 +488,7 @@
 inline JitterState& jitter_state() { static JitterState st; return st; }
 
 #define ZK_LAUNCH(kernel, grid, block, smem, stream, ...) \
-    emu::launch(dim3(grid), dim3(block), (size_t)(smem), [&]() { kernel(__VA_ARGS__); })
+    (++zk::dispatch_count().kernels, emu::launch(dim3(grid), dim3(block), (size_t)(smem), [&]() { kernel(__VA_ARGS__); }))
 #define ZK_DYN_SMEM(name) unsigned char* name = emu::dyn_smem()
 #define ZK_PRIO_HIGH() ((void)0)
 #define ZK_WAVE_ANY(pred) (emu::wave_ballot(pred) != 0)
diff --git a/zokrates_amd/csrc/gm17.cuh b/zokrates_amd/csrc/gm17.cuh
--- a/zokrates_amd/csrc/gm17.cuh
+++ b/zokrates_amd/csrc/gm17.cuh
@@ -79,12 +79,16 @@
         const Fr rho = add_mod(dd, rr);
         const bool bound = P::is_bound(pk, cs);
         NttPlan<C>* pl = P::open_slot(ctx, sl, pk);
+        sl.disp = ZkDispatch{};
+        P::count_begin(ctx);
         sl.check_idx = check_idx;
         memcpy(sl.r, rho.v, 32);
         memset(sl.s, 0, 32);
         Stream st = ctx->stream;
         P::stage_z(ctx, sl, m, M + 2, z_host, z_dev, check_idx >= 0, false, zp);
         uint8_t* d_scalars = (uint8_t*)sl.scalars.p;
+        sl.z_src = ptr<u32>(sl.scalars);
+        sl.z_tail = sl.z_src + M * 8;
         sl.zmont.ensure(m * 32);
         dev_h2d(d_scalars + M * 32, sl.r, 32, st);
         dev_memset(d_scalars + (M + 1) * 32, 0, 32, st);
@@ -108,7 +112,7 @@
 
         const typename P::Lay ly(ctx, pk);
         ly.reserve(sl);
-        P::start_z_lanes(ctx, sl, pk, ly);
+        P::start_z_lanes(ctx, sl, pk, ly, bound);
 
         Stream wn = ctx->serial ? st : ctx_ntt_stream(ctx);
         stream_wait_event(wn, sl.ev[1]);
@@ -129,6 +133,7 @@
         event_record(sl.ntt_e, wn);
 
         P::lanes_after_h(ctx, sl, pk, ly, bound, false, ptr<u32>(sl.va), wn);
+        P::count_end(ctx, sl, true);
     }
 
     static void finish(zkhip_ctx* ctx, ProofSlot& sl, const zkhip_pk* pk, uint8_t* out, zkhip_timings* tm) {
diff --git a/zokrates_amd/csrc/group.cuh b/zokrates_amd/csrc/group.cuh
--- a/zokrates_amd/csrc/group.cuh
+++ b/zokrates_amd/csrc/group.cuh
@@ -28,22 +28,17 @@
 
 template <class FS>
 void msm_run_tables(zkhip_ctx* ctx, MsmLane& lane, const MsmSort& so, const void* const* d_tables, int nt, const MsmShape& sh, Xyzz<FS>* d_window_sums,
-                    u32 sum_stride, Event ev_begin, Event ev_end, Event accum_after, Xyzz<FS>* h_window_sums) {
+                    u32 sum_stride, Event ev_begin, Event ev_end, Event accum_after, Xyzz<FS>* h_window_sums, bool heavy_pass, bool one_copy) {
     typedef typename Unsat<FS>::type F;
     require(nt >= 1 && nt <= MSM_MAX_TABLES, ZKHIP_ERR_BAD_ARG, "internal: number of tables of one MSM launch");
     MsmTables tables{};
     for (int t = 0; t < nt; ++t) tables.p[t] = d_tables[t];
     Stream s = ctx->serial ? ctx->stream : lane_stream(lane);
     stream_wait_event(s, so.ready);
-    const int single = MsmTuning<F>::IS_EXT ? (ctx->msm_g2_waves ? ctx->msm_g2_waves : MsmTuning<F>::SLICE_WPE)
-                                            : (ctx->msm_g1_waves ? ctx->msm_g1_waves : MsmTuning<F>::SLICE_WPE);
-    const int wpe = ctx->msm_waves ? ctx->msm_waves : (nt > 1 ? std::max(1, (ctx->msm_fused_waves ? ctx->msm_fused_waves : MsmTuning<F>::FUSED_WPE)) : single);
-    const u64 machine = ctx->msm_lanes ? (u64)ctx->msm_lanes : (u64)ctx->cus * 4 * 64 * wpe / (nt > 1 && !ctx->msm_waves ? nt : 1);
-    const u32 nlanes = (u32)std::max<u64>(1, std::min<u64>(machine, (sh.n * (u64)sh.W + ctx->msm_min_slice - 1) / ctx->msm_min_slice));
-    const MsmCut cut{nlanes, ctx->msm_min_slice, (u32)std::min<u64>(sh.n * (u64)sh.levels, 0x7fffffffu)};
+    const MsmCut cut = msm_cut<FS>(ctx, sh, nt);
+    const u32 nlanes = cut.nlanes;
     const u64 partial_stride = (u64)sh.nkeys + nlanes;
-    lane.heavy.ensure(((size_t)sh.nkeys + 1) * 4);
-    lane.lane_key.ensure((size_t)nlanes * 4);
+    require(lane.heavy.cap >= ((size_t)sh.nkeys + 1) * 4 && lane.lane_key.cap >= (size_t)nlanes * 4, ZKHIP_ERR_DEVICE, "internal: the sort did not slice its list for this lane");
     lane.partial.ensure((size_t)nt * partial_stride * sizeof(Xyzz<F>));
     lane.bucket.ensure((size_t)nt * sh.nkeys * sizeof(Xyzz<F>));
     lane.rows.ensure((size_t)nt * sh.sets * sh.H * sizeof(Xyzz<F>));
@@ -53,9 +48,6 @@
     lds_opt_in(ctx, (const void*)k_msm_fold_final<F, FS>);
     lds_opt_in(ctx, (const void*)k_msm_fold_final_scan<F, FS>);
     const unsigned T = 256;
-    ZK_LAUNCH(k_msm_lane_keys, dim3(blocks_for(nlanes, T)), dim3(T), 0, s, ptr<u32>(so.off), sh.nkeys, cut, ptr<u32>(lane.lane_key), ptr<u32>(lane.heavy));
-    ZK_LAUNCH(k_msm_find_heavy, dim3(blocks_for(sh.nkeys, T)), dim3(T), 0, s, ptr<u32>(so.off), sh.nkeys, cut, ptr<u32>(lane.heavy) + 1,
-              ptr<u32>(lane.heavy));
     if (accum_after && !ctx->serial) stream_wait_event(s, accum_after);
     if (ev_begin) event_record(ev_begin, s);
     const size_t acc_lds = msm_accum_lds_bytes<F>();
@@ -69,7 +61,8 @@
                   ptr<u32>(lane.lane_key), ptr<Xyzz<F>>(lane.partial), partial_stride, sh.nkeys, cut);
     }
     if (ev_end) event_record(ev_end, s);
-    if (ctx->heavy_runs) {
+    if (heavy_pass) {
+        ++ctx->enq.heavy_launches;
         lds_opt_in(ctx, (const void*)k_msm_heavy_reduce<F>);
         const unsigned TH = MSM_HEAVY_THREADS;
         ZK_LAUNCH((k_msm_heavy_reduce<F>), dim3(MSM_HEAVY_CHUNKS, nt), dim3(TH), (size_t)TH * sizeof(Xyzz<F>), s, ptr<Xyzz<F>>(lane.partial), partial_stride,
@@ -77,7 +70,7 @@
     }
     FoldDigits digs{};
     ZK_LAUNCH((k_msm_fold_rows<F>), dim3(sh.H, sh.sets, nt), dim3(sh.Lw), (size_t)sh.Lw * sizeof(Xyzz<F>), s, ptr<Xyzz<F>>(lane.partial), partial_stride,
-              ptr<u32>(so.off), sh.nkeys, cut, sh.K, sh.Lw, ptr<u32>(lane.heavy) + 1, ptr<u32>(lane.heavy), ctx->heavy_runs ? 1u : 0u, ptr<Xyzz<F>>(lane.bucket),
+              ptr<u32>(so.off), sh.nkeys, cut, sh.K, sh.Lw, ptr<u32>(lane.heavy) + 1, ptr<u32>(lane.heavy), heavy_pass ? 1u : 0u, ptr<Xyzz<F>>(lane.bucket),
               ptr<Xyzz<F>>(lane.rows));
     const u32 RG = sh.H;
     const u32 HG = std::max<u32>(1, std::min<u32>((u32)ctx->fold_hg, RG)), CW = std::min<u32>(sh.Lw, 256 / HG), NG = sh.H / RG;
@@ -95,9 +88,13 @@
         ZK_LAUNCH((k_msm_fold_final<F, FS>), dim3(sh.sets, nt), dim3(TF), TF * sizeof(Xyzz<F>), s, ptr<Xyzz<F>>(lane.rows), ptr<Xyzz<F>>(lane.cols), sh.Lw,
                   sh.H, d_window_sums, sum_stride);
     }
-    if (h_window_sums)
-        for (int t = 0; t < nt; ++t)
-            dev_d2h_pinned(h_window_sums + (size_t)t * sum_stride, d_window_sums + (size_t)t * sum_stride, (size_t)sh.nsums() * sizeof(Xyzz<FS>), s);
+    if (h_window_sums) {
+        if (one_copy || nt == 1)
+            dev_d2h_pinned(h_window_sums, d_window_sums, ((size_t)(nt - 1) * sum_stride + sh.nsums()) * sizeof(Xyzz<FS>), s);
+        else
+            for (int t = 0; t < nt; ++t)
+                dev_d2h_pinned(h_window_sums + (size_t)t * sum_stride, d_window_sums + (size_t)t * sum_stride, (size_t)sh.nsums() * sizeof(Xyzz<FS>), s);
+    }
     event_record(lane.done, s);
 }
 template <class FS>
@@ -120,8 +117,8 @@
 }
 template <class FS>
 void msm_run(zkhip_ctx* ctx, MsmLane& lane, const MsmSort& so, const void* d_table, const MsmShape& sh, Xyzz<FS>* d_window_sums,
-             Event ev_begin, Event ev_end, Event accum_after, Xyzz<FS>* h_window_sums) {
-    msm_run_tables<FS>(ctx, lane, so, &d_table, 1, sh, d_window_sums, 0, ev_begin, ev_end, accum_after, h_window_sums);
+             Event ev_begin, Event ev_end, Event accum_after, Xyzz<FS>* h_window_sums, bool heavy_pass) {
+    msm_run_tables<FS>(ctx, lane, so, &d_table, 1, sh, d_window_sums, 0, ev_begin, ev_end, accum_after, h_window_sums, heavy_pass, true);
 }
 
 template <class F>
@@ -179,8 +176,8 @@
     template void bind_l_finish<F>(zkhip_ctx*, const void*, const u64*, const void*, u64, const u32*, u64, void*, void*);
 
 #define ZK_INSTANTIATE_GROUP(F)                                                                                         \
-    template void msm_run<F>(zkhip_ctx*, MsmLane&, const MsmSort&, const void*, const MsmShape&, Xyzz<F>*, Event, Event, Event, Xyzz<F>*);   \
-    template void msm_run_tables<F>(zkhip_ctx*, MsmLane&, const MsmSort&, const void* const*, int, const MsmShape&, Xyzz<F>*, u32, Event, Event, Event, Xyzz<F>*); \
+    template void msm_run<F>(zkhip_ctx*, MsmLane&, const MsmSort&, const void*, const MsmShape&, Xyzz<F>*, Event, Event, Event, Xyzz<F>*, bool);   \
+    template void msm_run_tables<F>(zkhip_ctx*, MsmLane&, const MsmSort&, const void* const*, int, const MsmShape&, Xyzz<F>*, u32, Event, Event, Event, Xyzz<F>*, bool, bool); \
     template void points_to_packed<F>(zkhip_ctx*, const Aff<F>*, void*, u64);                    \
     template void msm_table_levels<F>(zkhip_ctx*, void*, u64, int, int);                         \
     template u64 count_infinite<F>(zkhip_ctx*, const void*, u64);                                \
diff --git a/zokrates_amd/csrc/kernels_msm.cuh b/zokrates_amd/csrc/kernels_msm.cuh
--- a/zokrates_amd/csrc/kernels_msm.cuh
+++ b/zokrates_amd/csrc/kernels_msm.cuh
@@ -117,19 +117,22 @@
 #endif
 static constexpr u32 MSM_HEAVY = 16;
 
-struct MsmZero { u32* p[3]; u32 n[3]; };
+static constexpr int MSM_MAX_USES = 4;
+static constexpr int MSM_ZERO_SLOTS = 3 + MSM_MAX_USES;
+struct MsmZero { u32* p[MSM_ZERO_SLOTS]; u32 n[MSM_ZERO_SLOTS]; };
 static __device__ __forceinline__ void msm_zero(const MsmZero& z) {
     const u64 g = (u64)blockIdx.x * blockDim.x + threadIdx.x, stride = (u64)gridDim.x * blockDim.x;
-    ZK_UNROLL for (int k = 0; k < 3; ++k)
+    ZK_UNROLL for (int k = 0; k < MSM_ZERO_SLOTS; ++k)
         if (z.p[k]) for (u64 i = g; i < z.n[k]; i += stride) z.p[k][i] = 0;
 }
 static __global__ void k_msm_zero(MsmZero z) { ZK_PRIO_HIGH(); msm_zero(z); }
-static __global__ void k_msm_digits(const u32* __restrict__ scalars, u64 n, int c, int W, u32* __restrict__ dig, MsmZero zero) {
+static __global__ void k_msm_digits(const u32* __restrict__ scalars, u64 n_head, const u32* __restrict__ tail, u64 n, int c, int W, u32* __restrict__ dig,
+                                    MsmZero zero) {
     ZK_PRIO_HIGH();
     msm_zero(zero);
     const u64 i = (u64)blockIdx.x * blockDim.x + threadIdx.x;
     if (i >= n) return;
-    const u32* __restrict__ sw = scalars + i * 8;
+    const u32* __restrict__ sw = i < n_head ? scalars + i * 8 : tail + (i - n_head) * 8;
     const u32 K = 1u << (c - 1), full = 1u << c;
     u32 carry = 0;
     for (int j = 0; j < W; ++j) {
@@ -513,12 +516,21 @@
     const u32 P = (total + cut.nlanes - 1) / cut.nlanes;
     return P > cut.min_slice ? P : cut.min_slice;
 }
-static __global__ void k_msm_lane_keys(const u32* __restrict__ off, u32 nkeys, MsmCut cut, u32* __restrict__ lane_key, u32* __restrict__ heavy_count) {
+static constexpr u32 MSM_HEAVY_REPORT_BITS = 6, MSM_HEAVY_REPORT_MAX = (1u << MSM_HEAVY_REPORT_BITS) - 1;
+static __global__ void k_msm_slices(const u32* __restrict__ off, u32 nkeys, MsmCut cut, u32* __restrict__ lane_key, u32* __restrict__ heavy_list,
+                                    u32* __restrict__ heavy_count, u32* __restrict__ report, u32 report_shift) {
     ZK_PRIO_HIGH();
     const u32 g = blockIdx.x * blockDim.x + threadIdx.x;
-    if (g == 0) *heavy_count = 0;
+    const u32 P = msm_slice_len(off, nkeys, cut);
+    if (g < nkeys) {
+        const u32 b = off[g], e = off[g + 1];
+        if (e > b && (e - 1) / P - b / P + 1 > MSM_HEAVY) {
+            const u32 at = atomicAdd(heavy_count, 1u);
+            heavy_list[at] = g;
+            if (report && at < MSM_HEAVY_REPORT_MAX) atomicAdd(report, 1u << report_shift);
+        }
+    }
     if (g >= cut.nlanes) return;
-    const u32 P = msm_slice_len(off, nkeys, cut);
     const u64 pos = (u64)g * P;
     if (pos >= off[nkeys]) { lane_key[g] = nkeys; return; }
     u32 lo = 0, hi = nkeys;
@@ -527,15 +539,6 @@
         if (off[mid] <= pos) lo = mid; else hi = mid;
     }
     lane_key[g] = lo;
-}
-static __global__ void k_msm_find_heavy(const u32* __restrict__ off, u32 nkeys, MsmCut cut, u32* __restrict__ heavy_list,
-                                        u32* __restrict__ heavy_count) {
-    ZK_PRIO_HIGH();
-    const u32 k = blockIdx.x * blockDim.x + threadIdx.x;
-    if (k >= nkeys) return;
-    const u32 P = msm_slice_len(off, nkeys, cut);
-    const u32 b = off[k], e = off[k + 1];
-    if (e > b && (e - 1) / P - b / P + 1 > MSM_HEAVY) heavy_list[atomicAdd(heavy_count, 1u)] = k;
 }
 
 #if defined(__HIP_DEVICE_COMPILE__)
diff --git a/zokrates_amd/csrc/zkhip_api.hip b/zokrates_amd/csrc/zkhip_api.hip
--- a/zokrates_amd/csrc/zkhip_api.hip
+++ b/zokrates_amd/csrc/zkhip_api.hip
@@ -678,6 +678,13 @@
         if (n_bad) n_bad[k] = ctx->unsat[k].n_bad;
     }
     if (count) *count = (uint32_t)ctx->unsat.size();
+    return ZKHIP_OK;
+}
+int32_t zkhip_ctx_dispatch_count(const zkhip_ctx* ctx, uint32_t cap, uint64_t* out) {
+    if (!ctx || (cap && !out)) return ZKHIP_ERR_BAD_ARG;
+    uint64_t v[3 + ZK_NLANES] = {ctx->last_dispatch.kernels, ctx->last_dispatch.copies, ctx->last_dispatch.heavy_launches};
+    for (int k = 0; k < ZK_NLANES; ++k) v[3 + k] = ctx->last_heavy[k];
+    for (uint32_t k = 0; k < cap && k < 3 + ZK_NLANES; ++k) out[k] = v[k];
     return ZKHIP_OK;
 }
 
diff --git a/zokrates_amd/native.py b/zokrates_amd/native.py
--- a/zokrates_amd/native.py
+++ b/zokrates_amd/native.py
@@ -60,7 +60,7 @@
         "zkhip_ctx_create_multi", "zkhip_multi_free", "zkhip_multi_size", "zkhip_multi_ctx", "zkhip_multi_last_error", "zkhip_multi_r1cs_load",
         "zkhip_multi_pk_load_g16", "zkhip_multi_pk_load_gm17", "zkhip_prove_g16_multi", "zkhip_prove_gm17_multi",
         "zkhip_multi_pk_load_g16_replicas", "zkhip_prove_g16_multi_batch", "zkhip_multi_use_rccl", "zkhip_multi_exchange",
-        "zkhip_r1cs_check", "zkhip_ctx_set_checked", "zkhip_ctx_unsatisfied",
+        "zkhip_r1cs_check", "zkhip_ctx_set_checked", "zkhip_ctx_unsatisfied", "zkhip_ctx_dispatch_count",
         "zkhip_assignment_pack_bound", "zkhip_assignment_pack", "zkhip_assignment_unpack", "zkhip_prog_assignment_packed",
         "zkhip_assignment_upload_packed",
         "zkhip_queue_open", "zkhip_queue_state", "zkhip_queue_submit", "zkhip_queue_submit_packed", "zkhip_queue_ready", "zkhip_queue_collect",
@@ -156,6 +156,7 @@
         L.zkhip_r1cs_check.restype = i32; L.zkhip_r1cs_check.argtypes = [vp] * 6
         L.zkhip_ctx_set_checked.restype = i32; L.zkhip_ctx_set_checked.argtypes = [vp, i32]
         L.zkhip_ctx_unsatisfied.restype = i32; L.zkhip_ctx_unsatisfied.argtypes = [vp, u32, vp, vp, vp, vp]
+        L.zkhip_ctx_dispatch_count.restype = i32; L.zkhip_ctx_dispatch_count.argtypes = [vp, u32, vp]
         L.zkhip_assignment_pack_bound.restype = i32; L.zkhip_assignment_pack_bound.argtypes = [u64, vp]
         L.zkhip_assignment_pack.restype = i32; L.zkhip_assignment_pack.argtypes = [vp, u64, vp, u64, vp]
         L.zkhip_assignment_unpack.restype = i32; L.zkhip_assignment_unpack.argtypes = [vp, sz, vp, u64, vp]
@@ -225,6 +226,11 @@
         idx, row, bad = np.zeros(max(k, 1), dtype=np.uint32), np.zeros(max(k, 1), dtype=np.uint64), np.zeros(max(k, 1), dtype=np.uint64)
         self.lib.L.zkhip_ctx_unsatisfied(self.h, k, _ptr(idx), _ptr(row), _ptr(bad), C.byref(count))
         return [(int(idx[i]), int(row[i]), int(bad[i])) for i in range(k)]
+
+    def dispatch_count(self):
+        out = np.zeros(8, dtype=np.uint64)
+        self._check(self.lib.L.zkhip_ctx_dispatch_count(self.h, 8, _ptr(out)))
+        return {"kernels": int(out[0]), "copies": int(out[1]), "heavy_launches": int(out[2]), "heavy": [int(v) for v in out[3:8]]}
 
     def describe(self):
         buf = C.create_string_buffer(256)
```

After: 109.9. About the same (-0.1%).
